# Grice-Lab/HmmUFOtu

Hardware: AMD Instinct MI355X
Metric: reads placed/sec (whole node), gg_97_otus GTR+dGamma 250bp; HBM GB/s %peak (higher is better)
Workload: dtype f64

## Files before the change

hmmufotu_amd/csrc/hu_engine.hip:

```cpp
#include <algorithm>
#include <cmath>
#include <cstdio>
#include <cstring>
#include <limits>
#include <map>
#include <atomic>
#include <thread>
#include <memory>
#include <mutex>
#include <chrono>
#include <fstream>
#include <sstream>
#include <new>
#include <stdexcept>
#include <fcntl.h>
#include <unistd.h>
#include "hu_common.h"
#include "hu_kern_sep.h"
#include "hu_kern_align.h"
#include "hu_kern_tree.h"
#include "hu_kern_blk.h"
#include "hu_kern_refsort.h"
#include "hu_kern_rank.h"
#include "hu_kern_anneal.h"
#include "hu_kern_build.h"
#include "hu_kern_otucs.h"
#include "hu_kern_sum.h"
#include "hu_sum_rule.h"
#include "hu_kern_csfm.h"
#include "hu_kern_sm.h"
#include "hu_kern_sim.h"

#define HIPCHK(call) do { hipError_t e_ = (call); if(e_ != hipSuccess) { \
	hu_set_error("%s failed: %s (%s:%d)", #call, hipGetErrorString(e_), __FILE__, __LINE__); return HU_ERR_DEVICE; } } while(0)

static const double kInf = std::numeric_limits<double>::infinity();

#include <condition_variable>
#include <functional>
struct HuPool {
	std::vector<std::thread> th;
	std::mutex m;
	std::condition_variable cvGo, cvDone;
	std::function<void(size_t)> fn;
	size_t n = 0, chunk = 64;
	std::atomic<size_t> next{0};
	uint64_t gen = 0;
	int active = 0, permit = 0;
	bool quit = false;
	std::exception_ptr err;
	explicit HuPool(unsigned nt) {
		try { th.reserve(nt); } catch(...) { return; }
		for(unsigned t = 0; t < nt; ++t) try { th.emplace_back([this] {
			uint64_t seen = 0;
			for(;;) {
				{
					std::unique_lock<std::mutex> lk(m);
					cvGo.wait(lk, [&] { return quit || gen != seen; });
					if(quit) return;
					seen = gen;
					if(permit > 0) --permit; else { if(--active == 0) cvDone.notify_all(); continue; }
				}
				work();
				std::lock_guard<std::mutex> lk(m);
				if(--active == 0) cvDone.notify_all();
			}
		}); } catch(...) { break; }
	}
	void work() noexcept {
		for(;;) {
			size_t a = next.fetch_add(chunk); if(a >= n) break; size_t e = std::min(n, a + chunk);
			try { for(size_t i = a; i < e; ++i) fn(i); }
			catch(...) { std::lock_guard<std::mutex> lk(m); if(!err) err = std::current_exception(); next = n; }
		}
	}
	template<class F> void run(size_t count, F f) {
		const int got = hu_helpers_acquire((int) th.size());
		{
			std::lock_guard<std::mutex> lk(m);
			fn = f; n = count; next = 0; active = (int) th.size(); permit = got; err = nullptr; ++gen;
		}
		cvGo.notify_all();
		work();
		std::unique_lock<std::mutex> lk(m);
		cvDone.wait(lk, [&] { return active == 0; });
		hu_helpers_release(got);
		if(err) { std::exception_ptr e = err; err = nullptr; lk.unlock(); std::rethrow_exception(e); }
	}
	~HuPool() { { std::lock_guard<std::mutex> lk(m); quit = true; } cvGo.notify_all(); for(auto& t : th) t.join(); }
};
template<class F> static void parallel_for(size_t n, F f) {
	static const unsigned cap = [] { const char* e = getenv("HU_HOST_THREADS"); int v = e ? atoi(e) : 8; return (unsigned)(v < 1 ? 1 : v > 64 ? 64 : v); }();
	unsigned nt = std::thread::hardware_concurrency();
	if(nt > cap) nt = cap;
	if(n < 512 || nt <= 1) { for(size_t i = 0; i < n; ++i) f(i); return; }
	static thread_local std::unique_ptr<HuPool> pool;
	if(!pool) pool.reset(new HuPool(nt - 1));
	pool->run(n, f);
}

template<class T> struct PinnedAlloc {
	typedef T value_type;
	PinnedAlloc() = default;
	template<class U> PinnedAlloc(const PinnedAlloc<U>&) {}
	T* allocate(size_t n) {
		void* p = nullptr;
		if(hipHostMalloc(&p, n * sizeof(T), hipHostMallocDefault) != hipSuccess) { (void) hipGetLastError(); p = malloc(n * sizeof(T)); std::lock_guard<std::mutex> lk(mtx()); pageable().push_back(p); }
		if(!p) throw std::bad_alloc();
		return (T*) p;
	}
	void deallocate(T* p, size_t) {
		{
			std::lock_guard<std::mutex> lk(mtx());
			auto& v = pageable();
			for(size_t i = 0; i < v.size(); ++i) if(v[i] == (void*) p) { v.erase(v.begin() + i); free(p); return; }
		}
		(void) hipHostFree(p);
	}
	static std::vector<void*>& pageable() { static std::vector<void*> v; return v; }
	static std::mutex& mtx() { static std::mutex m; return m; }
	template<class U> bool operator==(const PinnedAlloc<U>&) const { return true; }
	template<class U> bool operator!=(const PinnedAlloc<U>&) const { return false; }
};
template<class T> using PinnedVec = std::vector<T, PinnedAlloc<T>>;

template<class X> struct DBuf {
	X* p = nullptr; size_t cap = 0;
	int ensure(size_t n) {
		if(n <= cap) return HU_OK;
		if(p) (void) hipFree(p);
		p = nullptr; cap = 0;
		size_t want = n + n / 8 + 16;
		hipError_t e = hipMalloc((void**) &p, want * sizeof(X));
		if(e != hipSuccess) { hu_set_error("hipMalloc(%zu bytes) failed: %s", want * sizeof(X), hipGetErrorString(e)); return HU_ERR_NOMEM; }
		cap = want;
		return HU_OK;
	}
	void free_() { if(p) (void) hipFree(p); p = nullptr; cap = 0; }
	DBuf() = default;
	DBuf(const DBuf&) = delete;
	DBuf& operator=(const DBuf&) = delete;
	~DBuf() { free_(); }
};

struct hu_db {
	int device = 0;
	HuDbDev dev;
	double partialFrac = 0;
	HuModelDev mdl;
	hu_model_desc mdesc;
	HuProfileHost prof;
	std::vector<int32_t> parent, annoId;
	std::vector<double> blen, height, annoDist;
	std::vector<int8_t> seq;
	std::vector<std::string> annos, names;
	std::vector<void*> allocs;
	int64_t hbmBytes = 0;
	int32_t* dAnnoId = nullptr;
	double* dLlTab = nullptr;
	bool hasInvalidCode = false;
	std::mutex annealMu;
	bool annealReady = false;
	uint4* dInvPlane = nullptr;
	unsigned long long* dLeafMask = nullptr;
	std::vector<int32_t> colPos;
};

template<class X> static int dev_alloc(hu_db* db, X** p, size_t n) {
	size_t bytes = std::max<size_t>(n, 1) * sizeof(X);
	hipError_t e = hipMalloc((void**) p, bytes);
	if(e != hipSuccess) { hu_set_error("hipMalloc(%zu bytes) failed: %s", bytes, hipGetErrorString(e)); return HU_ERR_NOMEM; }
	db->allocs.push_back(*p);
	db->hbmBytes += (int64_t) bytes;
	return HU_OK;
}
template<class X> static int dev_upload(hu_db* db, X** p, const X* src, size_t n) {
	int rc = dev_alloc(db, p, n);
	if(rc != HU_OK) return rc;
	if(n) HIPCHK(hipMemcpy(*p, src, n * sizeof(X), hipMemcpyHostToDevice));
	return HU_OK;
}

extern "C" int hu_device_count(void) try {
	int n = 0;
	if(hipGetDeviceCount(&n) != hipSuccess) return 0;
	int ok = 0;
	for(int i = 0; i < n; ++i) {
		hipDeviceProp_t p;
		if(hipGetDeviceProperties(&p, i) == hipSuccess && strncmp(p.gcnArchName, "gfx950", 6) == 0) ok++;
	}
	return ok;
} catch(...) { return hu_catch_all("hu_device_count"); }

static int init_sym_map() {
	int8_t m[128];
	for(int i = 0; i < 128; ++i) m[i] = -1;
	m['A'] = 0; m['C'] = 1; m['G'] = 2; m['T'] = 3; m['U'] = 3;
	m['M'] = 0; m['R'] = 0; m['W'] = 0; m['S'] = 1; m['Y'] = 1; m['K'] = 2;
	m['V'] = 0; m['H'] = 0; m['D'] = 0; m['B'] = 1; m['N'] = 0;
	m['-'] = -2; m['.'] = -2; m['_'] = -2;
	HIPCHK(hipMemcpyToSymbol(HIP_SYMBOL(c_sym_map), m, sizeof(m)));
	return HU_OK;
}
static int8_t host_sym(char c) {
	switch(c) {
	case 'A': case 'M': case 'R': case 'W': case 'V': case 'H': case 'D': case 'N': return 0;
	case 'C': case 'S': case 'Y': case 'B': return 1;
	case 'G': case 'K': return 2;
	case 'T': case 'U': return 3;
	case '-': case '.': case '_': return -2;
	default: return -1;
	}
}

static hipError_t hu_wait(hipStream_t st) {
	static const bool spin = [] { const char* e = getenv("HU_SYNC"); return e && !strcmp(e, "spin"); }();
	if(spin) return hipStreamSynchronize(st);
	const auto t0 = std::chrono::steady_clock::now();
	long ns = 20000;
	for(;;) {
		const hipError_t e = hipStreamQuery(st);
		if(e != hipErrorNotReady) return e;
		if(std::chrono::steady_clock::now() - t0 < std::chrono::microseconds(30)) continue;
		timespec ts{0, ns};
		nanosleep(&ts, nullptr);
		if(ns < 100000) ns += 20000;
	}
}

extern "C" int hu_db_create(const hu_profile_desc* prof, const hu_tree_desc* tree, const hu_model_desc* model,
		int device, hu_db** out) try {
	if(!prof || !tree || !model || !out) { hu_set_error("hu_db_create: null argument"); return HU_ERR_ARG; }
	*out = nullptr;
	if(hu_device_count() <= 0) { hu_set_error("no gfx950 device visible: the engine has no CPU path"); return HU_ERR_DEVICE; }
	HIPCHK(hipSetDevice(device));
	hu_db* db = new hu_db;
	bool built = false;
	HuScope guard([&] { if(!built) hu_db_destroy(db); });
	db->device = device;
	int rc = db->prof.init(prof);
	if(rc == HU_OK) rc = hu_model_prepare(model, &db->mdl);
	if(rc != HU_OK) return rc;
	db->mdesc = *model;
	const int n = tree->n_nodes, L = tree->cs_len;
	if(n < 2 || n >= (1 << 24) || L != prof->L) { hu_set_error("tree: n_nodes %d / cs_len %d inconsistent with profile L %d", n, L, prof->L); return HU_ERR_ARG; }
	const int64_t winStart = tree->win_len > 0 ? tree->win_start : 0, winLen = tree->win_len > 0 ? tree->win_len : L;
	if(winStart < 0 || winStart + winLen > L) { hu_set_error("tree: message window out of range"); return HU_ERR_ARG; }
	db->parent.assign(tree->parent, tree->parent + n);
	db->blen.assign(tree->blen, tree->blen + n);
	db->height.assign(tree->height, tree->height + n);
	db->seq.assign(tree->seq, tree->seq + (size_t) n * L);
	if(tree->anno_id) db->annoId.assign(tree->anno_id, tree->anno_id + n);
	else { db->annoId.resize(n); for(int i = 0; i < n; ++i) db->annoId[i] = i; }
	if(tree->anno_dist) db->annoDist.assign(tree->anno_dist, tree->anno_dist + n); else db->annoDist.assign(n, 0.0);
	int root = -1, nroot = 0;
	for(int i = 0; i < n; ++i) {
		if(db->parent[i] < 0) { root = i; nroot++; }
		else if(db->parent[i] >= n) { hu_set_error("tree: parent of node %d out of range", i); return HU_ERR_ARG; }
	}
	if(nroot != 1) { hu_set_error("tree: %d roots", nroot); return HU_ERR_ARG; }
	HuDbDev& d = db->dev;
	memset(&d, 0, sizeof(d));
	d.nNodes = n; d.csLen = L; d.root = root;
	d.nNodesPad = (n + HU_NODE_PAD - 1) / HU_NODE_PAD * HU_NODE_PAD;
	d.W = (L + 31) / 32; d.WQ = (L + 127) / 128;
	d.winStart = winStart; d.winLen = winLen;
	d.K = prof->K; d.L = L;
	auto fail = [&](int code) { return code; };
	std::vector<int32_t> posCol((size_t) d.WQ * 128, -1), colPos(L, -1);
	{
		int p = 0;
		for(int k = 1; k <= prof->K; ++k) { const int c = db->prof.p2cs[k] - 1; colPos[c] = p; posCol[p++] = c; }
		for(int c = 0; c < L; ++c) if(colPos[c] < 0) { colPos[c] = p; posCol[p++] = c; }
		int32_t* dp = nullptr;
		if((rc = dev_upload(db, &dp, posCol.data(), posCol.size())) != HU_OK) return fail(rc);
		d.posCol = dp;
	}
	{
		const size_t np = d.nNodesPad, cnt = (size_t) d.WQ * 3 * np;
		std::vector<uint4> pl(cnt, make_uint4(0, 0, 0, 0));
		for(int i = 0; i < n; ++i) {
			const int8_t* s = &db->seq[(size_t) i * L];
			for(int cc = 0; cc < L; ++cc) {
				const int code = s[cc];
				if(code == -1) db->hasInvalidCode = true;
				if(code < 0) continue;
				const int c = colPos[cc];
				const int q = c >> 7, w = (c >> 5) & 3; const uint32_t bit = 1u << (c & 31);
				uint32_t* p0 = &pl[((size_t) q * 3 + 0) * np + i].x + w;
				uint32_t* p1 = &pl[((size_t) q * 3 + 1) * np + i].x + w;
				uint32_t* pv = &pl[((size_t) q * 3 + 2) * np + i].x + w;
				if(code & 1) *p0 |= bit;
				if(code & 2) *p1 |= bit;
				*pv |= bit;
			}
		}
		uint4* dp = nullptr;
		if((rc = dev_upload(db, &dp, pl.data(), cnt)) != HU_OK) return fail(rc);
		d.planes = dp;
		d.QM = (prof->K + 127) / 128;
		if(d.WQ > d.QM) {
			unsigned long long* cp = nullptr;
			if((rc = dev_alloc(db, &cp, (size_t)(d.WQ - d.QM) * 128 * 3 * (np / 64))) != HU_OK) return fail(rc);
			k_col_planes<<<dim3((unsigned)(np / 64), (unsigned)(d.WQ - d.QM)), 64>>>(d, cp);
			hipError_t e1 = hipGetLastError(), e2 = hipDeviceSynchronize();
			if(e1 != hipSuccess || e2 != hipSuccess) { hu_set_error("transposing the non-profile planes failed: %s", hipGetErrorString(e1 != hipSuccess ? e1 : e2)); return fail(HU_ERR_DEVICE); }
			d.colPlanes = cp;
		}
// ... 1046 lines not shown
	if(n_items > 0) { SCHK(hipMalloc((void**) &dItems, itemBytes)); SCHK(hipMalloc((void**) &dOut, outBytes)); }
	if(stride != cs_len) {
		SCHK(hipMemset(dRows, 0xFE, rowBytes));
		SCHK(hipMemcpy2D(dRows, (size_t) stride, rows, (size_t) cs_len, (size_t) cs_len, (size_t) n_rows, hipMemcpyHostToDevice));
	}
	else SCHK(hipMemcpy(dRows, rows, rowBytes, hipMemcpyHostToDevice));
	if(n_items > 0) SCHK(hipMemcpy(dItems, items, itemBytes, hipMemcpyHostToDevice));
	SCHK(hipDeviceSynchronize());
	g_smTiming[0] = since();
	(void) hipGetLastError();
	k_sm_counts<<<(unsigned)(n_items + n_rows), HU_SM_BLOCK>>>(dRows, n_rows, stride / 16, dItems, n_items, dOut, dBase);
	SCHK(hipGetLastError());
	SCHK(hipDeviceSynchronize());
	g_smTiming[1] = since() - g_smTiming[0];
	SCHK(hipMemcpy(base, dBase, baseBytes, hipMemcpyDeviceToHost));
	if(n_items > 0) {
		std::vector<int32_t> out((size_t) n_items * HU_SM_VALUES);
		SCHK(hipMemcpy(out.data(), dOut, outBytes, hipMemcpyDeviceToHost));
		for(int64_t i = 0; i < n_items; ++i) { memcpy(counts + 16 * i, out.data() + HU_SM_VALUES * i, 64); memcpy(dn + 4 * i, out.data() + HU_SM_VALUES * i + 16, 16); }
	}
	g_smTiming[2] = since() - g_smTiming[0] - g_smTiming[1];
	#undef SCHK
	return HU_OK;
} catch(...) { return hu_catch_all("hu_sm_counts"); }
extern "C" int hu_sm_counts_timing(double* seconds) {
	if(!seconds) return HU_ERR_ARG;
	memcpy(seconds, g_smTiming, sizeof(g_smTiming));
	return HU_OK;
}

static thread_local double g_simTiming[3] = {0, 0, 0};
extern "C" int hu_sim_reads(const hu_db* db, int64_t n, const int32_t* node, const double* rc, const int32_t* start, const int32_t* end,
		const double* gap_frac, uint64_t seed, uint64_t read0, int want_mate, char* aligned, char* seq, char* mate, int32_t* seq_len) try {
	const char* fn = "hu_sim_reads";
	if(!db || n < 0 || n > INT32_MAX || !gap_frac || (n > 0 && (!node || !rc || !start || !end || !aligned || !seq || !seq_len || (want_mate && !mate)))) { hu_set_error("%s: bad argument", fn); return HU_ERR_ARG; }
	const HuDbDev& d = db->dev;
	if(d.winStart != 0 || d.winLen != d.csLen) { hu_set_error("%s: the database holds a column window; the simulation needs the whole database", fn); return HU_ERR_ARG; }
	std::vector<int64_t> off((size_t) n);
	int64_t total = 0;
	for(int64_t r = 0; r < n; ++r) {
		if(node[r] < 0 || node[r] >= d.nNodes || node[r] == d.root) { hu_set_error("%s: read %lld: node %d is %s", fn, (long long) r, node[r], node[r] == d.root ? "the root, which has no branch above it" : "not a node of the database"); return HU_ERR_ARG; }
		if(!(start[r] >= 0 && start[r] <= end[r] && end[r] < d.csLen)) { hu_set_error("%s: read %lld: columns %d .. %d of a database of %d", fn, (long long) r, start[r], end[r], d.csLen); return HU_ERR_ARG; }
		if(!(rc[r] >= 0 && rc[r] <= 1)) { hu_set_error("%s: read %lld: branch point %g outside [0, 1]", fn, (long long) r, rc[r]); return HU_ERR_ARG; }
		off[(size_t) r] = total;
		total += (int64_t) end[r] - start[r] + 1;
	}
	if(n == 0) { g_simTiming[0] = g_simTiming[1] = g_simTiming[2] = 0; return HU_OK; }
	HIPCHK(hipSetDevice(db->device));
	const size_t L = (size_t) d.csLen, R = (size_t) n, T = (size_t) total;
	const size_t planBytes = R * (4 + 8 + 4 + 4 + 8 + 4);
	const int nOut = want_mate ? 3 : 2;
	char* dOut = nullptr; double *dGap = nullptr, *dRc = nullptr; int64_t* dOff = nullptr; int32_t* dI = nullptr;
	HuScope guard([&] { (void) hipFree(dOut); (void) hipFree(dGap); (void) hipFree(dRc); (void) hipFree(dOff); (void) hipFree(dI); });
	#define SCHK(call) do { hipError_t e_ = (call); if(e_ != hipSuccess) { hu_set_error("%s: %s failed: %s", fn, #call, hipGetErrorString(e_)); return HU_ERR_DEVICE; } } while(0)
	{
		size_t freeB = 0, totB = 0;
		SCHK(hipMemGetInfo(&freeB, &totB));
		const size_t need = T * nOut + L * 8 + planBytes + 4096;
		if(need > freeB) { hu_set_error("%s: %lld reads of %lld columns need %.3f GB of device memory, %.3f GB are free", fn, (long long) n, (long long) total, need / 1e9, freeB / 1e9); return HU_ERR_NOMEM; }
	}
	auto t0 = std::chrono::steady_clock::now();
	auto since = [&] { return std::chrono::duration<double>(std::chrono::steady_clock::now() - t0).count(); };
	SCHK(hipMalloc((void**) &dOut, T * nOut)); SCHK(hipMalloc((void**) &dGap, L * 8)); SCHK(hipMalloc((void**) &dRc, R * 8));
	SCHK(hipMalloc((void**) &dOff, R * 8)); SCHK(hipMalloc((void**) &dI, R * 16));
	SCHK(hipMemcpy(dGap, gap_frac, L * 8, hipMemcpyHostToDevice)); SCHK(hipMemcpy(dRc, rc, R * 8, hipMemcpyHostToDevice));
	SCHK(hipMemcpy(dOff, off.data(), R * 8, hipMemcpyHostToDevice));
	SCHK(hipMemcpy(dI, node, R * 4, hipMemcpyHostToDevice)); SCHK(hipMemcpy(dI + R, start, R * 4, hipMemcpyHostToDevice)); SCHK(hipMemcpy(dI + 2 * R, end, R * 4, hipMemcpyHostToDevice));
	SCHK(hipDeviceSynchronize());
	g_simTiming[0] = since();
	HuSimArgs a;
	a.up = d.up; a.down = d.down; a.blen = d.blen; a.csLen = d.csLen; a.gapFrac = dGap;
	a.node = dI; a.start = dI + R; a.end = dI + 2 * R; a.rc = dRc; a.off = dOff;
	a.key0 = (uint32_t)(seed & 0xffffffffu); a.key1 = (uint32_t)(seed >> 32); a.read0 = read0;
	a.aligned = dOut; a.seq = dOut + T; a.mate = want_mate ? dOut + 2 * T : nullptr; a.seqLen = dI + 3 * R;
	(void) hipGetLastError();
	k_sim_reads<<<(unsigned) n, HU_SIM_BLOCK>>>(db->mdl, a);
	SCHK(hipGetLastError());
	SCHK(hipDeviceSynchronize());
	g_simTiming[1] = since() - g_simTiming[0];
	std::vector<char> hOut(T * nOut); std::vector<int32_t> hLen(R);
	SCHK(hipMemcpy(hOut.data(), dOut, T * nOut, hipMemcpyDeviceToHost)); SCHK(hipMemcpy(hLen.data(), dI + 3 * R, R * 4, hipMemcpyDeviceToHost));
	memcpy(aligned, hOut.data(), T); memcpy(seq_len, hLen.data(), R * 4);
	memset(seq, 0, T); if(want_mate) memset(mate, 0, T);
	for(size_t r = 0; r < R; ++r) {
		memcpy(seq + off[r], hOut.data() + T + off[r], (size_t) hLen[r]);
		if(want_mate) memcpy(mate + off[r], hOut.data() + 2 * T + off[r], (size_t) hLen[r]);
	}
	g_simTiming[2] = since() - g_simTiming[0] - g_simTiming[1];
	#undef SCHK
	return HU_OK;
} catch(...) { return hu_catch_all("hu_sim_reads"); }
extern "C" int hu_sim_timing(double* seconds) {
	if(!seconds) return HU_ERR_ARG;
	memcpy(seconds, g_simTiming, sizeof(g_simTiming));
	return HU_OK;
}
extern "C" int hu_sim_gap_frac(const hu_db* db, int64_t n_seq, int64_t msa_len, const char* msa, double* gap_frac) try {
	const char* fn = "hu_sim_gap_frac";
	if(!db || !gap_frac || (msa && (n_seq < 1 || msa_len < 1))) { hu_set_error("%s: bad argument", fn); return HU_ERR_ARG; }
	const int64_t L = db->dev.csLen, n = db->dev.nNodes;
	std::vector<char> own;
	if(!msa) {
		std::vector<int32_t> nb((size_t) n, 0);
		for(int64_t i = 0; i < n; ++i) if(db->parent[i] >= 0) { ++nb[i]; ++nb[db->parent[i]]; }
		n_seq = 0;
		for(int64_t i = 0; i < n; ++i) n_seq += nb[i] == 1;
		if(n_seq < 1) { hu_set_error("%s: the tree has no leaf", fn); return HU_ERR_ARG; }
		own.resize((size_t) n_seq * L);
		size_t k = 0;
		for(int64_t i = 0; i < n; ++i) if(nb[i] == 1) { const int8_t* s = &db->seq[(size_t) i * L]; for(int64_t j = 0; j < L; ++j) { const int8_t b = s[j]; own[k++] = b >= 0 && b < 4 ? "ACGT"[b] : '-'; } }
		msa = own.data(); msa_len = L;
	}
	const size_t M = (size_t) msa_len, N = (size_t) n_seq;
	std::vector<int32_t> res(4 * M), gap(M), st(N), en(N), ln(N);
	std::vector<double> sw(N), wres(4 * M), wgap(M);
	const int rc = hu_msa_stats(db->device, n_seq, msa_len, msa, res.data(), gap.data(), st.data(), en.data(), ln.data(), sw.data(), wres.data(), wgap.data());
	if(rc != HU_OK) return rc;
	const bool prune = own.empty();
	int64_t kept = 0;
	for(size_t j = 0; j < M; ++j) kept += !prune || (res[j] | res[M + j] | res[2 * M + j] | res[3 * M + j]) != 0;
	if(kept != L) { hu_set_error("%s: %lld columns of the alignment hold a residue, the database has %lld columns", fn, (long long) kept, (long long) L); return HU_ERR_ARG; }
	size_t k = 0;
	for(size_t j = 0; j < M; ++j) {
		if(prune && !(res[j] | res[M + j] | res[2 * M + j] | res[3 * M + j])) continue;
		const double numRes = (wres[j] + wres[2 * M + j]) + (wres[M + j] + wres[3 * M + j]);
		gap_frac[k++] = wgap[j] / (numRes + wgap[j]);
	}
	return HU_OK;
} catch(...) { return hu_catch_all("hu_sim_gap_frac"); }

extern "C" int hu_device_mem_info(int device, int64_t* free_bytes, int64_t* total_bytes) try {
	if(hu_device_count() <= 0) { hu_set_error("no gfx950 device visible: the engine has no CPU path"); return HU_ERR_DEVICE; }
	HIPCHK(hipSetDevice(device));
	size_t f = 0, t = 0;
	HIPCHK(hipMemGetInfo(&f, &t));
	if(free_bytes) *free_bytes = (int64_t) f; if(total_bytes) *total_bytes = (int64_t) t;
	return HU_OK;
} catch(...) { return hu_catch_all("hu_device_mem_info"); }
extern "C" int hu_device_malloc(int device, int64_t bytes, void** out) try {
	if(!out || bytes < 1) { hu_set_error("hu_device_malloc: bad argument"); return HU_ERR_ARG; }
	*out = nullptr;
	if(hu_device_count() <= 0) { hu_set_error("no gfx950 device visible: the engine has no CPU path"); return HU_ERR_DEVICE; }
	HIPCHK(hipSetDevice(device));
	const hipError_t e = hipMalloc(out, (size_t) bytes);
	if(e != hipSuccess) { (void) hipGetLastError(); *out = nullptr; hu_set_error("hipMalloc(%lld bytes) failed: %s", (long long) bytes, hipGetErrorString(e)); return HU_ERR_NOMEM; }
	return HU_OK;
} catch(...) { return hu_catch_all("hu_device_malloc"); }
extern "C" void hu_device_free(int device, void* p) try {
	if(!p) return;
	if(hipSetDevice(device) == hipSuccess) (void) hipFree(p);
} catch(...) { (void) hu_catch_all("hu_device_free"); }

namespace {
struct HuSaDev {
	uint8_t* text = nullptr; uint64_t* key[2] = {nullptr, nullptr}; uint32_t* pos[2] = {nullptr, nullptr};
	uint32_t *rank = nullptr, *hist = nullptr, *tileSum = nullptr;
	int cur = 0;
	void dropKeys() { (void) hipFree(key[0]); (void) hipFree(key[1]); key[0] = key[1] = nullptr; }
	~HuSaDev() { dropKeys(); (void) hipFree(text); (void) hipFree(pos[0]); (void) hipFree(pos[1]); (void) hipFree(rank); (void) hipFree(hist); (void) hipFree(tileSum); }
};
inline uint32_t sa_bits(uint64_t v) { uint32_t b = 0; while(v) { ++b; v >>= 1; } return b; }
}
#define SCHK(call) do { hipError_t e_ = (call); if(e_ != hipSuccess) { hu_set_error("%s: %s failed: %s", fn, #call, hipGetErrorString(e_)); return HU_ERR_DEVICE; } } while(0)
static int sa_build(const char* fn, int device, const uint8_t* text, int64_t n64, int64_t extraBytes, HuSaDev& d, int32_t* rounds, double* seconds) {
	if(!text || n64 < 1 || n64 >= (1ll << 31)) { hu_set_error("%s: the text must hold 1 .. 2^31 - 1 symbols, got %lld", fn, (long long) n64); return HU_ERR_ARG; }
	const size_t n = (size_t) n64;
	for(size_t i = 0; i < n; ++i) if(text[i] > 4) { hu_set_error("%s: symbol %d at text position %zu (0 = separator, 1..4 = bases)", fn, (int) text[i], i); return HU_ERR_ARG; }
	if(hu_device_count() <= 0) { hu_set_error("no gfx950 device visible: the engine has no CPU path"); return HU_ERR_DEVICE; }
	SCHK(hipSetDevice(device));
	const uint32_t nTiles = (uint32_t)((n + HU_SA_TILE - 1) / HU_SA_TILE);
	const size_t m = (size_t) nTiles * 256, nScanN = (n + 1023) / 1024, nScanM = (m + 1023) / 1024;
	{
		size_t freeB = 0, totB = 0;
		SCHK(hipMemGetInfo(&freeB, &totB));
		const size_t need = n + 2 * 8 * n + 2 * 4 * n + 4 * n + 4 * m + 4 * (std::max(nScanN, nScanM) + 1) + (size_t) std::max<int64_t>(extraBytes, 0) + 4096;
		if(need > freeB) { hu_set_error("%s: a text of %zu symbols needs %.3f GB of device memory, %.3f GB are free", fn, n, need / 1e9, freeB / 1e9); return HU_ERR_NOMEM; }
	}
	SCHK(hipMalloc((void**) &d.text, n)); SCHK(hipMalloc((void**) &d.key[0], 8 * n)); SCHK(hipMalloc((void**) &d.key[1], 8 * n));
	SCHK(hipMalloc((void**) &d.pos[0], 4 * n)); SCHK(hipMalloc((void**) &d.pos[1], 4 * n)); SCHK(hipMalloc((void**) &d.rank, 4 * n));
	SCHK(hipMalloc((void**) &d.hist, 4 * m)); SCHK(hipMalloc((void**) &d.tileSum, 4 * (std::max(nScanN, nScanM) + 1)));
	SCHK(hipMemcpy(d.text, text, n, hipMemcpyHostToDevice));
	(void) hipGetLastError();
	const auto t0 = std::chrono::steady_clock::now();
	const unsigned gN = (unsigned)((n + 255) / 256), gT = (nTiles + 3) / 4;
	auto pass = [&](int shift) {
		k_sa_hist<<<gT, 256>>>(d.key[d.cur], n, shift, nTiles, d.hist);
		k_sa_scan_sums<<<(unsigned) nScanM, 1024>>>(m, d.hist, d.tileSum);
		k_sa_scan_tiles<<<1, 1024>>>(nScanM, d.tileSum);
		k_sa_scan_apply<<<(unsigned) nScanM, 1024>>>(m, d.hist, d.tileSum);
		k_sa_scatter<<<gT, 256>>>(d.key[d.cur], d.pos[d.cur], n, shift, nTiles, d.hist, d.key[d.cur ^ 1], d.pos[d.cur ^ 1]);
		d.cur ^= 1;
	};
	uint32_t groups = 0;
	auto rank = [&]() -> int {
		k_sa_head_sums<<<(unsigned) nScanN, 1024>>>(d.key[d.cur], n, d.tileSum);
		k_sa_scan_tiles<<<1, 1024>>>(nScanN, d.tileSum);
		k_sa_rank<<<(unsigned) nScanN, 1024>>>(d.key[d.cur], d.pos[d.cur], n, d.tileSum, d.rank);
		SCHK(hipGetLastError());
		SCHK(hipMemcpy(&groups, d.tileSum + nScanN, 4, hipMemcpyDeviceToHost));
		return HU_OK;
	};
	k_sa_key0<<<gN, 256>>>(d.text, n, d.key[d.cur], d.pos[d.cur]);
	for(int shift = 0; shift < 3 * HU_SA_H0; shift += 8) pass(shift);
	int rc = rank();
	if(rc != HU_OK) return rc;
	int32_t r = 0;
	const int32_t maxRounds = (int32_t) sa_bits(n - 1) + 2;
	for(size_t h = HU_SA_H0; groups < n; h *= 2) {
		if(++r > maxRounds || groups == 0) { hu_set_error("%s: internal: %u of %zu suffixes told apart after %d doubling rounds", fn, groups, n, (int) r - 1); return HU_ERR_STATE; }
		k_sa_key<<<gN, 256>>>(d.rank, n, h, d.key[d.cur], d.pos[d.cur]);
		for(int shift = 0; shift < (int) sa_bits(groups); shift += 8) pass(shift);
		for(int shift = 0; shift < (int) sa_bits(groups - 1); shift += 8) pass(32 + shift);
		if((rc = rank()) != HU_OK) return rc;
	}
	SCHK(hipDeviceSynchronize());
	if(rounds) *rounds = r;
	if(seconds) *seconds = std::chrono::duration<double>(std::chrono::steady_clock::now() - t0).count();
	return HU_OK;
}
extern "C" int32_t hu_suffix_array_tile(void) { return HU_SA_TILE; }
extern "C" int hu_suffix_array(int device, const uint8_t* text, int64_t n, int32_t* sa, int32_t* rounds, double* device_seconds) try {
	const char* fn = "hu_suffix_array";
	if(!sa) { hu_set_error("%s: bad argument", fn); return HU_ERR_ARG; }
	HuSaDev d;
	const int rc = sa_build(fn, device, text, n, 0, d, rounds, device_seconds);
	if(rc != HU_OK) return rc;
	SCHK(hipMemcpy(sa, d.pos[d.cur], 4 * (size_t) n, hipMemcpyDeviceToHost));
	return HU_OK;
} catch(...) { return hu_catch_all("hu_suffix_array"); }
int hu_csfm_device_pass(int device, const uint8_t* text, int64_t n64, uint8_t* bwt, uint64_t* marks, uint32_t* sampled, int32_t* rounds, double* sa_seconds) {
	const char* fn = "hu_csfm_write";
	HuSaDev d;
	const int rc = sa_build(fn, device, text, n64, 0, d, rounds, sa_seconds);
	if(rc != HU_OK) return rc;
	const size_t n = (size_t) n64, nScan = (n + 1023) / 1024, nWords = (n + 63) / 64, nSamp = (n + 3) / 4;
	d.dropKeys();
	uint8_t* dBwt = nullptr; unsigned long long* dMarks = nullptr; uint32_t* dSamp = nullptr;
	HuScope guard([&] { (void) hipFree(dBwt); (void) hipFree(dMarks); (void) hipFree(dSamp); });
	SCHK(hipMalloc((void**) &dBwt, n)); SCHK(hipMalloc((void**) &dMarks, 8 * nWords)); SCHK(hipMalloc((void**) &dSamp, 4 * nSamp));
	k_csfm_bwt<<<(unsigned) nScan, 1024>>>(d.text, d.pos[d.cur], n, dBwt, dMarks, d.tileSum);
	k_sa_scan_tiles<<<1, 1024>>>(nScan, d.tileSum);
	k_csfm_samples<<<(unsigned) nScan, 1024>>>(d.pos[d.cur], n, d.tileSum, nSamp, dSamp);
	SCHK(hipGetLastError());
	uint32_t got = 0;
	SCHK(hipMemcpy(&got, d.tileSum + nScan, 4, hipMemcpyDeviceToHost));
	if(got != nSamp) { hu_set_error("%s: internal: %u sampled rows, expected %zu: the sort did not return a permutation", fn, got, nSamp); return HU_ERR_STATE; }
	SCHK(hipMemcpy(bwt, dBwt, n, hipMemcpyDeviceToHost)); SCHK(hipMemcpy(marks, dMarks, 8 * nWords, hipMemcpyDeviceToHost));
	SCHK(hipMemcpy(sampled, dSamp, 4 * nSamp, hipMemcpyDeviceToHost));
	return HU_OK;
}
#undef SCHK

extern "C" int hu_tree_loglik(int device, int32_t n_nodes, int32_t cs_len, int32_t root, const hu_model_desc* model, const double* up_dev,
		double* per_col, double* sum) try {
	if(n_nodes < 1 || cs_len < 1 || root < 0 || root >= n_nodes || !model || !up_dev || !sum) { hu_set_error("hu_tree_loglik: bad argument"); return HU_ERR_ARG; }
	if(((uintptr_t) up_dev) & 15) { hu_set_error("hu_tree_loglik: the message buffer must be 16-byte aligned"); return HU_ERR_ARG; }
	if(hu_device_count() <= 0) { hu_set_error("no gfx950 device visible: the engine has no CPU path"); return HU_ERR_DEVICE; }
	HuModelDev mdl;
	int rc = hu_model_prepare(model, &mdl);
	if(rc != HU_OK) return rc;
	HIPCHK(hipSetDevice(device));
	const int64_t L = cs_len;
	DBuf<double> dOut;
	if((rc = dOut.ensure((size_t) L)) != HU_OK) return rc;
	(void) hipGetLastError();
	k_tree_loglik<<<(unsigned)((L + 255) / 256), 256>>>(up_dev + (size_t) root * L * 4, L, mdl.pi[0], mdl.pi[1], mdl.pi[2], mdl.pi[3], dOut.p);
	HIPCHK(hipGetLastError());
	std::vector<double> own;
	if(!per_col) { own.resize((size_t) L); per_col = own.data(); }
	HIPCHK(hipMemcpy(per_col, dOut.p, (size_t) L * 8, hipMemcpyDeviceToHost));
	double s = 0;
	for(int64_t j = 0; j < L; ++j) s += per_col[j];
	*sum = s;
	return HU_OK;
} catch(...) { return hu_catch_all("hu_tree_loglik"); }


typedef HuPlaceRec HostPlace;

struct HuKnobs {
	int viterbi_hbm = 0;
	int viterbi_values = 0;
	int viterbi_mode = 0;
	int viterbi_dec1 = 0;
	int vw_diag = 0;
	int viterbi_force_redo = 0;
	int tile_unsorted = 0;
	int pairs32 = 0;
	int topk_fast_min = 16384;
	int topk_general = 0;
	int scan_pairs = 0;
	int streaming_sep = 0;
	int est_unsorted = 0, place_unsorted = 0;
	int xcd_map = 1;
	int est_var = 0, place_var = 0;
	int place_nosplit = 0;
	int place_lds_pad = 0;
	int est_lds_pad = 0;
	int vit_lds_pad = 0;
	int scan_lds_pad = 0;
	int trace = 0;
	int width_split = 1;
	int sort_seq = 0;
	int refsort_wgs = HU_RS_WGS_PER_CU * 256;
	int ref_nofuse = 0;
	int refsort_host = 0;
	int inject_fault = 0;
};
struct HuKnobEntry { const char* name; int HuKnobs::* field; };
static const HuKnobEntry kKnobs[] = {
	{"viterbi_hbm", &HuKnobs::viterbi_hbm}, {"viterbi_values", &HuKnobs::viterbi_values}, {"viterbi_mode", &HuKnobs::viterbi_mode},
	{"viterbi_dec1", &HuKnobs::viterbi_dec1}, {"vw_diag", &HuKnobs::vw_diag}, {"viterbi_force_redo", &HuKnobs::viterbi_force_redo},
	{"pairs32", &HuKnobs::pairs32}, {"tile_unsorted", &HuKnobs::tile_unsorted}, {"topk_fast_min", &HuKnobs::topk_fast_min}, {"scan_pairs", &HuKnobs::scan_pairs}, {"topk_general", &HuKnobs::topk_general}, {"streaming_sep", &HuKnobs::streaming_sep},
	{"est_unsorted", &HuKnobs::est_unsorted}, {"place_unsorted", &HuKnobs::place_unsorted}, {"xcd_map", &HuKnobs::xcd_map},
	{"est_var", &HuKnobs::est_var}, {"place_var", &HuKnobs::place_var}, {"place_nosplit", &HuKnobs::place_nosplit}, {"width_split", &HuKnobs::width_split},
	{"place_lds_pad", &HuKnobs::place_lds_pad}, {"est_lds_pad", &HuKnobs::est_lds_pad}, {"vit_lds_pad", &HuKnobs::vit_lds_pad}, {"scan_lds_pad", &HuKnobs::scan_lds_pad}, {"trace", &HuKnobs::trace}, {"inject_fault", &HuKnobs::inject_fault}, {"refsort_host", &HuKnobs::refsort_host}, {"ref_nofuse", &HuKnobs::ref_nofuse}, {"refsort_wgs", &HuKnobs::refsort_wgs}, {"sort_seq", &HuKnobs::sort_seq},
};
static void knobs_from_env(HuKnobs& k) {
	for(const HuKnobEntry& e : kKnobs) {
		std::string env = "HU_";
		for(const char* c = e.name; *c; ++c) env += (char) toupper(*c);
		const char* v = getenv(env.c_str());
		if(!v) continue;
		char* end = nullptr;
		const long x = strtol(v, &end, 10);
		k.*(e.field) = (end == v) ? 1 : (int) x;
	}
}

enum { ST_NONE = 0, ST_READS = 1, ST_ALIGNED = 2, ST_SEEDED = 3, ST_ESTIMATED = 4, ST_FILTERED = 5, ST_PLACED = 6, ST_FINISHED = 7 };

struct hu_batch {
	hu_db* db = nullptr;
	int maxReads = 0, n = 0, nSeq = 0, state = ST_NONE;
	bool paired = false, fromCodes = false, profile = false;
	HuKnobs knob;
	int maxBases = 1 << 30;
	bool fixedRoot = false;
	bool placesGiven = false;
	bool pair16 = false;
	int scanWidth = 0;
	int pairsKind = 0;
	int seedCap = HU_MAX_SEEDS;
	hipStream_t stream = nullptr;
	hipEvent_t ev[2 * HU_T_COUNT];
	bool evSet[HU_T_COUNT] = {false};
	float ms[HU_T_COUNT];
	double wall[4] = {0, 0, 0, 0};
	DBuf<char> dBases, dTraces, dRows;
	DBuf<HuReadDesc> dDescs;
	DBuf<double> dScratch;
	DBuf<uint8_t> dDec;
	DBuf<HuVitOut> dVit;
	DBuf<HuAlnDev> dAlns;
	DBuf<int8_t> dCodes;
	DBuf<int32_t> dStart, dEnd, dSeedCnt, dSeedId, dGiven, dPermCnt;
	DBuf<uint16_t> dPerm;
	DBuf<uint32_t> dRp, dPairs, dSeedDN, dParDN, dBmin, dRSpan, dTileSpan;
	DBuf<int32_t> dTileQ, dSlotRead, dReadSlot;
	DBuf<uint32_t> dRq, dTileW;
	DBuf<unsigned long long> dRefScratch;
	DBuf<int32_t> dHv, dZeroPar; DBuf<unsigned long long> dPairsC; int refHvCount = 0; double refHvHeight = NAN;
	DBuf<int32_t> dBail, dNanCnt, dNanId; DBuf<uint32_t> dNanDN;
	int nRefBail = 0;
	DBuf<uint32_t> dRefPiv; DBuf<unsigned long long> dRefL0; bool refFused = false;
	int refHostAll = 0;
	DBuf<int32_t> dIns, dTileIns, dRetry;
	DBuf<uint32_t> dSortK, dSortV;
	DBuf<uint32_t> dCsCnt;
	DBuf<HuEstOut> dEst;
	DBuf<HuCand> dCands;
	DBuf<HuPlaceOut> dPlaceOut;
	DBuf<int32_t> dCandCnt, dCandOff, dMeta;
	DBuf<uint8_t> dFiltSlot;
	DBuf<HuPlaceRec> dPlaces;
	DBuf<hu_place_rec> dBest;
	size_t nc = 0;
	int maxGapSites = 0, maxBaseSites = 0;
	bool hostCands = false;
	DBuf<double> dRootLL;
	PinnedVec<double> hRootLL;
	std::vector<HuReadDesc> hDescs;
	std::vector<char> hBases;
	PinnedVec<HuVitOut> hVit;
	int64_t cellsTotal = 0, cornerTotal = 0;
	int rMain = 0;
	int maxAll = 1, maxMain = 1;
	std::vector<int32_t> wideReads;
	std::vector<uint32_t> hWideOrd, hWideCand; DBuf<uint32_t> dWideOrd, dWideCand;
	PinnedVec<int32_t> hCandOffAll;
	DBuf<double> dRedoScr; DBuf<HuReadDesc> dRedoDesc; DBuf<HuVitOut> dRedoVit;
	PinnedVec<HuAlnDev> hAlns;
	DBuf<int32_t> dAnRow, dAnThr, dAnTileQ; DBuf<int2> dAnReg; DBuf<uint32_t> dAnMasks; DBuf<unsigned long long> dAnHits;
	PinnedVec<int32_t> hStart, hEnd, hSeedCnt, hSeedId;
	PinnedVec<uint32_t> hSeedDN;
	PinnedVec<HuCand> hCands;
	std::vector<int64_t> candOffs;
	std::vector<HostPlace> places;
	PinnedVec<hu_place_rec> best;
	PinnedVec<int32_t> hMeta, hBail;
	PinnedVec<char> hRows;
	DBuf<uint32_t> dSumBits; DBuf<unsigned char> dSumCls; DBuf<int4> dSumOut; PinnedVec<int4> hSumOut; bool sumReady = false;
	std::vector<char> tsvBuf; std::vector<size_t> tsvOff, tsvLen; size_t tsvSize = 0;
};

struct Timer {
	hu_batch* b; int id;
	Timer(hu_batch* b, int id) : b(b), id(id) { if(b->profile) (void) hipEventRecord(b->ev[2 * id], b->stream); }
	~Timer() { if(b->profile) { (void) hipEventRecord(b->ev[2 * id + 1], b->stream); b->evSet[id] = true; } }
};

extern "C" int hu_batch_create(hu_db* db, int max_reads, hu_batch** out) try {
	if(!db || !out || max_reads < 1) { hu_set_error("hu_batch_create: bad argument"); return HU_ERR_ARG; }
	HIPCHK(hipSetDevice(db->device));
	hu_batch* b = new hu_batch;
	b->db = db; b->maxReads = max_reads;
	knobs_from_env(b->knob);
	for(int i = 0; i < 2 * HU_T_COUNT; ++i) b->ev[i] = nullptr;
	for(int i = 0; i < HU_T_COUNT; ++i) b->ms[i] = 0;
	hipError_t e = hipStreamCreateWithFlags(&b->stream, hipStreamNonBlocking);
	for(int i = 0; i < 2 * HU_T_COUNT && e == hipSuccess; ++i) e = hipEventCreate(&b->ev[i]);
	if(e != hipSuccess) {
		hu_set_error("hu_batch_create: stream / event creation failed: %s", hipGetErrorString(e));
		for(int i = 0; i < 2 * HU_T_COUNT; ++i) if(b->ev[i]) (void) hipEventDestroy(b->ev[i]);
		if(b->stream) (void) hipStreamDestroy(b->stream);
		delete b;
		return HU_ERR_DEVICE;
	}
	*out = b;
	return HU_OK;
} catch(...) { return hu_catch_all("hu_batch_create"); }
extern "C" int hu_batch_set_knob(hu_batch* b, const char* name, int value) try {
	if(!b || !name) return HU_ERR_ARG;
	for(const HuKnobEntry& e : kKnobs) if(strcmp(e.name, name) == 0) { b->knob.*(e.field) = value; return HU_OK; }
	hu_set_error("hu_batch_set_knob: no knob named '%s'", name);
	return HU_ERR_ARG;
} catch(...) { return hu_catch_all("hu_batch_set_knob"); }
extern "C" void hu_batch_destroy(hu_batch* b) try {
	if(!b) return;
	(void) hipSetDevice(b->db->device);
	(void) hu_wait(b->stream);
	for(int i = 0; i < 2 * HU_T_COUNT; ++i) (void) hipEventDestroy(b->ev[i]);
	(void) hipStreamDestroy(b->stream);
	delete b;
} catch(...) { (void) hu_catch_all("hu_batch_destroy"); }
extern "C" int hu_batch_sync(hu_batch* b) try { if(!b) return HU_ERR_ARG; HIPCHK(hu_wait(b->stream)); return HU_OK; } catch(...) { return hu_catch_all("hu_batch_sync"); }
extern "C" int hu_batch_profile(hu_batch* b, int enable) try { if(!b) return HU_ERR_ARG; b->profile = enable != 0; return HU_OK; } catch(...) { return hu_catch_all("hu_batch_profile"); }
extern "C" int hu_batch_timings(hu_batch* b, float* ms) try {
	if(!b || !ms) return HU_ERR_ARG;
	HIPCHK(hu_wait(b->stream));
	for(int i = 0; i < HU_T_COUNT; ++i) {
		float t = 0;
		if(b->profile && b->evSet[i] && hipEventElapsedTime(&t, b->ev[2 * i], b->ev[2 * i + 1]) == hipSuccess) b->ms[i] = t;
		ms[i] = b->ms[i];
	}
	return HU_OK;
} catch(...) { return hu_catch_all("hu_batch_timings"); }

static void build_regions(const hu_db* db, int L, const int32_t* vp , HuReadDesc& rd) {
	const int K = db->dev.K;
	const double kMinGapFrac = 0.2;
	struct VP { int start, end, from, to, nIns, nDel; } v[2];
	int nv = 0;
	for(int p = 0; p < 2 && vp; ++p) {
		VP x{vp[p*6], vp[p*6+1], vp[p*6+2], vp[p*6+3], vp[p*6+4], vp[p*6+5]};
		bool valid = x.start > 0 && x.start <= x.end && x.from > 0 && x.from <= x.to && x.nIns >= 0 && x.nDel >= 0;
		if(valid && x.end <= K && x.to <= L) v[nv++] = x;
	}
	rd.nRegions = 0;
	int64_t off = 0, doff = 0;
	auto add = [&](int j0, int j1, int i0, int i1, int withB, int band, const VP* bp) {
		HuRegion& g = rd.reg[rd.nRegions++];
		g.j0 = j0; g.j1 = j1; g.i0 = i0; g.i1 = i1; g.withB = withB; g.band = band;
		g.from = bp ? bp->from : 0; g.start = bp ? bp->start : 0; g.nIns = bp ? bp->nIns : 0; g.nDel = bp ? bp->nDel : 0;
		g.off = off; g.doff = doff;
		if(j1 >= j0 && i1 >= i0) {
			off += (int64_t)(j1 - j0 + 1) * (i1 - i0 + 1);
			const int64_t ni = i1 - i0 + 1, nj = j1 - j0 + 1;
			int64_t sz = (ni + nj - 1) * ((ni + 15) & ~15);
			sz = std::max(sz, (ni + nj - 1) * 64);
			sz = std::max(sz, (nj + (ni + 3) / 4 - 1) * 256);
			sz = std::max(sz, (nj + (ni + 7) / 8 - 1) * 512);
			doff += (sz + 15) & ~(int64_t) 15;
		}
	};
	if(nv == 0) add(1, K, 1, L, 1, 0, nullptr);
	else {
		for(int p = 0; p < nv; ++p) {
			int upQLen = p == 0 ? v[p].from - 1 : v[p].from - v[p - 1].to;
			if(upQLen < 0) upQLen = 0;
			int up_start = p == 0 ? v[p].start - upQLen * (1 + kMinGapFrac) : v[p - 1].end;
			if(up_start < 1) up_start = 1;
			int up_from = p == 0 ? v[p].from - upQLen * (1 + kMinGapFrac) : v[p - 1].to;
			if(up_from < 1) up_from = 1;
			add(up_start, v[p].start, up_from, v[p].from, 1, 0, nullptr);
			add(v[p].start, v[p].end, v[p].from, v[p].to, 1, 1, &v[p]);
		}
		const VP& last = v[nv - 1];
		int downQLen = L - last.to;
		int down_end = last.end + downQLen * (1 + kMinGapFrac);
		int down_to = last.to + downQLen * (1 + kMinGapFrac);
		if(down_end > K) down_end = K;
		if(down_to > L) down_to = L;
		add(last.end, down_end, last.to, down_to, 0, 0, nullptr);
	}
	int64_t coff = 0;
	for(int r = 0; r < rd.nRegions; ++r) {
		HuRegion& g = rd.reg[r];
		int nearI = INT32_MAX, nearJ = INT32_MAX;
		for(int r2 = r + 1; r2 < rd.nRegions; ++r2) {
			const HuRegion& g2 = rd.reg[r2];
			if(g2.i1 >= g2.i0 && g2.j1 >= g2.j0) { nearI = std::min(nearI, g2.i0 - 1); nearJ = std::min(nearJ, g2.j0 - 1); }
		}
		g.ci0 = std::max(g.i0, nearI); g.cj0 = std::max(g.j0, nearJ); g.coff = coff;
		if(nearI == INT32_MAX || g.ci0 > g.i1 || g.cj0 > g.j1 || g.i1 < g.i0 || g.j1 < g.j0) { g.ci0 = g.i1 + 1; g.cj0 = g.j1 + 1; }
		else coff += (int64_t)(g.i1 - g.ci0 + 1) * (g.j1 - g.cj0 + 1);
	}
	rd.scratchOff = off;
	rd.decOff = doff;
	rd.cornerOff = coff;
}

static int upload_descs(hu_batch* b) {
	int rc;
	if((rc = b->dDescs.ensure(b->hDescs.size())) != HU_OK) return rc;
	HIPCHK(hipMemcpyAsync(b->dDescs.p, b->hDescs.data(), b->hDescs.size() * sizeof(HuReadDesc), hipMemcpyHostToDevice, b->stream));
	return HU_OK;
}

extern "C" int hu_batch_set_reads(hu_batch* b, int n, const char* bases, const int64_t* offs, const int32_t* vpaths,
		const char* mates, const int64_t* moffs, const int32_t* mvpaths) try {
	if(!b || n < 0 || n > b->maxReads || (n > 0 && (!bases || !offs))) { hu_set_error("hu_batch_set_reads: bad argument"); return HU_ERR_ARG; }
	if(mates && !moffs) { hu_set_error("hu_batch_set_reads: mates without offsets"); return HU_ERR_ARG; }
	HIPCHK(hipSetDevice(b->db->device));
	b->n = n; b->paired = mates != nullptr; b->nSeq = b->paired ? 2 * n : n; b->fromCodes = false;
	b->hDescs.assign(b->nSeq, HuReadDesc());
	b->hBases.clear();
	b->maxBases = 0;
	for(int r = 0; r < n; ++r) {
		const int64_t l = (offs[r + 1] - offs[r]) + (mates ? moffs[r + 1] - moffs[r] : 0);
		if(l > b->maxBases) b->maxBases = (int) std::min<int64_t>(l, 1 << 30);
	}
	int64_t cells = 0, tr = 0, decs = 0, corners = 0;
	for(int s = 0; s < b->nSeq; ++s) {
		const bool isMate = s >= n;
		const int r = isMate ? s - n : s;
		const char* src = isMate ? mates + moffs[r] : bases + offs[r];
		const int64_t len64 = isMate ? moffs[r + 1] - moffs[r] : offs[r + 1] - offs[r];
		HuReadDesc& rd = b->hDescs[s];
		memset(&rd, 0, sizeof(rd));
		rd.baseOff = (int64_t) b->hBases.size();
		rd.len = (int32_t) len64;
		bool bad = len64 < 1 || len64 > 65535;
		for(int64_t i = 0; i < len64 && !bad; ++i) if(host_sym(src[i]) < 0) bad = true;
		if(!bad) {
			b->hBases.insert(b->hBases.end(), src, src + len64);
			const int32_t* vp = isMate ? (mvpaths ? mvpaths + (size_t) r * 12 : nullptr) : (vpaths ? vpaths + (size_t) r * 12 : nullptr);
			build_regions(b->db, rd.len, vp, rd);
			const int64_t c = rd.scratchOff, dc = rd.decOff, cc = rd.cornerOff;
			rd.scratchOff = cells; cells += c;
			rd.decOff = decs; decs += dc;
			rd.cornerOff = corners; corners += cc;
		}
		else { rd.len = 0; rd.nRegions = 0; }
		rd.traceOff = tr;
		tr += rd.len + b->db->dev.K + 8;
	}
	int rc;
	if((rc = b->dBases.ensure(b->hBases.size() + 1)) != HU_OK) return rc;
	b->cellsTotal = cells; b->cornerTotal = corners;
	if((rc = b->dDec.ensure((size_t) decs + 1)) != HU_OK) return rc;
	if((rc = b->dTraces.ensure((size_t) tr + 1)) != HU_OK) return rc;
	if((rc = b->dVit.ensure(b->nSeq)) != HU_OK) return rc;
	if(!b->hBases.empty()) HIPCHK(hipMemcpyAsync(b->dBases.p, b->hBases.data(), b->hBases.size(), hipMemcpyHostToDevice, b->stream));
	if((rc = upload_descs(b)) != HU_OK) return rc;
	b->state = ST_READS;
	return HU_OK;
} catch(...) { return hu_catch_all("hu_batch_set_reads"); }

static int ensure_read_buffers(hu_batch* b) {
	const HuDbDev& d = b->db->dev;
	const size_t n = (size_t) b->n;
	const size_t tiles = (n + HU_READ_TILE - 1) / HU_READ_TILE;
	int rc;
	if((rc = b->dCodes.ensure(n * d.csLen)) != HU_OK) return rc;
	if((rc = b->dStart.ensure(n)) != HU_OK) return rc;
	if((rc = b->dEnd.ensure(n)) != HU_OK) return rc;
	if((rc = b->dRp.ensure(tiles * d.WQ * HU_READ_TILE * 16)) != HU_OK) return rc;
	if((rc = b->dTileQ.ensure(tiles * (d.WQ + 1))) != HU_OK) return rc;
	if((rc = b->dTileW.ensure(std::max<size_t>(tiles, 1) * d.WQ * HU_TILEW_QUAD)) != HU_OK) return rc;
	if((rc = b->dSlotRead.ensure(std::max<size_t>(tiles, 1) * HU_READ_TILE)) != HU_OK) return rc;
	if((rc = b->dReadSlot.ensure(std::max<size_t>(n, 1))) != HU_OK) return rc;
	if((rc = b->dRq.ensure(std::max<size_t>(n, 1) * ((d.WQ + 31) / 32))) != HU_OK) return rc;
	if((rc = b->dIns.ensure(std::max<size_t>(n, 1) * (HU_MAX_INS + 1))) != HU_OK) return rc;
	if((rc = b->dTileIns.ensure(std::max<size_t>(tiles, 1) * HU_TILEINS_STRIDE)) != HU_OK) return rc;
	if((rc = b->dRSpan.ensure(std::max<size_t>(n, 1) * 2)) != HU_OK) return rc;
	if((rc = b->dTileSpan.ensure(std::max<size_t>(tiles, 1) * 2)) != HU_OK) return rc;
	return HU_OK;
}

static int order_by_key(hu_batch* b, const uint32_t* key, const uint32_t* val, size_t n, uint32_t bound, uint32_t* out, bool runsInOrder) {
	if(!n) return HU_OK;
	const size_t m = (size_t) bound + 1;
	int rc;
	const size_t nTiles = (m + 1023) / 1024;
	if((rc = b->dCsCnt.ensure(3 * m + nTiles + 8)) != HU_OK) return rc;
	uint32_t* cnt = b->dCsCnt.p; uint32_t* start = cnt + m; uint32_t* cur = start + m + 1; uint32_t* tiles = cur + m;
	HIPCHK(hipMemsetAsync(cnt, 0, m * 4, b->stream));
	k_cs_hist<<<(unsigned)((n + 255) / 256), 256, 0, b->stream>>>((int) n, key, bound, cnt);
	k_cs_tile_sums<<<(unsigned) nTiles, 1024, 0, b->stream>>>((int) m, cnt, tiles);
	k_cs_scan_tiles<<<1, 1024, 0, b->stream>>>((int) nTiles, tiles);
	k_cs_scan<<<(unsigned) nTiles, 1024, 0, b->stream>>>((int) m, cnt, tiles, start, cur);
	k_cs_scatter<<<(unsigned)((n + 255) / 256), 256, 0, b->stream>>>((int) n, key, val, bound, cur, out);
	if(runsInOrder) k_cs_runs<<<(unsigned)((m + 3) / 4), 256, 0, b->stream>>>((int) bound, start, out);
	HIPCHK(hipGetLastError());
	return HU_OK;
}

static int tile_reads(hu_batch* b, const HuAlnDev* alns) {
	const int n = b->n;
	if(!n) return HU_OK;
	const int tiles = (n + HU_READ_TILE - 1) / HU_READ_TILE;
	int rc;
	if((rc = b->dSortK.ensure((size_t) n * 2)) != HU_OK || (rc = b->dSortV.ensure((size_t) n * 2)) != HU_OK) return rc;
	k_tile_keys<<<(n + 255) / 256, 256, 0, b->stream>>>(n, alns, b->dStart.p, b->dEnd.p, b->dSortK.p, b->dSortV.p);
	if(b->knob.tile_unsorted) HIPCHK(hipMemcpyAsync(b->dSortV.p + n, b->dSortV.p, (size_t) n * 4, hipMemcpyDeviceToDevice, b->stream));
	else if((rc = order_by_key(b, b->dSortK.p, b->dSortV.p, (size_t) n, (uint32_t) b->db->dev.csLen + 1u, b->dSortV.p + n, true)) != HU_OK) return rc;
	k_tile_slots<<<(tiles * HU_READ_TILE + 255) / 256, 256, 0, b->stream>>>(n, tiles * HU_READ_TILE, b->dSortV.p + n, b->dSlotRead.p, b->dReadSlot.p);
	HIPCHK(hipGetLastError());
	return HU_OK;
}

static int set_aligned_impl(hu_batch* b, int n, const int8_t* codes, hipMemcpyKind kind, const int32_t* start, const int32_t* end, int maxBases = -1) {
	if(!b || n < 0 || n > b->maxReads || (n > 0 && (!codes || !start || !end))) { hu_set_error("hu_batch_set_aligned: bad argument"); return HU_ERR_ARG; }
	HIPCHK(hipSetDevice(b->db->device));
	const HuDbDev& d = b->db->dev;
	b->n = n; b->nSeq = n; b->paired = false; b->fromCodes = true;
	if(maxBases >= 0) b->maxBases = maxBases;
	else {
		int mb = 0;
		for(int r = 0; r < n; ++r) {
			if(!(start[r] >= 0 && start[r] <= end[r] && end[r] < d.csLen)) continue;
			const int8_t* c = codes + (size_t) r * d.csLen; int k = 0;
			for(int j = start[r]; j <= end[r]; ++j) k += c[j] >= 0;
			mb = std::max(mb, k);
		}
		b->maxBases = mb;
	}
	int rc;
	if((rc = ensure_read_buffers(b)) != HU_OK) return rc;
	b->hAlns.assign(n, HuAlnDev());
	b->hStart.assign(start, start + n); b->hEnd.assign(end, end + n);
	for(int r = 0; r < n; ++r) {
		HuAlnDev& a = b->hAlns[r];
		memset(&a, 0, sizeof(a));
		const bool ok = start[r] >= 0 && start[r] <= end[r] && end[r] < d.csLen && start[r] >= d.winStart && end[r] < d.winStart + d.winLen;
		a.status = ok ? HU_READ_OK : HU_READ_INVALID;
		a.csStart = start[r] + 1; a.csEnd = end[r] + 1;
		if(!ok) { b->hStart[r] = (int32_t) d.winStart; b->hEnd[r] = (int32_t) d.winStart - 1; }
	}
	(void) hipGetLastError();
	if(n) {
		if((const void*) codes != (const void*) b->dCodes.p) HIPCHK(hipMemcpyAsync(b->dCodes.p, codes, (size_t) n * d.csLen, kind, b->stream));
		HIPCHK(hipMemcpyAsync(b->dStart.p, b->hStart.data(), (size_t) n * 4, hipMemcpyHostToDevice, b->stream));
		HIPCHK(hipMemcpyAsync(b->dEnd.p, b->hEnd.data(), (size_t) n * 4, hipMemcpyHostToDevice, b->stream));
		const int tiles = (n + HU_READ_TILE - 1) / HU_READ_TILE;
		HIPCHK(hipMemsetAsync(b->dRp.p, 0, (size_t) tiles * d.WQ * HU_READ_TILE * 16 * 4, b->stream));
		if((rc = tile_reads(b, nullptr)) != HU_OK) return rc;
		k_planes_from_codes<<<n, 64, 0, b->stream>>>(d, b->dCodes.p, b->dStart.p, b->dEnd.p, b->dRp.p, b->dRq.p, b->dIns.p, b->dReadSlot.p, (uint2*) b->dRSpan.p);
		k_tile_lists<<<tiles, 64, 0, b->stream>>>(d, n, b->dRp.p, b->dRq.p, b->dIns.p, b->dTileQ.p, b->dTileW.p, b->dTileIns.p, b->dSlotRead.p, (const uint2*) b->dRSpan.p, (uint2*) b->dTileSpan.p);
		HIPCHK(hipGetLastError());
// ... 399 lines not shown
		for(int i = 0; i < hb[0]; ++i) nNan += (hb[2 + i] >> 26) == 3;
		const bool nanOnDevice = nNan > 16;
		if(nanOnDevice) {
			if((rc = b->dNanCnt.ensure((size_t) n)) != HU_OK || (rc = b->dNanId.ensure((size_t) n * HU_MAX_SEEDS)) != HU_OK || (rc = b->dNanDN.ensure((size_t) n * HU_MAX_SEEDS)) != HU_OK) return rc;
			if(b->pair16) k_seed_topk<uint16_t><<<n, 256, 0, b->stream>>>(d0, (const uint16_t*) b->dPairs.p, o->max_height, o->max_nseed, b->dNanCnt.p, b->dNanId.p, b->dNanDN.p, b->knob.topk_fast_min);
			else k_seed_topk<uint32_t><<<n, 256, 0, b->stream>>>(d0, b->dPairs.p, o->max_height, o->max_nseed, b->dNanCnt.p, b->dNanId.p, b->dNanDN.p, b->knob.topk_fast_min);
			k_take_nan_rows<<<hb[0], 64, 0, b->stream>>>(d0, b->dBail.p, b->dPairs.p, b->pair16 ? 1 : 0, b->dNanCnt.p, b->dNanId.p, b->dNanDN.p, b->dSeedCnt.p, b->dSeedId.p, b->dSeedDN.p, b->dParDN.p);
			HIPCHK(hipGetLastError());
			if(b->knob.trace) fprintf(stderr, "[hu] reference seed order: %d reads with a NaN distance take the (dist, node id) selection on the device\n", nNan);
		}
		for(int i = 0; i < hb[0]; ++i) if(!(nanOnDevice && (hb[2 + i] >> 26) == 3)) only.push_back(hb[2 + i] & 0x3ffffff);
		std::sort(only.begin(), only.end());
		if(!only.empty()) return seed_order_libstdcxx(b, o, &only);
	}
	return HU_OK;
}

static int seed_order_libstdcxx(hu_batch* b, const hu_opts* o, const std::vector<int32_t>* only) {
	const hu_db* db = b->db;
	const HuDbDev& d = db->dev;
	const size_t n = (size_t) b->n, np = (size_t) d.nNodesPad, K = (size_t) o->max_nseed;
	if(only) {
		const size_t rowB = np * (b->pair16 ? 2 : 4);
		std::vector<uint8_t> rowBuf(rowB);
		std::vector<uint64_t> a;
		const bool p16 = b->pair16;
		for(int32_t r : *only) {
			HIPCHK(hipMemcpyAsync(rowBuf.data(), (const uint8_t*) b->dPairs.p + (size_t) r * rowB, rowB, hipMemcpyDeviceToHost, b->stream));
			HIPCHK(hu_wait(b->stream));
			const uint16_t* q16 = (const uint16_t*) rowBuf.data(); const uint32_t* q32 = (const uint32_t*) rowBuf.data();
			auto pairOf = [&](int i) -> uint32_t { return p16 ? (((uint32_t)(q16[i] >> 8) << 16) | (q16[i] & 0xffu)) : q32[i]; };
			a.clear();
			bool nan = false;
			for(int i = 0; i < d.nNodes; ++i) {
				if(i == d.root || !(db->height[i] <= o->max_height)) continue;
				const uint32_t pr = pairOf(i); const uint64_t dd = pr >> 16, N = pr & 0xffffu;
				if(N == 0) { nan = true; a.push_back((((uint64_t) 1 << 39) + 1) << 24 | (uint64_t) i); continue; }
				a.push_back(((dd << 39) / N) << 24 | (uint64_t) i);
			}
			const size_t keep = std::min(K, a.size());
			if(!nan) hu_sort_prefix_packed(a.data(), a.size(), K); else std::partial_sort(a.begin(), a.begin() + keep, a.end());
			int32_t cnt = (b->hAlns[r].status == HU_READ_OK && b->hEnd[r] >= b->hStart[r]) ? (int32_t) keep : 0;
			int32_t ids[HU_MAX_SEEDS]; uint32_t dn[HU_MAX_SEEDS], pn[HU_MAX_SEEDS];
			for(size_t s = 0; s < keep; ++s) { const int id = (int)(a[s] & 0xffffffu); ids[s] = id; dn[s] = pairOf(id); pn[s] = pairOf(db->parent[id]); }
			HIPCHK(hipMemcpyAsync(b->dSeedCnt.p + r, &cnt, 4, hipMemcpyHostToDevice, b->stream));
			HIPCHK(hipMemcpyAsync(b->dSeedId.p + (size_t) r * HU_MAX_SEEDS, ids, keep * 4, hipMemcpyHostToDevice, b->stream));
			HIPCHK(hipMemcpyAsync(b->dSeedDN.p + (size_t) r * HU_MAX_SEEDS, dn, keep * 4, hipMemcpyHostToDevice, b->stream));
			HIPCHK(hipMemcpyAsync(b->dParDN.p + (size_t) r * HU_MAX_SEEDS, pn, keep * 4, hipMemcpyHostToDevice, b->stream));
			HIPCHK(hu_wait(b->stream));
		}
		return HU_OK;
	}
	const size_t rowBytes = np * (b->pair16 ? 2 : 4);
	const size_t CH = std::max<size_t>(1, std::min<size_t>(n, (192u << 20) / rowBytes));
	b->hSeedCnt.assign(n, 0); b->hSeedId.assign(n * HU_MAX_SEEDS, 0); b->hSeedDN.assign(n * HU_MAX_SEEDS, 0);
	PinnedVec<uint32_t> hPar(n * HU_MAX_SEEDS, 0);
	PinnedVec<uint8_t> buf[2];
	buf[0].resize(CH * rowBytes); buf[1].resize(CH * rowBytes);
	hipEvent_t ev[2] = {nullptr, nullptr};
	HuScope guard([&] { for(int i = 0; i < 2; ++i) if(ev[i]) (void) hipEventDestroy(ev[i]); });
	for(int i = 0; i < 2; ++i) HIPCHK(hipEventCreateWithFlags(&ev[i], hipEventDisableTiming));
	auto copy = [&](size_t c) -> int {
		const size_t r0 = c * CH, cnt = std::min(CH, n - r0);
		HIPCHK(hipMemcpyAsync(buf[c & 1].data(), (const uint8_t*) b->dPairs.p + r0 * rowBytes, cnt * rowBytes, hipMemcpyDeviceToHost, b->stream));
		HIPCHK(hipEventRecord(ev[c & 1], b->stream));
		return HU_OK;
	};
	const size_t nChunks = (n + CH - 1) / CH;
	const double maxH = o->max_height;
	const bool p16 = b->pair16;
	const uint64_t nanKey = ((uint64_t) 1 << 39) + 1;
	static const std::vector<uint64_t> key16 = [] {
		std::vector<uint64_t> t(65536);
		for(uint32_t v = 0; v < 65536; ++v) { const uint64_t dd = v >> 8, N = v & 0xffu; t[v] = N ? (dd << 39) / N : ((uint64_t) 1 << 39) + 1; }
		return t;
	}();
	int rc;
	if(nChunks && (rc = copy(0)) != HU_OK) return rc;
	for(size_t c = 0; c < nChunks; ++c) {
		HIPCHK(hipEventSynchronize(ev[c & 1]));
		if(c + 1 < nChunks && (rc = copy(c + 1)) != HU_OK) return rc;
		const size_t r0 = c * CH, cnt = std::min(CH, n - r0);
		const uint8_t* rows = buf[c & 1].data();
		static const unsigned sortThreads = [] { const char* e = getenv("HU_SORT_THREADS"); int v = e ? atoi(e) : 32; unsigned hw = std::thread::hardware_concurrency(); if(hw < 1) hw = 1; return (unsigned) std::min<int>(std::max(v, 1), (int) hw); }();
		std::atomic<size_t> next{0};
		auto oneRead = [&](size_t k) {
			const size_t r = r0 + k;
			if(b->hAlns[r].status != HU_READ_OK || b->hEnd[r] < b->hStart[r]) return;
			static thread_local std::vector<uint64_t> a;
			a.clear();
			const uint16_t* q16 = (const uint16_t*)(rows + k * rowBytes); const uint32_t* q32 = (const uint32_t*)(rows + k * rowBytes);
			auto pairOf = [&](int i) -> uint32_t { return p16 ? (((uint32_t)(q16[i] >> 8) << 16) | (q16[i] & 0xffu)) : q32[i]; };
			bool nan = false;
			for(int i = 0; i < d.nNodes; ++i) {
				if(i == d.root || !(db->height[i] <= maxH)) continue;
				if(p16) {
					const uint64_t kk = key16[q16[i]];
					nan |= kk == nanKey;
					a.push_back(kk << 24 | (uint64_t) i);
					continue;
				}
				const uint32_t pr = q32[i]; const uint64_t dd = pr >> 16, N = pr & 0xffffu;
				if(N == 0) { nan = true; a.push_back(nanKey << 24 | (uint64_t) i); continue; }
				a.push_back(((dd << 39) / N) << 24 | (uint64_t) i);
			}
			const size_t keep = std::min(K, a.size());
			if(!nan) hu_sort_prefix_packed(a.data(), a.size(), K);
			else std::partial_sort(a.begin(), a.begin() + keep, a.end());
			b->hSeedCnt[r] = (int32_t) keep;
			for(size_t s = 0; s < keep; ++s) {
				const int id = (int)(a[s] & 0xffffffu);
				b->hSeedId[r * HU_MAX_SEEDS + s] = id;
				b->hSeedDN[r * HU_MAX_SEEDS + s] = pairOf(id);
				hPar[r * HU_MAX_SEEDS + s] = pairOf(db->parent[id]);
			}
		};
		hu_run_threads(std::min<unsigned>(sortThreads, (unsigned) cnt), [&] { for(;;) { const size_t k = next.fetch_add(4); if(k >= cnt) break; for(size_t q = k; q < std::min(cnt, k + 4); ++q) oneRead(q); } });
	}
	if(n) {
		HIPCHK(hipMemcpyAsync(b->dSeedCnt.p, b->hSeedCnt.data(), n * 4, hipMemcpyHostToDevice, b->stream));
		HIPCHK(hipMemcpyAsync(b->dSeedId.p, b->hSeedId.data(), n * HU_MAX_SEEDS * 4, hipMemcpyHostToDevice, b->stream));
		HIPCHK(hipMemcpyAsync(b->dSeedDN.p, b->hSeedDN.data(), n * HU_MAX_SEEDS * 4, hipMemcpyHostToDevice, b->stream));
		HIPCHK(hipMemcpyAsync(b->dParDN.p, hPar.data(), n * HU_MAX_SEEDS * 4, hipMemcpyHostToDevice, b->stream));
		HIPCHK(hu_wait(b->stream));
	}
	return HU_OK;
}

extern "C" int hu_seed_batch(hu_batch* b, const hu_opts* o) try {
	if(!b || !o) return HU_ERR_ARG;
	if(b->state < ST_ALIGNED) { hu_set_error("hu_seed_batch: reads are not aligned"); return HU_ERR_STATE; }
	if(o->max_nseed < 1 || o->max_nseed > HU_MAX_SEEDS) { hu_set_error("max_nseed must be in 1..%d", HU_MAX_SEEDS); return HU_ERR_ARG; }
	HIPCHK(hipSetDevice(b->db->device));
	const HuDbDev& d = b->db->dev;
	const size_t n = (size_t) b->n;
	int rc;
	const int nBlk = d.nNodesPad / 256;
	const bool manyPartial = b->db->partialFrac > 0.02 && b->knob.scan_pairs != -1;
	if(o->seed_order != HU_SEED_ORDER_STABLE && o->seed_order != HU_SEED_ORDER_LIBSTDCXX) { hu_set_error("seed_order must be HU_SEED_ORDER_STABLE or HU_SEED_ORDER_LIBSTDCXX"); return HU_ERR_ARG; }
	const bool refOrder = o->seed_order == HU_SEED_ORDER_LIBSTDCXX;
	const bool dOnly = !refOrder && b->knob.scan_pairs != 1 && !manyPartial && o->max_height == INFINITY && nBlk >= 2 * o->max_nseed && nBlk <= 2048 && d.nNodes - 1 >= o->max_nseed;
	const bool narrow = !b->knob.pairs32 && b->maxBases <= 255;
	b->pair16 = !dOnly && narrow;
	b->pairsKind = dOnly ? 0 : (b->pair16 ? 16 : 32);
	b->scanWidth = dOnly ? (narrow ? 1 : 2) : 0;
	if((rc = b->dPairs.ensure(std::max<size_t>(n, 1) * d.nNodesPad / (dOnly ? (narrow ? 4 : 2) : (b->pair16 ? 2 : 1)))) != HU_OK) return rc;
	if((rc = b->dSeedCnt.ensure(n)) != HU_OK) return rc;
	if((rc = b->dSeedId.ensure(n * HU_MAX_SEEDS)) != HU_OK) return rc;
	if((rc = b->dSeedDN.ensure(n * HU_MAX_SEEDS)) != HU_OK) return rc;
	if((rc = b->dParDN.ensure(n * HU_MAX_SEEDS)) != HU_OK) return rc;
	uint32_t* bmin = nullptr;
	if(dOnly) {
		if((rc = b->dBmin.ensure(std::max<size_t>(n, 1) * nBlk + 16)) != HU_OK) return rc;
		if((rc = b->dRetry.ensure(n + 1)) != HU_OK) return rc;
		bmin = b->dBmin.p;
	}
	b->refFused = refOrder && n > 0 && ref_fused_l0(b, o, b->pair16);
	if(b->refFused) {
		if((rc = b->dRefPiv.ensure(n * 4)) != HU_OK || (rc = b->dRefL0.ensure(n * (size_t)(d.nNodesPad / 64) * 2)) != HU_OK) return rc;
		k_ref_pivots<<<(unsigned)((n + 63) / 64), 64, 0, b->stream>>>(d, read_planes(b), b->n, b->dRefPiv.p);
		HIPCHK(hipGetLastError());
	}
	uint32_t* stat = bmin && b->knob.trace ? bmin + n * nBlk : nullptr;
	if(stat) HIPCHK(hipMemsetAsync(stat, 0, 64, b->stream));
	(void) hipGetLastError();
	if(n) {
		const int tiles = (b->n + HU_READ_TILE - 1) / HU_READ_TILE;
		const dim3 grid(tiles, d.nNodesPad / 256);
		{
			Timer t(b, HU_T_SEED_PDIST);
			const dim3 grid4(tiles, (d.nNodesPad + 1023) / 1024);
			if(dOnly && narrow) k_seed_dscan4<uint8_t><<<grid4, 256, (size_t)(b->knob.scan_lds_pad > 0 && b->knob.scan_lds_pad <= 44 ? b->knob.scan_lds_pad : 0) * 1024, b->stream>>>(d, b->dRp.p, b->dTileQ.p, (uint8_t*) b->dPairs.p, b->dSlotRead.p, bmin, (const uint2*) b->dTileSpan.p);
			else if(dOnly) k_seed_dscan4<uint16_t><<<grid4, 256, 0, b->stream>>>(d, b->dRp.p, b->dTileQ.p, (uint16_t*) b->dPairs.p, b->dSlotRead.p, bmin, (const uint2*) b->dTileSpan.p);
			else if(b->refFused && b->pair16) k_seed_pdist2<uint16_t, true><<<grid, 256, 0, b->stream>>>(d, b->dTileW.p, b->dTileQ.p, b->dTileIns.p, (uint16_t*) b->dPairs.p, b->dSlotRead.p, b->dRefPiv.p, b->dRefL0.p);
			else if(b->refFused) k_seed_pdist2<uint32_t, true><<<grid, 256, 0, b->stream>>>(d, b->dTileW.p, b->dTileQ.p, b->dTileIns.p, b->dPairs.p, b->dSlotRead.p, b->dRefPiv.p, b->dRefL0.p);
			else if(b->pair16) k_seed_pdist2<uint16_t><<<grid, 256, 0, b->stream>>>(d, b->dTileW.p, b->dTileQ.p, b->dTileIns.p, (uint16_t*) b->dPairs.p, b->dSlotRead.p);
			else k_seed_pdist2<uint32_t><<<grid, 256, 0, b->stream>>>(d, b->dTileW.p, b->dTileQ.p, b->dTileIns.p, b->dPairs.p, b->dSlotRead.p);
		}
		{
			Timer t(b, HU_T_SEED_TOPK);
			if(dOnly) {
				int32_t* retry = b->dRetry.p;
				HIPCHK(hipMemsetAsync(retry, 0, 4, b->stream));
				#define TOPK_ARGS(T) d, (const T*) b->dPairs.p, bmin, read_planes(b), o->max_nseed, b->dSeedCnt.p, b->dSeedId.p, b->dSeedDN.p, b->dParDN.p, stat, retry
				if(narrow) { k_seed_topk_straight<uint8_t><<<b->n, 256, 0, b->stream>>>(TOPK_ARGS(uint8_t), b->knob.topk_general); k_seed_topk_d<uint8_t, true><<<std::min(b->n, 1024), 256, 0, b->stream>>>(TOPK_ARGS(uint8_t)); }
				else { k_seed_topk_straight<uint16_t><<<b->n, 256, 0, b->stream>>>(TOPK_ARGS(uint16_t), b->knob.topk_general); k_seed_topk_d<uint16_t, true><<<std::min(b->n, 1024), 256, 0, b->stream>>>(TOPK_ARGS(uint16_t)); }
				#undef TOPK_ARGS
			}
			else if(refOrder) { if((rc = seed_order_libstdcxx_device(b, o)) != HU_OK) return rc; }
			else {
				if(b->pair16) k_seed_topk<uint16_t><<<b->n, 256, 0, b->stream>>>(d, (const uint16_t*) b->dPairs.p, o->max_height, o->max_nseed, b->dSeedCnt.p, b->dSeedId.p, b->dSeedDN.p, b->knob.topk_fast_min);
				else k_seed_topk<uint32_t><<<b->n, 256, 0, b->stream>>>(d, b->dPairs.p, o->max_height, o->max_nseed, b->dSeedCnt.p, b->dSeedId.p, b->dSeedDN.p, b->knob.topk_fast_min);
				k_parent_pairs<<<((unsigned) n * HU_MAX_SEEDS + 255) / 256, 256, 0, b->stream>>>(d, b->n, b->dPairs.p, b->pair16 ? 1 : 0, b->dSeedCnt.p, b->dSeedId.p, b->dParDN.p);
			}
		}
		k_seed_drop_empty<<<(b->n + 255) / 256, 256, 0, b->stream>>>(b->n, b->dStart.p, b->dEnd.p, b->dSeedCnt.p);
		HIPCHK(hipGetLastError());
		if(stat) {
			uint32_t h[16];
			HIPCHK(hipMemcpyAsync(h, stat, 64, hipMemcpyDeviceToHost, b->stream)); HIPCHK(hu_wait(b->stream));
			fprintf(stderr, "[hu] top-k after the distance-only scan: %u of %zu reads on the block path (%.1f blocks, %.1f candidates per read), %u by the exact recomputation; "
				"%u of them through the general launch\n",
				h[0] + h[8], n, h[0] + h[8] ? (double) h[1] / (h[0] + h[8]) : 0.0, h[0] + h[8] ? (double) h[2] / (h[0] + h[8]) : 0.0, h[3], h[8]);
		}
	}
	b->seedCap = o->max_nseed;
	b->state = ST_SEEDED;
	return HU_OK;
} catch(...) { return hu_catch_all("hu_seed_batch"); }

__global__ void k_seed_drop_empty(int n, const int32_t* __restrict__ rstart, const int32_t* __restrict__ rend, int32_t* __restrict__ seedCnt) {
	const int r = blockIdx.x * 256 + threadIdx.x;
	if(r < n && rend[r] < rstart[r]) seedCnt[r] = 0;
}

__global__ void k_seed_given(HuDbDev db, HuReadPlanes R, int n, const int32_t* __restrict__ cnt, const int32_t* __restrict__ ids,
		const int32_t* __restrict__ distIds, int32_t* __restrict__ seedCnt, int32_t* __restrict__ seedId, uint32_t* __restrict__ seedDN, uint32_t* __restrict__ parDN) {
	const int i = blockIdx.x * 256 + threadIdx.x;
	if(i >= n * HU_MAX_SEEDS) return;
	const int r = i / HU_MAX_SEEDS, sl = i % HU_MAX_SEEDS;
	if(sl == 0) seedCnt[r] = cnt[r];
	if(sl < cnt[r]) {
		seedId[i] = ids[i];
		seedDN[i] = pair_exact(db, R, r, distIds ? distIds[i] : ids[i]);
		parDN[i] = pair_exact(db, R, r, db.parent[ids[i]]);
	}
}

extern "C" int hu_seed_batch_given(hu_batch* b, const int32_t* n_seeds, const int32_t* ids, const int32_t* dist_ids, int stride) try {
	if(!b || (b->n > 0 && (!n_seeds || !ids)) || stride < 1) { hu_set_error("hu_seed_batch_given: bad argument"); return HU_ERR_ARG; }
	if(b->state < ST_ALIGNED) { hu_set_error("hu_seed_batch_given: reads are not aligned"); return HU_ERR_STATE; }
	HIPCHK(hipSetDevice(b->db->device));
	const HuDbDev& d = b->db->dev;
	const size_t n = (size_t) b->n;
	std::vector<int32_t> pk((n * 3) * HU_MAX_SEEDS + n, 0);
	int32_t* pc = pk.data(); int32_t* pi = pc + n; int32_t* pd = pi + n * HU_MAX_SEEDS;
	for(size_t r = 0; r < n; ++r) {
		const int c = n_seeds[r];
		if(c < 0 || c > HU_MAX_SEEDS || c > stride) { hu_set_error("hu_seed_batch_given: read %zu has %d seeds (0..%d)", r, c, std::min(stride, (int) HU_MAX_SEEDS)); return HU_ERR_ARG; }
		pc[r] = c;
		for(int k = 0; k < c; ++k) {
			const int32_t id = ids[r * stride + k], di = dist_ids ? dist_ids[r * stride + k] : id;
			if(id < 0 || id >= d.nNodes || b->db->parent[id] < 0 || di < 0 || di >= d.nNodes) { hu_set_error("hu_seed_batch_given: read %zu seed %d names node %d / %d", r, k, id, di); return HU_ERR_ARG; }
			pi[r * HU_MAX_SEEDS + k] = id; pd[r * HU_MAX_SEEDS + k] = di;
		}
	}
	int rc;
	b->pair16 = false; b->pairsKind = 0; b->scanWidth = 0;
	if((rc = b->dSeedCnt.ensure(n)) != HU_OK) return rc;
	if((rc = b->dSeedId.ensure(n * HU_MAX_SEEDS)) != HU_OK) return rc;
	if((rc = b->dSeedDN.ensure(n * HU_MAX_SEEDS)) != HU_OK) return rc;
	if((rc = b->dParDN.ensure(n * HU_MAX_SEEDS)) != HU_OK) return rc;
	if((rc = b->dGiven.ensure(pk.size())) != HU_OK) return rc;
	(void) hipGetLastError();
	if(n) {
		HIPCHK(hipMemcpyAsync(b->dGiven.p, pk.data(), pk.size() * 4, hipMemcpyHostToDevice, b->stream));
		{
			Timer t(b, HU_T_SEED_PDIST);
			k_seed_given<<<((unsigned) n * HU_MAX_SEEDS + 255) / 256, 256, 0, b->stream>>>(d, read_planes(b), b->n, b->dGiven.p, b->dGiven.p + n,
					dist_ids ? b->dGiven.p + n + n * HU_MAX_SEEDS : nullptr, b->dSeedCnt.p, b->dSeedId.p, b->dSeedDN.p, b->dParDN.p);
			k_seed_drop_empty<<<(b->n + 255) / 256, 256, 0, b->stream>>>(b->n, b->dStart.p, b->dEnd.p, b->dSeedCnt.p);
		}
		HIPCHK(hipGetLastError());
		HIPCHK(hu_wait(b->stream));
	}
	b->seedCap = 1;
	for(size_t r = 0; r < n; ++r) b->seedCap = std::max(b->seedCap, (int) n_seeds[r]);
	b->state = ST_SEEDED;
	return HU_OK;
} catch(...) { return hu_catch_all("hu_seed_batch_given"); }

__global__ void k_seed_sortkeys(int n, const int32_t* __restrict__ seedCnt, const int32_t* __restrict__ seedId, uint32_t* __restrict__ key, uint32_t* __restrict__ val) {
	const int i = blockIdx.x * 256 + threadIdx.x;
	if(i >= n * HU_MAX_SEEDS) return;
	key[i] = (i % HU_MAX_SEEDS) < seedCnt[i / HU_MAX_SEEDS] ? (uint32_t) seedId[i] : 0xffffffffu;
	val[i] = (uint32_t) i;
}

static void plan_width_split(hu_batch* b) {
	b->rMain = 0; b->wideReads.clear(); b->maxAll = b->maxMain = 1;
	if((int) b->hStart.size() < b->n || (int) b->hEnd.size() < b->n) return;
	std::vector<int> R((size_t) b->n);
	for(int r = 0; r < b->n; ++r) { R[r] = std::max(0, b->hEnd[r] - b->hStart[r] + 1); b->maxAll = std::max(b->maxAll, R[r]); }
	b->maxMain = b->maxAll;
	if(!b->knob.width_split || b->n < 256) return;
	const int W = std::min(64, b->n / 128);
	std::vector<int> tmp(R);
	std::nth_element(tmp.begin(), tmp.begin() + W, tmp.end(), std::greater<int>());
	const int kth = tmp[W];
	static const int bounds[] = {512, 768, 1024, 1536, 2048, 3072};
	int bound = 0;
	for(int x : bounds) if(kth <= x) { bound = x; break; }
	if(!bound || bound >= b->maxAll) return;
	b->rMain = bound; b->maxMain = 1;
	for(int r = 0; r < b->n; ++r) { if(R[r] > bound) b->wideReads.push_back(r); else b->maxMain = std::max(b->maxMain, R[r]); }
	if(b->knob.trace) fprintf(stderr, "[hu] width split: %zu of %d reads beyond %d columns (widest %d) take a launch of their own\n", b->wideReads.size(), b->n, bound, b->maxAll);
}
static HuDbDev width_pass_dev(const hu_batch* b, int pass, const uint32_t* wideList) {
	HuDbDev dev = b->db->dev;
	if(b->rMain) { dev.rLo = pass ? b->rMain : -1; dev.rHi = pass ? 0x7fffffff : b->rMain; dev.wideList = pass ? wideList : nullptr; }
	return dev;
}

extern "C" int hu_estimate_batch(hu_batch* b, const hu_opts* o) try {
	if(!b || !o) return HU_ERR_ARG;
	if(b->state < ST_SEEDED) { hu_set_error("hu_estimate_batch: no seeds"); return HU_ERR_STATE; }
	HIPCHK(hipSetDevice(b->db->device));
	const size_t n = (size_t) b->n;
	int rc;
	if((rc = b->dEst.ensure(n * HU_MAX_SEEDS)) != HU_OK) return rc;
	(void) hipGetLastError();
	if(n) {
		Timer t(b, HU_T_ESTIMATE);
		plan_width_split(b);
		const bool stream = b->knob.streaming_sep != 0;
		if(b->rMain) {
			b->hWideOrd.clear();
			for(int r : b->wideReads) for(int sd = 0; sd < HU_MAX_SEEDS; ++sd) b->hWideOrd.push_back((uint32_t) r * HU_MAX_SEEDS + sd);
			if((rc = b->dWideOrd.ensure(b->hWideOrd.size())) != HU_OK) return rc;
			HIPCHK(hipMemcpyAsync(b->dWideOrd.p, b->hWideOrd.data(), b->hWideOrd.size() * 4, hipMemcpyHostToDevice, b->stream));
		}
		for(int pass = 0; pass < (b->rMain ? 2 : 1); ++pass) {
			const int maxR = pass ? b->maxAll : b->maxMain;
			const HuDbDev dev = width_pass_dev(b, pass, b->dWideOrd.p);
			#define EST_ARGS dev, b->db->mdl, b->dCodes.p, b->dStart.p, b->dEnd.p, b->dParDN.p, b->dSeedCnt.p, b->dSeedId.p, b->dSeedDN.p, o->weighted, b->dEst.p
			const unsigned eg = pass ? (unsigned) b->hWideOrd.size() : (unsigned) b->n * HU_MAX_SEEDS;
			const uint32_t* order = nullptr;
			if(pass) order = b->dWideOrd.p;
			else if(!b->knob.est_unsorted) {
				if((rc = b->dSortK.ensure((size_t) eg * 2)) != HU_OK || (rc = b->dSortV.ensure((size_t) eg * 2)) != HU_OK) return rc;
				k_seed_sortkeys<<<(eg + 255) / 256, 256, 0, b->stream>>>(b->n, b->dSeedCnt.p, b->dSeedId.p, b->dSortK.p, b->dSortV.p);
				if((rc = order_by_key(b, b->dSortK.p, b->dSortV.p, (size_t) eg, (uint32_t) b->db->dev.nNodes, b->dSortV.p + eg, false)) != HU_OK) return rc;
				order = b->dSortV.p + eg;
			}
			const int spt = (maxR + 255) / 256;
			const int xm = b->knob.xcd_map;
			const unsigned egl = pass ? eg : order ? std::min<unsigned>(eg, (unsigned) b->n * (unsigned) b->seedCap) : eg;
			const int var = b->knob.est_var;
			auto said = [&](const char* k) { if(b->knob.trace) fprintf(stderr, "[hu] estimate: max region %d, %s\n", maxR, k); };
			if(stream || spt > 12) { said("k_estimate"); k_estimate<<<eg, 64, 0, b->stream>>>(EST_ARGS); }
			else if(var == 2) {
				if(spt <= 2) { said("k_estimate_blk<2,256>"); k_estimate_blk<2, 256><<<eg, 256, 0, b->stream>>>(EST_ARGS); }
				else if(spt <= 4) { said("k_estimate_blk<4,256>"); k_estimate_blk<4, 256><<<eg, 256, 0, b->stream>>>(EST_ARGS); }
				else if(spt <= 6) { said("k_estimate_blk<6,256>"); k_estimate_blk<6, 256><<<eg, 256, 0, b->stream>>>(EST_ARGS); }
				else if(spt <= 8) { said("k_estimate_blk<8,256>"); k_estimate_blk<8, 256><<<eg, 256, 0, b->stream>>>(EST_ARGS); }
				else { said("k_estimate_blk<12,256>"); k_estimate_blk<12, 256><<<eg, 256, 0, b->stream>>>(EST_ARGS); }
			}
			else if(var == 98 && spt > 4 && spt <= 6) {
				said("k_estimate_prod<6,4,4,true>");
				DBuf<long long> ddb;
				if((rc = ddb.ensure((size_t) egl * 4)) != HU_OK) return rc;
				HIPCHK(hipMemsetAsync(ddb.p, 0, (size_t) egl * 4 * sizeof(long long), b->stream));
				k_estimate_prod<6, 4, 4, true><<<egl, 256, 0, b->stream>>>(EST_ARGS, order, xm, ddb.p);
				std::vector<long long> hd((size_t) egl * 4);
				HIPCHK(hipMemcpyAsync(hd.data(), ddb.p, hd.size() * sizeof(long long), hipMemcpyDeviceToHost, b->stream));
				HIPCHK(hu_wait(b->stream));
				double acc[4] = {0}; size_t ran = 0;
				for(size_t c = 0; c < (size_t) egl; ++c) if(hd[c * 4 + 3]) { ++ran; for(int i = 0; i < 4; ++i) acc[i] += (double) hd[c * 4 + i]; }
				if(ran) fprintf(stderr, "[est dbg] per slot (s_memtime ticks, %zu slots): prologue %.0f load %.0f rest %.0f total %.0f\n", ran, acc[0] / ran, acc[1] / ran, acc[2] / ran, acc[3] / ran);
			}
			else if(var == 1 && spt <= 6) { said("k_estimate_prod<12,2>"); k_estimate_prod<12, 2><<<egl, 128, 0, b->stream>>>(EST_ARGS, order, xm); }
			else if(var == 3 && spt <= 6) { said("k_estimate_prod<6,4,1>"); k_estimate_prod<6, 4, 1><<<egl, 256, 0, b->stream>>>(EST_ARGS, order, xm); }
			else if(spt <= 2) { said("k_estimate_prod<2,4>"); k_estimate_prod<2, 4><<<egl, 256, 0, b->stream>>>(EST_ARGS, order, xm); }
			else if(spt <= 4) { said("k_estimate_prod<4,4>"); k_estimate_prod<4, 4><<<egl, 256, 0, b->stream>>>(EST_ARGS, order, xm); }
			else if(spt <= 6) { said("k_estimate_prod<6,4,4>"); k_estimate_prod<6, 4, 4><<<egl, 256, (size_t)(b->knob.est_lds_pad > 0 && b->knob.est_lds_pad <= 60 ? b->knob.est_lds_pad : 0) * 1024, b->stream>>>(EST_ARGS, order, xm); }
			else if(spt <= 8) { said("k_estimate_prod<8,4>"); k_estimate_prod<8, 4><<<egl, 256, 0, b->stream>>>(EST_ARGS, order, xm); }
			else if(var == 4) { said("k_estimate_prod<12,4>"); k_estimate_prod<12, 4><<<egl, 256, 0, b->stream>>>(EST_ARGS, order, xm); }
			else { said("k_estimate_prod<6,8,2>"); k_estimate_prod<6, 8, 2><<<egl, 512, 0, b->stream>>>(EST_ARGS, order, xm); }
			#undef EST_ARGS
		}
	}
	HIPCHK(hipGetLastError());
	if(n) {
		if((rc = b->dPermCnt.ensure(n * 2)) != HU_OK) return rc;
		k_site_count<<<b->n, 64, 0, b->stream>>>(b->db->dev, b->n, b->dCodes.p, b->dStart.p, b->dEnd.p, b->dPermCnt.p);
		HIPCHK(hipGetLastError());
	}
	b->state = ST_ESTIMATED;
	return HU_OK;
} catch(...) { return hu_catch_all("hu_estimate_batch"); }


static int sync_host_cands(hu_batch* b) {
	if(b->hostCands) return HU_OK;
	const size_t n = (size_t) b->n;
	std::vector<int32_t> off(n + 1, 0);
	b->places.resize(b->nc);
	HIPCHK(hipSetDevice(b->db->device));
	if(n) HIPCHK(hipMemcpyAsync(off.data(), b->dCandOff.p, (n + 1) * 4, hipMemcpyDeviceToHost, b->stream));
	if(b->nc) HIPCHK(hipMemcpyAsync(b->places.data(), b->dPlaces.p, b->nc * sizeof(HuPlaceRec), hipMemcpyDeviceToHost, b->stream));
	HIPCHK(hu_wait(b->stream));
	b->candOffs.assign(off.begin(), off.end());
	b->hostCands = true;
	return HU_OK;
}
static int scan_cands(hu_batch* b, bool withPerm) {
	int rc;
	if((rc = b->dCandOff.ensure((size_t) b->n + 1)) != HU_OK || (rc = b->dMeta.ensure(4)) != HU_OK) return rc;
	k_cand_scan<<<1, 1024, 0, b->stream>>>(b->n, b->dCandCnt.p, b->dCandOff.p, withPerm ? b->dPermCnt.p : nullptr, b->dStart.p, b->dEnd.p, b->dMeta.p, b->rMain);
	HIPCHK(hipGetLastError());
	b->hMeta.assign(4, 0);
	int32_t* meta = b->hMeta.data();
	HIPCHK(hipMemcpyAsync(meta, b->dMeta.p, 12, hipMemcpyDeviceToHost, b->stream));
	if(b->rMain) { b->hCandOffAll.resize((size_t) b->n + 1); HIPCHK(hipMemcpyAsync(b->hCandOffAll.data(), b->dCandOff.p, ((size_t) b->n + 1) * 4, hipMemcpyDeviceToHost, b->stream)); }
	HIPCHK(hu_wait(b->stream));
	b->nc = (size_t) meta[0]; b->maxGapSites = meta[1]; b->maxBaseSites = meta[2];
	return HU_OK;
}

extern "C" int hu_filter_batch(hu_batch* b, const hu_opts* o) try {
	if(!b || !o) return HU_ERR_ARG;
	if(b->state < ST_ESTIMATED) { hu_set_error("hu_filter_batch: no estimates"); return HU_ERR_STATE; }
	if(!(o->max_error >= 0)) { hu_set_error("max_error must be >= 0"); return HU_ERR_ARG; }
	HIPCHK(hipSetDevice(b->db->device));
	const size_t n = (size_t) b->n;
	if(b->knob.inject_fault == 1) parallel_for(std::max<size_t>(n, 600), [&](size_t r) { if(r + 1 == std::max<size_t>(n, 600)) throw std::bad_alloc(); });
	int rc;
	if((rc = b->dCandCnt.ensure(std::max<size_t>(n, 1))) != HU_OK || (rc = b->dFiltSlot.ensure(std::max<size_t>(n, 1) * HU_MAX_SEEDS)) != HU_OK) return rc;
	(void) hipGetLastError();
	b->nc = 0; b->maxGapSites = b->maxBaseSites = 0;
	if(n) {
		k_filter<<<(unsigned)((n + 3) / 4), 256, 0, b->stream>>>(b->n, b->dSeedCnt.p, b->dEst.p, o->max_error, b->dCandCnt.p, b->dFiltSlot.p, b->knob.sort_seq);
		HIPCHK(hipGetLastError());
		if((rc = scan_cands(b, true)) != HU_OK) return rc;
		if((rc = b->dCands.ensure(std::max<size_t>(b->nc, 1))) != HU_OK || (rc = b->dPlaces.ensure(std::max<size_t>(b->nc, 1))) != HU_OK) return rc;
		k_build_cands<<<(unsigned)((n * HU_MAX_SEEDS + 255) / 256), 256, 0, b->stream>>>(b->db->dev, b->n, b->dCandCnt.p, b->dCandOff.p, b->dFiltSlot.p, b->dSeedId.p, b->dEst.p, b->dCands.p, b->dPlaces.p);
		HIPCHK(hipGetLastError());
	}
	b->hostCands = false; b->placesGiven = false;
	b->state = ST_FILTERED;
	return HU_OK;
} catch(...) { return hu_catch_all("hu_filter_batch"); }

extern "C" int hu_batch_set_candidates(hu_batch* b, const int64_t* offs, const hu_place_rec* recs, int placed) try {
	if(!b || !offs) { hu_set_error("hu_batch_set_candidates: null argument"); return HU_ERR_ARG; }
	if(b->state < ST_ALIGNED) { hu_set_error("hu_batch_set_candidates: reads are not aligned"); return HU_ERR_STATE; }
	const hu_db* db = b->db;
	const size_t n = (size_t) b->n;
	if(offs[0] != 0) { hu_set_error("hu_batch_set_candidates: offs[0] must be 0"); return HU_ERR_ARG; }
	for(size_t r = 0; r < n; ++r) {
		const int64_t k = offs[r + 1] - offs[r];
		if(k < 0 || k > HU_MAX_SEEDS || (k > 0 && (!recs || b->hAlns[r].status != HU_READ_OK || b->hEnd[r] < b->hStart[r]))) {
			hu_set_error("hu_batch_set_candidates: read %zu: %lld candidates (0..%d, none for a read that is not placed)", r, (long long) k, HU_MAX_SEEDS); return HU_ERR_ARG;
		}
		for(int64_t c = offs[r]; c < offs[r + 1]; ++c) {
			const int32_t u = recs[c].c_node;
			if(u < 0 || u >= db->dev.nNodes || db->parent[u] < 0) { hu_set_error("hu_batch_set_candidates: read %zu names node %d (a branch is named by its child end: a non-root node)", r, u); return HU_ERR_ARG; }
		}
	}
	HIPCHK(hipSetDevice(db->device));
	b->candOffs.assign(offs, offs + n + 1);
	const size_t nc = (size_t) offs[n];
	b->places.resize(nc); b->hCands.resize(nc);
	std::vector<int32_t> hCnt(std::max<size_t>(n, 1), 0);
	for(size_t r = 0; r < n; ++r) hCnt[r] = (int32_t)(offs[r + 1] - offs[r]);
	for(size_t r = 0; r < n; ++r) for(int64_t c = offs[r]; c < offs[r + 1]; ++c) {
		const hu_place_rec& q = recs[c];
		HostPlace p;
		memset(&p, 0, sizeof(p));
		p.seedIdx = (int32_t)(c - offs[r]); p.cNode = q.c_node; p.pNode = db->parent[q.c_node]; p.wuv = db->blen[q.c_node];
		p.ratio = q.ratio; p.wnr = q.wnr; p.estLoglik = q.est_loglik; p.rootLoglik = NAN; p.qPlace = p.qTaxon = NAN;
		if(placed) { p.loglik = q.loglik; p.height = q.height; p.aNode = q.a_node == p.pNode ? p.pNode : p.cNode; p.rootLoglik = q.root_loglik; }
		else { p.loglik = q.est_loglik; p.aNode = p.ratio <= 0.5 ? p.cNode : p.pNode; }
		b->places[c] = p;
		HuCand cd; cd.read = (int32_t) r; cd.node = p.cNode; cd.ratio0 = p.ratio; cd.wnr0 = p.wnr;
		b->hCands[c] = cd;
	}
	{
		int rc;
		if((rc = b->dCandCnt.ensure(std::max<size_t>(n, 1))) != HU_OK || (rc = b->dCands.ensure(std::max<size_t>(nc, 1))) != HU_OK ||
				(rc = b->dPlaces.ensure(std::max<size_t>(nc, 1))) != HU_OK || (rc = b->dPermCnt.ensure(std::max<size_t>(n, 1) * 2)) != HU_OK) return rc;
		(void) hipGetLastError();
		if(n) {
			HIPCHK(hipMemcpyAsync(b->dCandCnt.p, hCnt.data(), n * 4, hipMemcpyHostToDevice, b->stream));
			if(nc) {
				HIPCHK(hipMemcpyAsync(b->dCands.p, b->hCands.data(), nc * sizeof(HuCand), hipMemcpyHostToDevice, b->stream));
				HIPCHK(hipMemcpyAsync(b->dPlaces.p, b->places.data(), nc * sizeof(HuPlaceRec), hipMemcpyHostToDevice, b->stream));
			}
			k_site_count<<<b->n, 64, 0, b->stream>>>(db->dev, b->n, b->dCodes.p, b->dStart.p, b->dEnd.p, b->dPermCnt.p);
			HIPCHK(hipGetLastError());
			plan_width_split(b);
			if((rc = scan_cands(b, true)) != HU_OK) return rc;
		}
		else { b->nc = 0; b->maxGapSites = b->maxBaseSites = 0; }
	}
	b->hostCands = true;
	b->placesGiven = placed != 0;
	b->fixedRoot = false;
	b->state = placed ? ST_PLACED : ST_FILTERED;
	return HU_OK;
} catch(...) { return hu_catch_all("hu_batch_set_candidates"); }

__global__ void k_cand_sortkeys(int nc, const HuCand* __restrict__ cands, uint32_t* __restrict__ key, uint32_t* __restrict__ val) {
	const int i = blockIdx.x * 256 + threadIdx.x;
	if(i >= nc) return;
	key[i] = (uint32_t) cands[i].node; val[i] = (uint32_t) i;
}

extern "C" int hu_place_batch(hu_batch* b, const hu_opts* o) try {
	if(!b || !o) return HU_ERR_ARG;
	if(b->state < ST_FILTERED) { hu_set_error("hu_place_batch: candidates are not filtered"); return HU_ERR_STATE; }
	HIPCHK(hipSetDevice(b->db->device));
	const size_t nc = b->nc;
	int rc;
	if((rc = b->dPlaceOut.ensure(std::max<size_t>(nc, 1))) != HU_OK) return rc;
	(void) hipGetLastError();
	if(nc) {
		Timer t(b, HU_T_PLACE);
		int passes = 1;
		if(b->rMain) {
			b->hWideCand.clear();
			if(b->hCandOffAll.size() < (size_t) b->n + 1) { hu_set_error("hu_place_batch: candidate offsets of the wide reads are missing"); return HU_ERR_STATE; }
			for(int r : b->wideReads) for(int32_t c = b->hCandOffAll[r]; c < b->hCandOffAll[r + 1]; ++c) b->hWideCand.push_back((uint32_t) c);
			if(!b->hWideCand.empty()) {
				if((rc = b->dWideCand.ensure(b->hWideCand.size())) != HU_OK) return rc;
				HIPCHK(hipMemcpyAsync(b->dWideCand.p, b->hWideCand.data(), b->hWideCand.size() * 4, hipMemcpyHostToDevice, b->stream));
				passes = 2;
			}
		}
		for(int pass = 0; pass < passes; ++pass) {
			const int maxR = pass ? b->maxAll : b->maxMain;
			const HuDbDev dev = width_pass_dev(b, pass, b->dWideCand.p);
			const unsigned grid = pass ? (unsigned) b->hWideCand.size() : (unsigned) nc;
			const int spt2 = (maxR + 127) / 128, spt4 = (maxR + 255) / 256;
			const bool stream = b->knob.streaming_sep != 0 || spt4 > 12;
			#define PL_ARGS dev, b->db->mdl, b->dCodes.p, b->dStart.p, b->dEnd.p, b->dCands.p, b->dPlaceOut.p
			auto said = [&](int S, int NW, bool split, const char* text) {
				if(!b->knob.trace) return;
				char k[96]; size_t kn = 0;
				for(const char* c = text; *c && kn + 1 < sizeof(k); ++c) if(*c != ' ') k[kn++] = *c;
				k[kn] = 0;
				if(!S) fprintf(stderr, "[hu] place: %zu candidates, max region %d, sites streamed per sweep, column order, one wave per candidate, %s\n", nc, maxR, k);
				else fprintf(stderr, "[hu] place: %zu candidates, max region %d, %d sites per thread, %s, %s, %s\n", nc, maxR, S, split ? "gap/base split slots" : "column order",
						NW == 2 ? "EM across both waves" : "EM across four waves", k);
			};
			if(stream) {
				const size_t lds = (size_t)(3 * HU_MAX_DGK * 4 + HU_MAX_DGK * 5 * 4 + maxR) * sizeof(double);
				if(lds > 160 * 1024) { hu_set_error("alignment region of %d columns does not fit the placement kernel's LDS", maxR); return HU_ERR_ARG; }
				if(lds > 64 * 1024) HIPCHK(hipFuncSetAttribute((const void*) k_place, hipFuncAttributeMaxDynamicSharedMemorySize, (int) lds));
				said(0, 1, false, "k_place");
				k_place<<<grid, 64, lds, b->stream>>>(PL_ARGS);
			}
			else {
				const int var = b->knob.place_var;
				const int xm = b->knob.xcd_map;
				const uint32_t* order = nullptr;
				if(pass) order = b->dWideCand.p;
				else if(!b->knob.place_unsorted) {
					if((rc = b->dSortK.ensure(nc * 2)) != HU_OK || (rc = b->dSortV.ensure(nc * 2)) != HU_OK) return rc;
					k_cand_sortkeys<<<(unsigned)((nc + 255) / 256), 256, 0, b->stream>>>((int) nc, b->dCands.p, b->dSortK.p, b->dSortV.p);
					if((rc = order_by_key(b, b->dSortK.p, b->dSortV.p, nc, (uint32_t) b->db->dev.nNodes, b->dSortV.p + nc, false)) != HU_OK) return rc;
					order = b->dSortV.p + nc;
				}
				#define PL_RUN(SPLIT, LDS, DD, PERM, PCNT, S, NW, ...) do { said(S, NW, SPLIT, "k_place_blk<" #S "," #NW "," #__VA_ARGS__ ">"); \
					k_place_blk<S, NW, __VA_ARGS__><<<grid, 64 * NW, LDS, b->stream>>>(PL_ARGS, DD, order, PERM, PCNT, xm); } while(0)
				#define PL_GO(S, NW, E, R, O) PL_RUN(false, 0, nullptr, nullptr, nullptr, S, NW, E, R, O)
				const bool split8 = spt2 > 4 && spt2 <= 8 && !pass && !b->knob.place_nosplit && b->maxGapSites <= 6 * 128 && b->maxBaseSites <= 2 * 128;
				if((var == 99 || var == 98) && spt4 <= 6) {
					DBuf<long long> ddb;
					if((rc = ddb.ensure(nc * 12)) != HU_OK) return rc;
					long long* dd = ddb.p;
					HIPCHK(hipMemsetAsync(dd, 0, nc * 12 * sizeof(long long), b->stream));
					const bool split98 = var == 98 && !pass && !b->knob.place_nosplit && spt2 > 8 && b->maxGapSites <= 10 * 128 && b->maxBaseSites <= 2 * 128;
					if(var == 99) { said(6, 4, false, "k_place_blk<6,4,3,0,1,true>"); k_place_blk<6, 4, 3, 0, 1, true><<<grid, 256, 0, b->stream>>>(PL_ARGS, dd); }
					else if(split98) {
						if((rc = b->dPerm.ensure((size_t) b->n * 12 * 128)) != HU_OK) return rc;
						k_site_perm<<<b->n, 64, 0, b->stream>>>(dev, b->n, b->dCodes.p, b->dStart.p, b->dEnd.p, 10 * 128, 2 * 128, b->dPerm.p);
						PL_RUN(true, 0, dd, b->dPerm.p, b->dPermCnt.p, 12, 2, 3, 0, 2, true, 1, 10);
					}
					else PL_RUN(false, 0, dd, nullptr, nullptr, 12, 2, 3, 0, 2, true, 1);
					std::vector<long long> hd(nc * 12);
					HIPCHK(hipMemcpyAsync(hd.data(), dd, nc * 12 * sizeof(long long), hipMemcpyDeviceToHost, b->stream));
					HIPCHK(hu_wait(b->stream));
					double acc[8] = {0}, ae[4] = {0};
					for(size_t c = 0; c < nc; ++c) { for(int i = 0; i < 8; ++i) acc[i] += (double) hd[c * 8 + i]; for(int i = 0; i < 4; ++i) ae[i] += (double) hd[nc * 8 + c * 4 + i]; }
					fprintf(stderr, "[place dbg] %s, per candidate (s_memtime ticks): load %.0f tables %.0f sweeps %.0f em %.0f total %.0f | outer %.2f em steps %.2f\n",
							var == 99 ? "4 waves x 6 sites" : split98 ? "2 waves x 12 sites, gap/base split slots" : "2 waves x 12 sites, column order",
							acc[0] / nc, acc[1] / nc, acc[2] / nc, acc[3] / nc, acc[4] / nc, acc[5] / nc, acc[6] / nc);
					fprintf(stderr, "[place dbg] inside the EM steps, per step: arithmetic %.0f wave reduction %.0f exchange between the waves %.0f tail %.0f\n",
							ae[0] / acc[6], ae[1] / acc[6], ae[2] / acc[6], ae[3] / acc[6]);
				}
				else if(var == 4 && spt4 <= 6) PL_GO(6, 4, 1, 0, 1);
				else if(var == 5 && spt4 <= 6) PL_GO(6, 4, 2, 1, 1);
				else if(var == 6 && spt2 <= 12 && !split8) PL_GO(12, 2, 1, 0, 2);
				else if(spt2 <= 4) PL_GO(4, 2, 3, 0, 2);
				else if(spt2 <= 12 && !(var == 7)) {
					const int S = spt2 <= 8 ? 8 : 12, G = S - 2;
					const bool split = S == 8 ? split8 : !pass && !b->knob.place_nosplit && b->maxGapSites <= G * 128 && b->maxBaseSites <= (S - G) * 128;
					if(split) {
						if((rc = b->dPerm.ensure((size_t) b->n * S * 128)) != HU_OK) return rc;
						k_site_perm<<<b->n, 64, 0, b->stream>>>(dev, b->n, b->dCodes.p, b->dStart.p, b->dEnd.p, G * 128, (S - G) * 128, b->dPerm.p);
						if(S == 8 && var != 6) PL_RUN(true, 3 * 8 * 128 * sizeof(double), nullptr, b->dPerm.p, b->dPermCnt.p, 8, 2, 3, 0, 3, false, 3, 6);
						else if(S == 8) PL_RUN(true, 0, nullptr, b->dPerm.p, b->dPermCnt.p, 8, 2, 3, 0, 2, false, 0, 6);
						else PL_RUN(true, (size_t)(b->knob.place_lds_pad > 0 && b->knob.place_lds_pad <= 44 ? b->knob.place_lds_pad : 0) * 1024, nullptr, b->dPerm.p, b->dPermCnt.p, 12, 2, 3, 0, 2, false, 1, 10);
					}
					else if(S == 8) PL_GO(8, 2, 3, 0, 2);
					else PL_RUN(false, 0, nullptr, nullptr, nullptr, 12, 2, 3, 0, 2, false, 1);
				}
				else if(var == 7 && spt2 <= 12) PL_GO(12, 2, 3, 0, 2);
				else if(spt4 <= 8) PL_GO(8, 4, 3, 0, 1);
				else if(var == 9) PL_GO(12, 4, 3, 0, 1);
				else PL_RUN(false, 0, nullptr, nullptr, nullptr, 12, 4, 3, 0, 2, false, 1);
				#undef PL_GO
				#undef PL_RUN
			}
			#undef PL_ARGS
		}
		HIPCHK(hipGetLastError());
		if(o->fix_root_loglik) {
			if((rc = b->dRootLL.ensure(nc)) != HU_OK) return rc;
			k_root_loglik<<<(unsigned) nc, 64, 0, b->stream>>>(b->db->dev, b->db->mdl, b->dCodes.p, b->dStart.p, b->dEnd.p, b->dCands.p, b->dPlaceOut.p, (int) nc, b->dRootLL.p);
			HIPCHK(hipGetLastError());
		}
	}
	b->fixedRoot = o->fix_root_loglik != 0 && nc > 0;
	b->placesGiven = false;
	b->state = ST_PLACED;
	return HU_OK;
} catch(...) { return hu_catch_all("hu_place_batch"); }


static int hu_alleq_table(int device) {
	static std::mutex mu; static bool done[64] = {false};
	std::lock_guard<std::mutex> lk(mu);
	if(device < 0 || device >= 64) { hu_set_error("device %d out of range", device); return HU_ERR_ARG; }
	if(done[device]) return HU_OK;
	(void) hipGetLastError();
	k_alleq_init<<<1, 128>>>();
	HIPCHK(hipGetLastError());
	HIPCHK(hipDeviceSynchronize());
	done[device] = true;
	return HU_OK;
}

extern "C" int hu_finish_batch(hu_batch* b, const hu_opts* o) try {
	if(!b || !o) return HU_ERR_ARG;
	if(b->state < ST_PLACED) { hu_set_error("hu_finish_batch: candidates are not placed"); return HU_ERR_STATE; }
	const hu_db* db = b->db;
	const size_t n = (size_t) b->n;
	if(b->knob.inject_fault == 2) throw std::length_error("injected");
	HIPCHK(hipSetDevice(db->device));
	b->best.assign(n, hu_place_rec());
	int rc;
	if((rc = b->dBest.ensure(std::max<size_t>(n, 1))) != HU_OK) return rc;
	(void) hipGetLastError();
	if(n) {
		if((rc = hu_alleq_table(db->device)) != HU_OK) return rc;
		k_finish<<<(unsigned)((n + 63) / 64), 64, 0, b->stream>>>(db->dev, b->n, b->dStart.p, b->dEnd.p, b->dCandOff.p, b->dPlaces.p, b->dPlaceOut.p,
				b->fixedRoot ? b->dRootLL.p : nullptr, db->dLlTab, db->dAnnoId, o->max_height, o->only_ml, o->prior, b->placesGiven ? 1 : 0, b->dBest.p, b->knob.sort_seq);
		HIPCHK(hipGetLastError());
		HIPCHK(hipMemcpyAsync(b->best.data(), b->dBest.p, n * sizeof(hu_place_rec), hipMemcpyDeviceToHost, b->stream));
		HIPCHK(hu_wait(b->stream));
	}
	b->hostCands = false;
	b->state = ST_FINISHED;
	return HU_OK;
} catch(...) { return hu_catch_all("hu_finish_batch"); }

extern "C" int hu_assign_batch(hu_batch* b, const hu_opts* o) try {
	int rc;
	if(!b || !o) return HU_ERR_ARG;
	auto now = [] { return std::chrono::steady_clock::now(); };
	auto ms = [](std::chrono::steady_clock::time_point a, std::chrono::steady_clock::time_point c) { return std::chrono::duration<double, std::milli>(c - a).count(); };
	auto t0 = now();
	if(!b->fromCodes && (rc = hu_align_batch(b, o)) != HU_OK) return rc;
	auto t1 = now();
	if((rc = hu_seed_batch(b, o)) != HU_OK) return rc;
	if((rc = hu_estimate_batch(b, o)) != HU_OK) return rc;
	if((rc = hu_filter_batch(b, o)) != HU_OK) return rc;
	auto t2 = now();
	if((rc = hu_place_batch(b, o)) != HU_OK) return rc;
// ... 912 lines not shown
```

hmmufotu_amd/csrc/hu_kern_blk.h:

```cpp
#pragma once
#include "hu_kern_sep.h"

#define HU_BLK_THREADS 256

__device__ inline void lds_wave_sync() { asm volatile("s_waitcnt lgkmcnt(0)" ::: "memory"); }
__device__ inline void lds_barrier() { asm volatile("s_waitcnt lgkmcnt(0)\n\ts_barrier" ::: "memory"); }

template<int NW = 4>
__device__ inline double block_sum(double v, double* red, int& phase) {
	v = wave_sum_uniform(v);
	double* r = red + (phase & 1) * NW;
	if((threadIdx.x & 63) == 0) r[threadIdx.x >> 6] = v;
	lds_barrier();
	double s = r[0];
#pragma unroll
	for(int w = 1; w < NW; ++w) s += r[w];
	phase ^= 1;
	return s;
}
template<int NW = 4>
__device__ inline long long block_sum_ll(long long v, long long* red, int& phase) {
	for(int m = 32; m > 0; m >>= 1) v += __shfl_xor(v, m);
	long long* r = red + (phase & 1) * NW;
	if((threadIdx.x & 63) == 0) r[threadIdx.x >> 6] = v;
	lds_barrier();
	long long s = r[0];
#pragma unroll
	for(int w = 1; w < NW; ++w) s += r[w];
	phase ^= 1;
	return s;
}

template<int SPT, int THREADS>
__global__ __launch_bounds__(THREADS) void k_estimate_blk(HuDbDev db, HuModelDev mdl, const int8_t* __restrict__ codes,
		const int32_t* __restrict__ rstart, const int32_t* __restrict__ rend, const uint32_t* __restrict__ parDN,
		const int32_t* __restrict__ seedCnt, const int32_t* __restrict__ seedId, const uint32_t* __restrict__ seedDN,
		int weighted, HuEstOut* __restrict__ out) {
	__shared__ double red[2 * THREADS / 64];
	__shared__ long long redl[2 * THREADS / 64];
	constexpr int NW = THREADS / 64;
	const uint32_t slot = db.wideList ? db.wideList[blockIdx.x] : blockIdx.x;
	const int read = slot / HU_MAX_SEEDS, s = slot % HU_MAX_SEEDS, tid = threadIdx.x;
	if(s >= seedCnt[read] || hu_skip_width(db, rend[read] - rstart[read] + 1)) return;
	const int u = seedId[(size_t) read * HU_MAX_SEEDS + s];
	const int v = db.parent[u];
	const uint32_t dn = seedDN[(size_t) read * HU_MAX_SEEDS + s];
	const uint32_t pv = parDN[(size_t) read * HU_MAX_SEEDS + s];
	const double cDist = (double)(dn >> 16) / (double)(dn & 0xffffu);
	const double pDist = (double)(pv >> 16) / (double)(pv & 0xffffu);
	double ratio = cDist / (cDist + pDist);
	if(isnan(ratio)) ratio = 0.5;
	const double w0 = db.blen[u];
	const double wur = w0 * ratio, wvr = w0 - wur;
	double Eu[4], Ev[4];
#pragma unroll
	for(int k = 0; k < 4; ++k) { Eu[k] = exp(mdl.lam[k] * wur); Ev[k] = exp(mdl.lam[k] * wvr); }
	const int start = rstart[read], end = rend[read], n = end - start + 1;
	const int8_t* __restrict__ cd = codes + (size_t) read * db.csLen + start;
	const int64_t sOff = (int64_t) u * db.winLen + (start - db.winStart);
	const int piMax = argmax4d(mdl.logpi);
	double piw[4];
	{ double mx = max4d(mdl.logpi), sm; for(int i = 0; i < 4; ++i) piw[i] = exp(mdl.logpi[i] - mx); sm = (piw[0] + piw[2]) + (piw[1] + piw[3]); for(int i = 0; i < 4; ++i) piw[i] /= sm; }
	double z[SPT][4]; int bb[SPT]; long long ksum = 0;
	{
		double eU[SPT][4], eV[SPT][4];
#pragma unroll
		for(int t = 0; t < SPT; ++t) {
			const int j = tid + THREADS * t;
			const int jj = j < n ? j : 0;
			load4(db.up + (sOff + jj) * 4, eU[t]); load4(db.down + (sOff + jj) * 4, eV[t]);
			bb[t] = cd[jj];
			if(j < n) ksum += (long long) db.upK[sOff + jj] + (long long) db.downK[sOff + jj];
		}
#pragma unroll
		for(int t = 0; t < SPT; ++t) {
			double c[4];
			conv_eig(mdl, Eu, eU[t], z[t]);
			conv_eig(mdl, Ev, eV[t], c);
			for(int i = 0; i < 4; ++i) z[t][i] *= c[i];
		}
	}
	int phase = 0;
	double dsum = 0, nsum = 0;
#pragma unroll
	for(int t = 0; t < SPT; ++t) {
		if(tid + THREADS * t >= n) continue;
		const int b = bb[t];
		const int b1 = argmax4_tied_lin(z[t]), b2 = b >= 0 ? b : piMax;
		if(!weighted) { if(b1 != b2) dsum += 1; }
		else {
			const double w1 = sel4(z[t], b1) / ((z[t][0] + z[t][2]) + (z[t][1] + z[t][3]));
			const double w2 = b >= 0 ? 1.0 : piw[b2];
			if(b1 != b2) dsum += w1 * w2;
			nsum += w1 * w2;
		}
	}
	dsum = block_sum<NW>(dsum, red, phase);
	double wnr;
	if(!weighted) wnr = dsum / (double) n;
	else { nsum = block_sum<NW>(nsum, red, phase); wnr = dsum / nsum; }
	double En[4], Ppi[4];
#pragma unroll
	for(int k = 0; k < 4; ++k) En[k] = exp(mdl.lam[k] * wnr);
	{ double a[4]; to_eig(mdl, mdl.pi, a); if(wnr == 0) { for(int i = 0; i < 4; ++i) Ppi[i] = mdl.pi[i]; } else conv_eig(mdl, En, a, Ppi); }
	double ll = 0;
#pragma unroll
	for(int t = 0; t < SPT; ++t) {
		if(tid + THREADS * t >= n) continue;
		const int b = bb[t];
		double c[4];
		if(b >= 0) {
			if(wnr == 0) { for(int i = 0; i < 4; ++i) c[i] = i == b ? 1.0 : 0.0; }
			else { double a[4]; for(int k = 0; k < 4; ++k) a[k] = mdl.U1[k*4+b]; conv_eig(mdl, En, a, c); }
		}
		else for(int i = 0; i < 4; ++i) c[i] = Ppi[i];
		ll += log((mdl.pi[0] * z[t][0] * c[0] + mdl.pi[2] * z[t][2] * c[2]) + (mdl.pi[1] * z[t][1] * c[1] + mdl.pi[3] * z[t][3] * c[3]));
	}
	ll = block_sum<NW>(ll, red, phase);
	int lphase = 0;
	const long long kt = block_sum_ll<NW>(ksum, redl, lphase);
	ll += (double) kt * HU_LN2;
	if(tid == 0) { HuEstOut o; o.ratio = ratio; o.wnr = wnr; o.loglik = ll; out[(size_t) read * HU_MAX_SEEDS + s] = o; }
}

template<int CTRL>
__device__ inline double dpp_mul_full(double v) {
	const int lo = __builtin_amdgcn_mov_dpp(__double2loint(v), CTRL, 0xf, 0xf, true);
	const int hi = __builtin_amdgcn_mov_dpp(__double2hiint(v), CTRL, 0xf, 0xf, true);
	return v * __hiloint2double(hi, lo);
}
__device__ inline double wave_prod(double v) {
	v = dpp_mul_full<0xB1>(v);
	v = dpp_mul_full<0x4E>(v);
	v = dpp_mul_full<0x141>(v);
	v = dpp_mul_full<0x140>(v);
	v *= __shfl_xor(v, 16);
	v *= __shfl_xor(v, 32);
	return v;
}
__device__ inline int wave_sum_i32(int v) {
	for(int m = 32; m > 0; m >>= 1) v += __shfl_xor(v, m);
	return v;
}

__device__ inline uint32_t hu_xcd_pos(uint32_t b, uint32_t nb, int xmap) {
	if(!xmap) return b;
	const uint32_t per = nb >> 3;
	return b < per * 8 ? (b & 7u) * per + (b >> 3) : b;
}

__host__ __device__ constexpr int hu_est_waves(int spt, int occ) {
	const int w = spt <= 2 ? 8 : spt <= 4 ? 5 : spt <= 6 ? 4 : spt <= 8 ? 3 : 2;
	return occ > w ? occ : w;
}
template<int SPT, int NW, int OCC = 1, bool DBG = false>
__global__ __launch_bounds__(64 * NW, hu_est_waves(SPT, OCC)) void k_estimate_prod(HuDbDev db, HuModelDev mdl, const int8_t* __restrict__ codes,
		const int32_t* __restrict__ rstart, const int32_t* __restrict__ rend, const uint32_t* __restrict__ parDN,
		const int32_t* __restrict__ seedCnt, const int32_t* __restrict__ seedId, const uint32_t* __restrict__ seedDN,
		int weighted, HuEstOut* __restrict__ out, const uint32_t* __restrict__ order, int xmap = 0, long long* __restrict__ dbg = nullptr) {
	constexpr int THREADS = 64 * NW;
	long long tk[4] = {0, 0, 0, 0}, t0 = 0, tl = 0;
	auto stamp = [&](int i) { if(DBG) { const long long t = (long long) __builtin_amdgcn_s_memtime(); tk[i] += t - tl; tl = t; } };
	if(DBG) { t0 = tl = (long long) __builtin_amdgcn_s_memtime(); }
	__shared__ double redd[2 * NW];
	__shared__ int redi[2 * NW];
	__shared__ __attribute__((aligned(16))) double Qtab[24];
	__shared__ __attribute__((aligned(16))) double pro[12];
	__shared__ __attribute__((aligned(16))) double mtab[36];
	const uint32_t slot = order ? order[hu_xcd_pos(blockIdx.x, gridDim.x, xmap)] : blockIdx.x;
	const int read = slot / HU_MAX_SEEDS, s = slot % HU_MAX_SEEDS, tid = threadIdx.x, lane = tid & 63;
	const int wave = __builtin_amdgcn_readfirstlane(tid >> 6);
	const bool builder = wave == (int)(blockIdx.x % NW);
	if(s >= seedCnt[read] || hu_skip_width(db, rend[read] - rstart[read] + 1)) return;
	const int un = seedId[(size_t) read * HU_MAX_SEEDS + s];
	double ratio = 0;
	if(builder) {
		static_assert(offsetof(HuModelDev, U) == offsetof(HuModelDev, pi) + 64 && offsetof(HuModelDev, U1) == offsetof(HuModelDev, pi) + 192, "pi, logpi, U, U1 in a row");
		const double* __restrict__ mp = reinterpret_cast<const double*>(reinterpret_cast<const char*>(&mdl) + offsetof(HuModelDev, pi));
		const int l36 = lane < 36 ? lane : 0;
		const double mc = mp[l36 < 4 ? l36 : l36 + 4];
		const uint32_t dn = seedDN[(size_t) read * HU_MAX_SEEDS + s];
		const uint32_t pv = parDN[(size_t) read * HU_MAX_SEEDS + s];
		const double cDist = (double)(dn >> 16) / (double)(dn & 0xffffu);
		const double pDist = (double)(pv >> 16) / (double)(pv & 0xffffu);
		ratio = cDist / (cDist + pDist);
		if(isnan(ratio)) ratio = 0.5;
		ratio = __hiloint2double(__builtin_amdgcn_readfirstlane(__double2hiint(ratio)), __builtin_amdgcn_readfirstlane(__double2loint(ratio)));
		const double w0 = db.blen[un];
		const double wur = w0 * ratio, wvr = w0 - wur;
		const int l6 = lane < 6 ? lane : 0, m3 = l6 % 3;
		const double e = exp((m3 == 0 ? mdl.lam[1] : m3 == 1 ? mdl.lam[2] : mdl.lam[3]) * (l6 < 3 ? wur : wvr));
		if(lane < 6) pro[lane] = e;
		if(weighted) {
			double piw[4];
			{ double mx = max4d(mdl.logpi), sm; for(int i = 0; i < 4; ++i) piw[i] = exp(mdl.logpi[i] - mx); sm = (piw[0] + piw[2]) + (piw[1] + piw[3]); for(int i = 0; i < 4; ++i) piw[i] /= sm; }
			if(lane < 4) pro[8 + lane] = sel4(piw, lane);
		}
		if(lane < 36) mtab[lane] = mc;
	}
	const int start = rstart[read], end = rend[read], n = end - start + 1;
	const int8_t* __restrict__ cd = codes + (size_t) read * db.csLen + start;
	const int64_t sOff = (int64_t) un * db.winLen + (start - db.winStart);
	const int piMax = argmax4d(mdl.logpi);
	double z[SPT][4]; unsigned long long bop = 0; int ksum = 0;
	double Eu[3], Ev[3];
	double aU[SPT][4], aV[SPT][4];
	const double* __restrict__ Ub = db.up + sOff * 4; const double* __restrict__ Vb = db.down + sOff * 4;
	const int32_t* __restrict__ upKb = db.upK + sOff; const int32_t* __restrict__ downKb = db.downK + sOff;
	auto inr = [&](int t) { return tid < n - THREADS * t; };
	stamp(0);
	{
		int kU[SPT], kV[SPT];
#pragma unroll
		for(int t = 0; t < SPT; ++t) {
			const int jj = inr(t) ? tid + THREADS * t : 0;
			kU[t] = upKb[(size_t) jj]; kV[t] = downKb[(size_t) jj];
		}
		__builtin_amdgcn_sched_barrier(0);
#pragma unroll
		for(int t = 0; t < SPT; ++t) {
			const int jj = inr(t) ? tid + THREADS * t : 0;
			load4(Ub + (size_t) jj * 4, aU[t]); load4(Vb + (size_t) jj * 4, aV[t]);
			const int b = cd[jj];
			bop |= (unsigned long long)(b >= 0 ? b : 4) << (3 * t);
		}
		__builtin_amdgcn_sched_barrier(0);
		lds_barrier();
		{
			const double e = pro[lane < 6 ? lane : 0];
			const int lo = __double2loint(e), hi = __double2hiint(e);
#pragma unroll
			for(int k = 0; k < 3; ++k) {
				Eu[k] = __hiloint2double(__builtin_amdgcn_readlane(hi, k), __builtin_amdgcn_readlane(lo, k));
				Ev[k] = __hiloint2double(__builtin_amdgcn_readlane(hi, 3 + k), __builtin_amdgcn_readlane(lo, 3 + k));
			}
		}
#pragma unroll
		for(int t = 0; t < SPT; ++t) {
			asm volatile("" : "+v"(kU[t]), "+v"(kV[t]));
			ksum += inr(t) ? kU[t] + kV[t] : 0;
		}
	}
	if(DBG) { double x = 0; for(int t = 0; t < SPT; ++t) x += aU[t][0] + aV[t][0]; if(x == 1.2345e-300 || bop == ~0ull) tk[2] = 1; }
	stamp(1);
	{
#pragma unroll
		for(int t = 0; t < SPT; ++t) {
			const double su1 = Eu[0] * aU[t][1], su2 = Eu[1] * aU[t][2], su3 = Eu[2] * aU[t][3];
			const double sv1 = Ev[0] * aV[t][1], sv2 = Ev[1] * aV[t][2], sv3 = Ev[2] * aV[t][3];
#pragma unroll
			for(int i = 0; i < 4; ++i) {
				const double cu = fmax(fma(mdl.U[i*4+3], su3, fma(mdl.U[i*4+2], su2, fma(mdl.U[i*4+1], su1, aU[t][0]))), 0.0);
				const double cv = fmax(fma(mdl.U[i*4+3], sv3, fma(mdl.U[i*4+2], sv2, fma(mdl.U[i*4+1], sv1, aV[t][0]))), 0.0);
				z[t][i] = cu * cv;
			}
		}
	}
	double wnr = 0;
	if(!weighted) {
		int nd = 0;
#pragma unroll
		for(int t = 0; t < SPT; ++t) {
			const int bi = (int)((bop >> (3 * t)) & 7u);
			const int b1 = argmax4_tied_lin(z[t]), b2 = bi < 4 ? bi : piMax;
			nd += __popcll(__ballot(inr(t) && b1 != b2));
		}
		if(lane == 0) redi[wave] = nd;
		lds_barrier();
		if(builder) {
			int tot = redi[0];
#pragma unroll
			for(int w = 1; w < NW; ++w) tot += redi[w];
			wnr = (double) tot / (double) n;
		}
	}
	else {
		const double piwGap = pro[8 + piMax];
		double dsum = 0, nsum = 0;
#pragma unroll
		for(int t = 0; t < SPT; ++t) {
			if(!inr(t)) continue;
			const int bi = (int)((bop >> (3 * t)) & 7u);
			const int b1 = argmax4_tied_lin(z[t]), b2 = bi < 4 ? bi : piMax;
			const double w1 = sel4(z[t], b1) / ((z[t][0] + z[t][2]) + (z[t][1] + z[t][3]));
			const double w2 = bi < 4 ? 1.0 : piwGap;
			if(b1 != b2) dsum += w1 * w2;
			nsum += w1 * w2;
		}
		dsum = wave_sum(dsum); nsum = wave_sum(nsum);
		if(lane == 0) { redd[wave] = dsum; redd[NW + wave] = nsum; }
		lds_barrier();
		if(builder) {
			double a = redd[0], c = redd[NW];
#pragma unroll
			for(int w = 1; w < NW; ++w) { a += redd[w]; c += redd[NW + w]; }
			wnr = a / c;
		}
	}
	double* Q = Qtab;
	if(builder) {
		if(lane < 3) Q[1 + lane] = exp((lane == 0 ? mdl.lam[1] : lane == 1 ? mdl.lam[2] : mdl.lam[3]) * wnr);
		lds_wave_sync();
		if(lane < 20) {
			const int b = lane >> 2, i = lane & 3;
			const double* mU = mtab + 4 + i * 4, * mU1 = mtab + 20 + (b & 3);
			const double pii = mtab[i];
			double c;
			if(wnr == 0) c = b < 4 ? (i == b ? 1.0 : 0.0) : pii;
			else {
				double a0, a1, a2, a3;
				if(b < 4) { a0 = mU1[0]; a1 = mU1[4]; a2 = mU1[8]; a3 = mU1[12]; }
				else {
					a0 = (mdl.U1[0] * mdl.pi[0] + mdl.U1[1] * mdl.pi[1]) + (mdl.U1[2] * mdl.pi[2] + mdl.U1[3] * mdl.pi[3]);
					a1 = (mdl.U1[4] * mdl.pi[0] + mdl.U1[5] * mdl.pi[1]) + (mdl.U1[6] * mdl.pi[2] + mdl.U1[7] * mdl.pi[3]);
					a2 = (mdl.U1[8] * mdl.pi[0] + mdl.U1[9] * mdl.pi[1]) + (mdl.U1[10] * mdl.pi[2] + mdl.U1[11] * mdl.pi[3]);
					a3 = (mdl.U1[12] * mdl.pi[0] + mdl.U1[13] * mdl.pi[1]) + (mdl.U1[14] * mdl.pi[2] + mdl.U1[15] * mdl.pi[3]);
				}
				const double Ui1 = mU[1], Ui2 = mU[2], Ui3 = mU[3];
				c = fmax(fma(Ui3, Q[3] * a3, fma(Ui2, Q[2] * a2, fma(Ui1, Q[1] * a1, a0))), 0.0);
			}
			Q[4 + b * 4 + i] = pii * c;
		}
	}
	lds_barrier();
	double mant = 1.0; int esum = ksum;
#pragma unroll
	for(int t = 0; t < SPT; ++t) {
		const double* q = Q + 4 + ((bop >> (3 * t)) & 7u) * 4;
		double x = fmax(fma(q[3], z[t][3], fma(q[2], z[t][2], fma(q[1], z[t][1], q[0] * z[t][0]))), 0.0);
		if(!inr(t)) x = 1.0;
		mant *= __builtin_amdgcn_frexp_mant(x);
		esum += x == 0.0 ? 0 : __builtin_amdgcn_frexp_exp(x);
	}
	esum += __builtin_amdgcn_frexp_exp(mant); mant = __builtin_amdgcn_frexp_mant(mant);
	mant = wave_prod(mant);
	esum = wave_sum_i32(esum);
	if(lane == 0) { redd[wave] = mant; redi[NW + wave] = esum; }
	lds_barrier();
	if(builder && lane == 0) {
		double m = redd[0]; long long e = redi[NW];
#pragma unroll
		for(int w = 1; w < NW; ++w) { m *= redd[w]; e += redi[NW + w]; }
		HuEstOut o; o.ratio = ratio; o.wnr = wnr; o.loglik = log(m) + (double) e * HU_LN2;
		out[(size_t) read * HU_MAX_SEEDS + s] = o;
	}
	if(DBG) {
		stamp(2);
		if(builder && lane == 0) { tk[3] = tl - t0; for(int i = 0; i < 4; ++i) dbg[(size_t) blockIdx.x * 4 + i] = tk[i]; }
	}
}

#define HU_RHO_SKIP 1e60
#define HU_TP 18
#define HU_EXP_MEPS 0.99999000004999983333
#define HU_EXP_PEPS 1.00001000005000016667

__device__ inline double fast_div(double a, double b) {
	double y = __builtin_amdgcn_rcp(b);
	y = fma(fma(-b, y, 1.0), y, y);
	y = fma(fma(-b, y, 1.0), y, y);
	const double q = a * y;
	return fma(fma(-b, q, a), y, q);
}

__device__ __attribute__((noinline)) double hu_exp_call(double x) { return exp(x); }
__device__ __attribute__((noinline)) double hu_log_call(double x) { return log(x); }

template<int SPT, int NW, int EMV, int RED>
__device__ inline double em_branch_blk(const double (&rho)[SPT], int nvalidWave, double q0, double maxL,
		double* red, double* redc, int& phase, int& emIters, long long* st = nullptr) {
	long long tl = st ? (long long) __builtin_amdgcn_s_memtime() : 0;
	auto stamp = [&](int i) { if(st) { const long long t = (long long) __builtin_amdgcn_s_memtime(); st[i] += t - tl; tl = t; } };
	const int lane = threadIdx.x & 63, wave = threadIdx.x >> 6;
	double p0 = 1 - q0, p = p0, q = q0, rc = 0;
	const int em0 = emIters;
	if(lane == 0) redc[(phase & 1) * NW + wave] = (double) nvalidWave;
	for(int it = 0; it < HU_MAX_ITER && p >= 0 && p <= 1; ++it) {
		double s = 0;
		const bool fast = q0 >= 1e-30 && p0 >= 1e-30;
		if(fast) {
			if(EMV == 3 && SPT % 4 == 0) {
				constexpr int G = SPT / 4;
				double x[SPT], ab[G], cd[G], X[G], nm[G], y[G], w[G];
#pragma unroll
				for(int t = 0; t < SPT; ++t) x[t] = fma(rho[t], q0, p0);
				__builtin_amdgcn_sched_barrier(0);
#pragma unroll
				for(int g = 0; g < G; ++g) { ab[g] = x[4 * g] * x[4 * g + 1]; cd[g] = x[4 * g + 2] * x[4 * g + 3]; }
#pragma unroll
				for(int g = 0; g < G; ++g) { X[g] = ab[g] * cd[g]; x[4 * g] += x[4 * g + 1]; x[4 * g + 2] += x[4 * g + 3]; }
				__builtin_amdgcn_sched_barrier(0);
#pragma unroll
				for(int g = 0; g < G; ++g) { y[g] = __builtin_amdgcn_rcp(X[g]); nm[g] = x[4 * g + 2] * ab[g]; }
#pragma unroll
				for(int g = 0; g < G; ++g) nm[g] = fma(x[4 * g], cd[g], nm[g]);
				__builtin_amdgcn_sched_barrier(0);
#pragma unroll
				for(int g = 0; g < G; ++g) { w[g] = fma(-X[g], y[g], 2.0); nm[g] *= y[g]; }
				__builtin_amdgcn_sched_barrier(0);
#pragma unroll
				for(int g = 0; g < G; ++g) s = fma(nm[g], w[g], s);
			}
			else if(EMV == 4 && SPT % 2 == 0) {
#pragma unroll
				for(int t = 0; t < SPT; t += 2) {
					const double a = fma(rho[t], q0, p0), bb = fma(rho[t + 1], q0, p0);
					const double x = a * bb, y = __builtin_amdgcn_rcp(x);
					s = fma((a + bb) * y, fma(-x, y, 2.0), s);
				}
			}
			else {
#pragma unroll
				for(int t = 0; t < SPT; ++t) {
					const double x = fma(rho[t], q0, p0);
					const double y = __builtin_amdgcn_rcp(x);
					if(EMV == 1 || EMV == 3 || EMV == 4) s = fma(y, fma(-x, y, 2.0), s);
					else { const double y1 = fma(fma(-x, y, 1.0), y, y); s = fma(y1, fma(-x, y1, 2.0), s); }
				}
			}
		}
		else {
#pragma unroll
			for(int t = 0; t < SPT; ++t) {
				const double r = rho[t];
				const double tt = p0 / fma(r, q0, p0);
				s += r == HU_RHO_SKIP ? 0.0 : tt;
			}
		}
		if(st) { if(s == 1.2345e-300) st[7] = 1; }
		stamp(0);
		s = wave_sum_uniform(s);
		stamp(1);
		double* r = red + (phase & 1) * NW;
		if(lane == 0) r[wave] = s;
		lds_barrier();
		s = r[0];
#pragma unroll
		for(int w = 1; w < NW; ++w) s += r[w];
		if(it == 0) {
			const double* c = redc + (phase & 1) * NW;
			double cnt = c[0];
#pragma unroll
			for(int w = 1; w < NW; ++w) cnt += c[w];
			rc = 1.0 / cnt;
		}
		phase ^= 1;
		if(st) { if(s == 1.2345e-300) st[7] = 1; }
		stamp(2);
		if(fast) s *= p0;
		p = s * rc; q = 1 - p;
		++emIters;
		if(q0 * HU_EXP_MEPS < q && q < q0 * HU_EXP_PEPS) { stamp(3); break; }
		p0 = p; q0 = q;
		stamp(3);
	}
	double w = -hu_log_call(q);
	if(w > maxL) w = maxL;
	if(q < 0) { w = maxL; emIters = em0 + HU_MAX_ITER; }
	return w;
}

__global__ __launch_bounds__(64) void k_site_count(HuDbDev db, int n, const int8_t* __restrict__ codes, const int32_t* __restrict__ rstart,
		const int32_t* __restrict__ rend, int32_t* __restrict__ cnt) {
	const int read = blockIdx.x, lane = threadIdx.x;
	const int start = rstart[read], len = rend[read] - start + 1;
	int g = 0, bc = 0;
	for(int j0 = 0; j0 < len; j0 += 64) {
		const int j = j0 + lane;
		const bool val = j < len;
		const int b = val ? codes[(size_t) read * db.csLen + start + j] : 0;
		g += __popcll(__ballot(val && b < 0)); bc += __popcll(__ballot(val && b >= 0));
	}
	if(lane == 0) { cnt[2 * read] = g; cnt[2 * read + 1] = bc; }
}
__global__ __launch_bounds__(64) void k_site_perm(HuDbDev db, int n, const int8_t* __restrict__ codes, const int32_t* __restrict__ rstart,
		const int32_t* __restrict__ rend, int gapCap, int baseCap, uint16_t* __restrict__ perm) {
	const int read = blockIdx.x, lane = threadIdx.x;
	const int start = rstart[read], len = rend[read] - start + 1;
	if(hu_skip_width(db, len)) return;
	uint16_t* __restrict__ pr = perm + (size_t) read * (gapCap + baseCap);
	const unsigned long long lt = (1ull << lane) - 1ull;
	int g = 0, bc = 0;
	for(int j0 = 0; j0 < len; j0 += 64) {
		const int j = j0 + lane;
		const bool val = j < len;
		const int b = val ? codes[(size_t) read * db.csLen + start + j] : 0;
		const unsigned long long mg = __ballot(val && b < 0), mb = __ballot(val && b >= 0);
		if(val && b < 0) { const int at = g + __popcll(mg & lt); if(at < gapCap) pr[at] = (uint16_t) j; }
		if(val && b >= 0) { const int at = bc + __popcll(mb & lt); if(at < baseCap) pr[gapCap + at] = (uint16_t) j; }
		g += __popcll(mg); bc += __popcll(mb);
	}
}

__device__ __forceinline__ double hu_gtab_entry(const double* a, const double* b, int Kc) {
	double g = 0;
	if(Kc == 4) {
		const double a0 = a[0], a1 = a[4], a2 = a[8], a3 = a[12], b0 = b[0], b1 = b[4], b2 = b[8], b3 = b[12];
		g += a0 * b0; g += a1 * b1; g += a2 * b2; g += a3 * b3;
	}
	else if(Kc == 1) g += a[0] * b[0];
	else for(int k = 0; k < Kc; ++k) g += a[k * 4] * b[k * 4];
	return g;
}

template<int SPT, int NW, int EMV, int RED, int OCC, bool DBG = false, int VL = 0, int GS = 0>
__global__ __launch_bounds__(64 * NW, OCC) void k_place_blk(HuDbDev db, HuModelDev mdl, const int8_t* __restrict__ codes,
		const int32_t* __restrict__ rstart, const int32_t* __restrict__ rend,
		const HuCand* __restrict__ cands, HuPlaceOut* __restrict__ out, long long* __restrict__ dbg = nullptr, const uint32_t* __restrict__ order = nullptr,
		const uint16_t* __restrict__ perm = nullptr, const int32_t* __restrict__ permCnt = nullptr, int xmap = 0) {
	constexpr int THREADS = 64 * NW;
	long long tk[8] = {0, 0, 0, 0, 0, 0, 0, 0}, t0 = 0, tl = 0;
	long long te[8] = {0, 0, 0, 0, 0, 0, 0, 0};
	auto stamp = [&](int slot) { if(DBG) { const long long t = (long long) __builtin_amdgcn_s_memtime(); tk[slot] += t - tl; tl = t; } };
	if(DBG) { t0 = tl = (long long) __builtin_amdgcn_s_memtime(); }
	__shared__ double red[2 * NW], redc[2 * NW];
	__shared__ double cst[HU_PC_COUNT];
	__shared__ double Etab[3 * HU_MAX_DGK * 4];
	__shared__ double Gtab[16];
	__shared__ __attribute__((aligned(16))) double tabM[5 * HU_TP];
	__shared__ __attribute__((aligned(16))) double tabD[6 * 4];
	__shared__ double q0s[2];
	__shared__ double vl[VL == 1 ? SPT * 64 * NW : 1];
	extern __shared__ double vdyn[];
	const int tid = threadIdx.x;
	const int vt = (tid + 64 * (blockIdx.x % NW)) % THREADS;
	const uint32_t ci = order ? order[hu_xcd_pos(blockIdx.x, gridDim.x, xmap)] : blockIdx.x;
	const HuCand cd = cands[ci];
	const int read = cd.read, un = cd.node;
	const int start = rstart[read], end = rend[read], n = end - start + 1;
	if(hu_skip_width(db, n)) return;
	const int Kc = mdl.dgK > 0 ? mdl.dgK : 1;
	const double rKc = 1.0 / (double) Kc;
	const int8_t* __restrict__ cdr = codes + (size_t) read * db.csLen + start;
	const int64_t mOff = ((int64_t) un * db.winLen + (start - db.winStart)) * 4;
	const double* __restrict__ Ub = db.up + mOff;
	const double* __restrict__ Vb = db.down + mOff;
	const int nGap = GS > 0 ? permCnt[2 * read] : 0, nBase = GS > 0 ? permCnt[2 * read + 1] : 0;
	double u[SPT][3], v[SPT][3]; unsigned long long bop = 0, bop2 = 0;
	{
		double aU[SPT][4], aV[SPT][4];
		int js[SPT];
#pragma unroll
		for(int t = 0; t < SPT; ++t) {
			if(GS > 0) {
				const int i = t < GS ? tid + THREADS * t : tid + THREADS * (t - GS);
				const bool val = i < (t < GS ? nGap : nBase);
				const int e = (int) perm[(size_t) read * (SPT * THREADS) + (t < GS ? 0 : GS * THREADS) + (val ? i : 0)];
				js[t] = val ? e : 0;
			}
			else { const int j = tid + THREADS * t; js[t] = j < n ? j : 0; }
		}
#pragma unroll
		for(int t = 0; t < SPT; ++t) {
			const int jj = js[t];
			load4(Ub + (size_t) jj * 4, aU[t]); load4(Vb + (size_t) jj * 4, aV[t]);
			const int b = cdr[jj];
			if(t < 21) bop |= (unsigned long long)(b >= 0 ? b : 4) << (3 * t);
			else bop2 |= (unsigned long long)(b >= 0 ? b : 4) << (3 * (t - 21));
		}
		__builtin_amdgcn_sched_barrier(0);
#pragma unroll
		for(int t = 0; t < SPT; ++t) {
			const double iu = 1.0 / aU[t][0], iv = 1.0 / aV[t][0];
#pragma unroll
			for(int m = 0; m < 3; ++m) { u[t][m] = aU[t][m + 1] * iu; v[t][m] = aV[t][m + 1] * iv; }
			if(VL == 1) { vl[t * THREADS + tid] = v[t][2]; v[t][2] = 0; }
			if(VL == 3) {
#pragma unroll
				for(int m = 0; m < 3; ++m) { vdyn[(m * SPT + t) * THREADS + tid] = v[t][m]; v[t][m] = 0; }
			}
		}
	}
	for(int i = tid; i < HU_PC_COUNT; i += THREADS) cst[i] = db.placeConst[i];
	lds_barrier();
	const double* clam = cst + HU_PC_LAM; const double* crate = cst + HU_PC_RATE; const double* cW = cst + HU_PC_W;
	const double* cC = cst + HU_PC_C; const double* ccb = cst + HU_PC_CB;
	const double w0 = db.blen[un];
	double lenUR = w0 * cd.ratio0, lenVR = w0 * (1 - cd.ratio0), lenNR = cd.wnr0;
	double wur0 = lenUR, wnr0 = lenNR;
	const double w0j = lenUR + lenVR;
	double wur = wur0, wnr = wnr0;
	int iter = 0, emIters = 0, phase = 0;
	double rho[SPT];
	auto build_exp = [&](int wh0, int nE, double len0, double len1, double w, double* q0p) __attribute__((always_inline)) {
		for(int e = vt; e <= nE; e += THREADS) {
			const bool second = e >= 4 * Kc;
			const int wh = wh0 + (second ? 1 : 0), k = (e >> 2) % Kc, m = e & 3;
			const double len = second ? len1 : len0;
			const double x = hu_exp_call(e == nE ? -w : clam[m] * (len * crate[k]));
			if(e == nE) *q0p = x;
			else Etab[(wh * HU_MAX_DGK + k) * 4 + m] = x;
		}
		lds_barrier();
	};
	if(DBG) { double x = 0; for(int t = 0; t < SPT; ++t) x += u[t][0] + u[t][1]; if(x == 1.2345e-300) tk[7] = 1; }
	stamp(0);
	for(; iter < HU_MAX_ITER && 0 <= wur && wur <= w0j; ++iter) {
		build_exp(0, 8 * Kc, lenUR, lenVR, lenNR, q0s);
		if(vt < 16)
			Gtab[vt] = hu_gtab_entry(Etab + (vt >> 2), Etab + HU_MAX_DGK * 4 + (vt & 3), Kc) * rKc;
		lds_barrier();
		for(int e = vt; e < 84; e += THREADS) {
			if(e < 80) tabM[(e >> 4) * HU_TP + (e & 15)] = cW[e] * Gtab[e & 15];
			else tabD[e - 80] = Gtab[(e - 80) * 5];
		}
		lds_barrier();
		const double q0n = q0s[0];
		stamp(1);
		int nv = 0;
		{
			unsigned long long bq = bop, bq2 = bop2;
			asm volatile("" : "+v"(bq), "+v"(bq2));
			const double g0 = tabD[0], g1 = tabD[1], g2 = tabD[2], g3 = tabD[3];
			double Mg[GS > 0 ? 16 : 1];
			if(GS > 0) {
#pragma unroll
				for(int e = 0; e < 16; ++e) Mg[e] = tabM[4 * HU_TP + e];
			}
#pragma unroll
			for(int t = 0; t < SPT; ++t) {
				const double* M = (GS > 0 && t < GS) ? Mg : tabM + (unsigned)(((t < 21 ? bq >> (3 * t) : bq2 >> (3 * (t - 21)))) & 7u) * HU_TP;
				const double v0 = VL == 3 ? vdyn[(0 * SPT + t) * THREADS + tid] : v[t][0], v1 = VL == 3 ? vdyn[(1 * SPT + t) * THREADS + tid] : v[t][1];
				const double v2 = VL == 3 ? vdyn[(2 * SPT + t) * THREADS + tid] : VL == 1 ? vl[t * THREADS + tid] : v[t][2];
				double num = fma(M[3], v2, fma(M[2], v1, fma(M[1], v0, M[0])));
#pragma unroll
				for(int m = 1; m < 4; ++m) {
					const double tm = fma(M[m * 4 + 3], v2, fma(M[m * 4 + 2], v1, fma(M[m * 4 + 1], v0, M[m * 4 + 0])));
					num = fma(tm, u[t][m - 1], num);
				}
				const double den = fma(g3 * u[t][2], v2, fma(g2 * u[t][1], v1, fma(g1 * u[t][0], v0, g0)));
				const double r = fast_div(num, den);
				const bool inr = GS > 0 ? (t < GS ? tid + THREADS * t < nGap : tid + THREADS * (t - GS) < nBase) : tid + THREADS * t < n;
				const bool ok = inr && fabs(r) < HU_RHO_SKIP;
				rho[t] = ok ? r : HU_RHO_SKIP;
				nv += __popcll(__ballot(ok));
			}
		}
		stamp(2);
		wnr = em_branch_blk<SPT, NW, EMV, RED>(rho, nv, q0n, 1.0, red, redc, phase, emIters, DBG ? te : nullptr);
		lenNR = wnr;
		stamp(3);
		build_exp(2, 4 * Kc, lenNR, lenNR, lenUR, q0s + 1);
		if(vt < 16)
			Gtab[vt] = hu_gtab_entry(Etab + HU_MAX_DGK * 4 + (vt >> 2), Etab + 2 * HU_MAX_DGK * 4 + (vt & 3), Kc) * rKc;
		lds_barrier();
		for(int e = vt; e < 100; e += THREADS) {
			if(e < 80) {
				const int b = e >> 4, m = (e >> 2) & 3, kk = e & 3;
				double z = 0;
#pragma unroll
				for(int nn = 0; nn < 4; ++nn) z = fma(ccb[b * 4 + nn] * Gtab[m * 4 + nn], cC[(m * 4 + nn) * 4 + kk], z);
				tabM[b * HU_TP + m * 4 + kk] = z;
			}
			else { const int b = (e - 80) >> 2, m = (e - 80) & 3; tabD[b * 4 + m] = ccb[b * 4 + m] * Gtab[m * 5]; }
		}
		lds_barrier();
		const double q0u = q0s[1];
		stamp(1);
		nv = 0;
		{
			unsigned long long bq = bop, bq2 = bop2;
			asm volatile("" : "+v"(bq), "+v"(bq2));
			double Mg[GS > 0 ? 16 : 1], Dg[GS > 0 ? 4 : 1];
			if(GS > 0) {
#pragma unroll
				for(int e = 0; e < 16; ++e) Mg[e] = tabM[4 * HU_TP + e];
#pragma unroll
				for(int e = 0; e < 4; ++e) Dg[e] = tabD[4 * 4 + e];
			}
// ... 38 lines not shown
```

profiles/est_isa_count.py:

```python
import argparse
import re
import sys

NAMES = {
    "<2,4>": "ILi2ELi4ELi1ELb0EE", "<4,4>": "ILi4ELi4ELi1ELb0EE", "<6,4,4,false>": "ILi6ELi4ELi4ELb0EE", "<6,4,4,true>": "ILi6ELi4ELi4ELb1EE",
    "<6,4,1>": "ILi6ELi4ELi1ELb0EE", "<8,4>": "ILi8ELi4ELi1ELb0EE", "<12,4>": "ILi12ELi4ELi1ELb0EE", "<12,2>": "ILi12ELi2ELi1ELb0EE",
    "<6,8,2>": "ILi6ELi8ELi2ELb0EE",
}


def kernel_lines(path, inst):
    txt = open(path).read().split("\n")
    pref = "_Z15k_estimate_prod" + NAMES[inst]
    a = next(i for i, l in enumerate(txt) if l.startswith(pref) and l.split(";")[0].rstrip().endswith(":"))
    b = next(i for i in range(a, len(txt)) if txt[i].startswith(".Lfunc_end"))
    out = []
    for i in range(a + 1, b):
        l = txt[i].split(";")[0].strip()
        if l and not l.startswith(".") or re.match(r"\.LBB\d+_\d+:", l):
            out.append((i + 1, l))
    return out


def kind(op):
    if op.startswith("v_"):
        return "valu"
    if op.startswith("ds_"):
        return "lds"
    if op.startswith(("global_", "scratch_", "buffer_", "flat_")):
        return "vmem"
    if op.startswith("s_"):
        return "salu"
    return None


def exec_written(L, i):
    j = i - 1
    while j >= 0 and not L[j][1].endswith(":") and not L[j][1].startswith(("s_cbranch", "s_branch")):
        if re.search(r"saveexec|\bexec\b", L[j][1].split(",")[0]):
            return True
        j -= 1
    return False


def barrier_sets(L):
    lab = {l[:-1]: i for i, (_, l) in enumerate(L) if l.endswith(":")}
    arrive = [set() for _ in L]
    arrive[0].add(0)
    ends = {}
    work = [0]
    while work:
        i = work.pop()
        _, l = L[i]
        op = l.split()[0]
        cnt = {c + (op == "s_barrier") for c in arrive[i]}
        nxt = []
        if op == "s_endpgm":
            continue
        if op == "s_branch":
            nxt = [lab[l.split()[1]]]
        elif op.startswith("s_cbranch_exec") and not exec_written(L, i):
            nxt = [lab[l.split()[1]] if op == "s_cbranch_execnz" else i + 1]
        elif op.startswith("s_cbranch"):
            nxt = [lab[l.split()[1]], i + 1]
        else:
            nxt = [i + 1]
        for j in nxt:
            if L[j][1].split()[0] == "s_endpgm" or (L[j][1].endswith(":") and L[j + 1][1] == "s_endpgm"):
                ends.setdefault(L[i][0], set()).update(cnt)
            if not cnt <= arrive[j]:
                arrive[j] |= cnt
                work.append(j)
    return ends


def walk(L, uniform, idle):
    lab = {l[:-1]: i for i, (_, l) in enumerate(L) if l.endswith(":")}
    seg = dict(valu=0, lds=0, vmem=0, salu=0)
    segs, marks, notes = [], ["entry"], []
    i, nu, ne, seen_load, nbar = 0, 0, 0, False, 0

    def close(mark):
        nonlocal seg
        segs.append(seg)
        marks.append(mark)
        seg = dict(valu=0, lds=0, vmem=0, salu=0)

    while True:
        ln, l = L[i]
        if l.endswith(":"):
            i += 1
            continue
        op = l.split()[0]
        if op == "global_load_dword" and not seen_load:
            seen_load = True
            close("first message load (line %d)" % ln)
        if op.startswith("global_load") and nbar >= 1:
            notes.append("line %d: %s behind barrier %d" % (ln, l, nbar))
        k = kind(op)
        if k:
            seg[k] += 1
        if op == "s_barrier":
            nbar += 1
            close("barrier %d (line %d)" % (nbar, ln))
        if op == "s_endpgm":
            close("s_endpgm (line %d)" % ln)
            return segs, marks, notes, nbar
        if op == "s_branch":
            i = lab[l.split()[1]]
            continue
        if op.startswith("s_cbranch_exec"):
            active = ne not in idle
            taken = (op == "s_cbranch_execnz") == active
            print("  exec branch %2d, line %d: %-34s lanes %s" % (ne, ln, l, "active" if active else "idle"))
            ne += 1
            i = lab[l.split()[1]] if taken else i + 1
            continue
        if op.startswith("s_cbranch"):
            if nu >= len(uniform):
                sys.exit("uniform branch %d at line %d (%s): no letter left in --uniform" % (nu, ln, l))
            taken = uniform[nu] == "T"
            print("  uniform branch %2d, line %d: %-31s %s" % (nu, ln, l, "taken" if taken else "not taken"))
            nu += 1
            i = lab[l.split()[1]] if taken else i + 1
            continue
        i += 1


def main():
    ap = argparse.ArgumentParser()
    ap.add_argument("listing")
    ap.add_argument("--kernel", default="<6,4,4,false>", choices=sorted(NAMES))
    ap.add_argument("--uniform", default="")
    ap.add_argument("--idle", default="")
    a = ap.parse_args()
    L = kernel_lines(a.listing, a.kernel)
    ends = barrier_sets(L)
    allc = set().union(*ends.values())
    print("k_estimate_prod%s: barrier counts at s_endpgm over all paths: %s" % (a.kernel, sorted(allc)))
    for ln, c in sorted(ends.items()):
        print("  edge into s_endpgm from line %d: %s" % (ln, sorted(c)))
    if a.uniform or a.idle:
        idle = {int(x) for x in a.idle.split(",") if x}
        segs, marks, notes, nbar = walk(L, a.uniform, idle)
        tot = dict(valu=0, lds=0, vmem=0, salu=0)
        for s, m0, m1 in zip(segs, marks, marks[1:]):
            print("%-36s -> %-36s VALU %4d  LDS %3d  VMEM %3d  scalar %4d" % (m0, m1, s["valu"], s["lds"], s["vmem"], s["salu"]))
            for k in tot:
                tot[k] += s[k]
        print("path: %d barriers, vector instructions %d (VALU %d, LDS %d, VMEM %d), scalar %d" %
              (nbar, tot["valu"] + tot["lds"] + tot["vmem"], tot["valu"], tot["lds"], tot["vmem"], tot["salu"]))
        for n in notes:
            print("  NOTE", n)


if __name__ == "__main__":
    main()
```

Measured before the change: 430,800.

## Run estimate kernel as persistent workgroups pulling seed slots from atomic tickets

Replaces the one-workgroup-per-seed-slot launch of k_estimate_prod with a grid sized to resident occupancy. Each workgroup loops, drawing slots from per-XCD atomic ticket counters. A scout wave prefetches and decodes the next slot's metadata (read, seed, ratio, branch-length exponentials) into double-buffered LDS while the current slot is being computed. The aim is to cut launch and workgroup-startup overhead and hide prologue load latency. In exchange the kernel carries extra loop-carried state, ticket atomics and barriers, and more register pressure.

```diff
diff --git a/hmmufotu_amd/csrc/hu_engine.hip b/hmmufotu_amd/csrc/hu_engine.hip
--- a/hmmufotu_amd/csrc/hu_engine.hip
+++ b/hmmufotu_amd/csrc/hu_engine.hip
@@ -4,6 +4,7 @@
 #include <cstring>
 #include <limits>
 #include <map>
+#include <tuple>
 #include <atomic>
 #include <thread>
 #include <memory>
@@ -1656,6 +1657,7 @@
 	int trace = 0;
 	int width_split = 1;
 	int sort_seq = 0;
+	int est_wgs = 0;
 	int refsort_wgs = HU_RS_WGS_PER_CU * 256;
 	int ref_nofuse = 0;
 	int refsort_host = 0;
@@ -1668,7 +1670,7 @@
 	{"pairs32", &HuKnobs::pairs32}, {"tile_unsorted", &HuKnobs::tile_unsorted}, {"topk_fast_min", &HuKnobs::topk_fast_min}, {"scan_pairs", &HuKnobs::scan_pairs}, {"topk_general", &HuKnobs::topk_general}, {"streaming_sep", &HuKnobs::streaming_sep},
 	{"est_unsorted", &HuKnobs::est_unsorted}, {"place_unsorted", &HuKnobs::place_unsorted}, {"xcd_map", &HuKnobs::xcd_map},
 	{"est_var", &HuKnobs::est_var}, {"place_var", &HuKnobs::place_var}, {"place_nosplit", &HuKnobs::place_nosplit}, {"width_split", &HuKnobs::width_split},
-	{"place_lds_pad", &HuKnobs::place_lds_pad}, {"est_lds_pad", &HuKnobs::est_lds_pad}, {"vit_lds_pad", &HuKnobs::vit_lds_pad}, {"scan_lds_pad", &HuKnobs::scan_lds_pad}, {"trace", &HuKnobs::trace}, {"inject_fault", &HuKnobs::inject_fault}, {"refsort_host", &HuKnobs::refsort_host}, {"ref_nofuse", &HuKnobs::ref_nofuse}, {"refsort_wgs", &HuKnobs::refsort_wgs}, {"sort_seq", &HuKnobs::sort_seq},
+	{"place_lds_pad", &HuKnobs::place_lds_pad}, {"est_lds_pad", &HuKnobs::est_lds_pad}, {"vit_lds_pad", &HuKnobs::vit_lds_pad}, {"scan_lds_pad", &HuKnobs::scan_lds_pad}, {"trace", &HuKnobs::trace}, {"inject_fault", &HuKnobs::inject_fault}, {"refsort_host", &HuKnobs::refsort_host}, {"ref_nofuse", &HuKnobs::ref_nofuse}, {"refsort_wgs", &HuKnobs::refsort_wgs}, {"est_wgs", &HuKnobs::est_wgs}, {"sort_seq", &HuKnobs::sort_seq},
 };
 static void knobs_from_env(HuKnobs& k) {
 	for(const HuKnobEntry& e : kKnobs) {
@@ -1721,6 +1723,7 @@
 	int refHostAll = 0;
 	DBuf<int32_t> dIns, dTileIns, dRetry;
 	DBuf<uint32_t> dSortK, dSortV;
+	DBuf<uint32_t> dEstTick;
 	DBuf<uint32_t> dCsCnt;
 	DBuf<HuEstOut> dEst;
 	DBuf<HuCand> dCands;
@@ -2726,6 +2729,23 @@
 	return dev;
 }
 
+#define HU_EST_TICKETS 9
+static int resident_workgroups(const void* kern, int threads, size_t lds, int device, int* out) {
+	static std::mutex mu;
+	static std::map<std::tuple<const void*, size_t, int>, int> known;
+	std::lock_guard<std::mutex> g(mu);
+	const auto key = std::make_tuple(kern, lds, device);
+	auto it = known.find(key);
+	if(it == known.end()) {
+		int perCu = 0, cus = 0;
+		HIPCHK(hipOccupancyMaxActiveBlocksPerMultiprocessor(&perCu, kern, threads, lds));
+		HIPCHK(hipDeviceGetAttribute(&cus, hipDeviceAttributeMultiprocessorCount, device));
+		it = known.emplace(key, std::max(1, perCu) * std::max(1, cus)).first;
+	}
+	*out = it->second;
+	return HU_OK;
+}
+
 extern "C" int hu_estimate_batch(hu_batch* b, const hu_opts* o) try {
 	if(!b || !o) return HU_ERR_ARG;
 	if(b->state < ST_SEEDED) { hu_set_error("hu_estimate_batch: no seeds"); return HU_ERR_STATE; }
@@ -2762,6 +2782,23 @@
 			const unsigned egl = pass ? eg : order ? std::min<unsigned>(eg, (unsigned) b->n * (unsigned) b->seedCap) : eg;
 			const int var = b->knob.est_var;
 			auto said = [&](const char* k) { if(b->knob.trace) fprintf(stderr, "[hu] estimate: max region %d, %s\n", maxR, k); };
+			auto walk = [&](auto kern, int threads, size_t lds, long long* dbg) -> int {
+				unsigned G = egl;
+				if(b->knob.est_wgs > 0) G = (unsigned) b->knob.est_wgs;
+				else {
+					int res = 0;
+					const int rcr = resident_workgroups((const void*) kern, threads, lds, b->db->device, &res);
+					if(rcr != HU_OK) return rcr;
+					G = std::min<unsigned>(egl, (unsigned) res);
+				}
+				G = std::max(G, 1u);
+				int rcw;
+				if((rcw = b->dEstTick.ensure(HU_EST_TICKETS)) != HU_OK) return rcw;
+				HIPCHK(hipMemsetAsync(b->dEstTick.p, 0, HU_EST_TICKETS * sizeof(uint32_t), b->stream));
+				if(b->knob.trace) fprintf(stderr, "[hu] estimate walk: %u workgroups take %u slots\n", G, egl);
+				kern<<<G, threads, lds, b->stream>>>(EST_ARGS, order, xm, egl, b->dEstTick.p, dev.blen, dbg);
+				return HU_OK;
+			};
 			if(stream || spt > 12) { said("k_estimate"); k_estimate<<<eg, 64, 0, b->stream>>>(EST_ARGS); }
 			else if(var == 2) {
 				if(spt <= 2) { said("k_estimate_blk<2,256>"); k_estimate_blk<2, 256><<<eg, 256, 0, b->stream>>>(EST_ARGS); }
@@ -2775,7 +2812,7 @@
 				DBuf<long long> ddb;
 				if((rc = ddb.ensure((size_t) egl * 4)) != HU_OK) return rc;
 				HIPCHK(hipMemsetAsync(ddb.p, 0, (size_t) egl * 4 * sizeof(long long), b->stream));
-				k_estimate_prod<6, 4, 4, true><<<egl, 256, 0, b->stream>>>(EST_ARGS, order, xm, ddb.p);
+				if((rc = walk(k_estimate_prod<6, 4, 4, true>, 256, 0, ddb.p)) != HU_OK) return rc;
 				std::vector<long long> hd((size_t) egl * 4);
 				HIPCHK(hipMemcpyAsync(hd.data(), ddb.p, hd.size() * sizeof(long long), hipMemcpyDeviceToHost, b->stream));
 				HIPCHK(hu_wait(b->stream));
@@ -2783,14 +2820,14 @@
 				for(size_t c = 0; c < (size_t) egl; ++c) if(hd[c * 4 + 3]) { ++ran; for(int i = 0; i < 4; ++i) acc[i] += (double) hd[c * 4 + i]; }
 				if(ran) fprintf(stderr, "[est dbg] per slot (s_memtime ticks, %zu slots): prologue %.0f load %.0f rest %.0f total %.0f\n", ran, acc[0] / ran, acc[1] / ran, acc[2] / ran, acc[3] / ran);
 			}
-			else if(var == 1 && spt <= 6) { said("k_estimate_prod<12,2>"); k_estimate_prod<12, 2><<<egl, 128, 0, b->stream>>>(EST_ARGS, order, xm); }
-			else if(var == 3 && spt <= 6) { said("k_estimate_prod<6,4,1>"); k_estimate_prod<6, 4, 1><<<egl, 256, 0, b->stream>>>(EST_ARGS, order, xm); }
-			else if(spt <= 2) { said("k_estimate_prod<2,4>"); k_estimate_prod<2, 4><<<egl, 256, 0, b->stream>>>(EST_ARGS, order, xm); }
-			else if(spt <= 4) { said("k_estimate_prod<4,4>"); k_estimate_prod<4, 4><<<egl, 256, 0, b->stream>>>(EST_ARGS, order, xm); }
-			else if(spt <= 6) { said("k_estimate_prod<6,4,4>"); k_estimate_prod<6, 4, 4><<<egl, 256, (size_t)(b->knob.est_lds_pad > 0 && b->knob.est_lds_pad <= 60 ? b->knob.est_lds_pad : 0) * 1024, b->stream>>>(EST_ARGS, order, xm); }
-			else if(spt <= 8) { said("k_estimate_prod<8,4>"); k_estimate_prod<8, 4><<<egl, 256, 0, b->stream>>>(EST_ARGS, order, xm); }
-			else if(var == 4) { said("k_estimate_prod<12,4>"); k_estimate_prod<12, 4><<<egl, 256, 0, b->stream>>>(EST_ARGS, order, xm); }
-			else { said("k_estimate_prod<6,8,2>"); k_estimate_prod<6, 8, 2><<<egl, 512, 0, b->stream>>>(EST_ARGS, order, xm); }
+			else if(var == 1 && spt <= 6) { said("k_estimate_prod<12,2>"); if((rc = walk(k_estimate_prod<12, 2>, 128, 0, nullptr)) != HU_OK) return rc; }
+			else if(var == 3 && spt <= 6) { said("k_estimate_prod<6,4,1>"); if((rc = walk(k_estimate_prod<6, 4, 1>, 256, 0, nullptr)) != HU_OK) return rc; }
+			else if(spt <= 2) { said("k_estimate_prod<2,4>"); if((rc = walk(k_estimate_prod<2, 4>, 256, 0, nullptr)) != HU_OK) return rc; }
+			else if(spt <= 4) { said("k_estimate_prod<4,4>"); if((rc = walk(k_estimate_prod<4, 4>, 256, 0, nullptr)) != HU_OK) return rc; }
+			else if(spt <= 6) { said("k_estimate_prod<6,4,4>"); if((rc = walk(k_estimate_prod<6, 4, 4>, 256, (size_t)(b->knob.est_lds_pad > 0 && b->knob.est_lds_pad <= 60 ? b->knob.est_lds_pad : 0) * 1024, nullptr)) != HU_OK) return rc; }
+			else if(spt <= 8) { said("k_estimate_prod<8,4>"); if((rc = walk(k_estimate_prod<8, 4>, 256, 0, nullptr)) != HU_OK) return rc; }
+			else if(var == 4) { said("k_estimate_prod<12,4>"); if((rc = walk(k_estimate_prod<12, 4>, 256, 0, nullptr)) != HU_OK) return rc; }
+			else { said("k_estimate_prod<6,8,2>"); if((rc = walk(k_estimate_prod<6, 8, 2>, 512, 0, nullptr)) != HU_OK) return rc; }
 			#undef EST_ARGS
 		}
 	}
diff --git a/hmmufotu_amd/csrc/hu_kern_blk.h b/hmmufotu_amd/csrc/hu_kern_blk.h
--- a/hmmufotu_amd/csrc/hu_kern_blk.h
+++ b/hmmufotu_amd/csrc/hu_kern_blk.h
@@ -143,6 +143,9 @@
 	return v;
 }
 
+__device__ __attribute__((noinline)) double hu_exp_call(double x) { return exp(x); }
+__device__ __attribute__((noinline)) double hu_log_call(double x) { return log(x); }
+
 __device__ inline uint32_t hu_xcd_pos(uint32_t b, uint32_t nb, int xmap) {
 	if(!xmap) return b;
 	const uint32_t per = nb >> 3;
@@ -153,200 +156,271 @@
 	const int w = spt <= 2 ? 8 : spt <= 4 ? 5 : spt <= 6 ? 4 : spt <= 8 ? 3 : 2;
 	return occ > w ? occ : w;
 }
+enum { HU_EST_END = 0, HU_EST_RUN = 1, HU_EST_SKIP = 2 };
 template<int SPT, int NW, int OCC = 1, bool DBG = false>
 __global__ __launch_bounds__(64 * NW, hu_est_waves(SPT, OCC)) void k_estimate_prod(HuDbDev db, HuModelDev mdl, const int8_t* __restrict__ codes,
 		const int32_t* __restrict__ rstart, const int32_t* __restrict__ rend, const uint32_t* __restrict__ parDN,
 		const int32_t* __restrict__ seedCnt, const int32_t* __restrict__ seedId, const uint32_t* __restrict__ seedDN,
-		int weighted, HuEstOut* __restrict__ out, const uint32_t* __restrict__ order, int xmap = 0, long long* __restrict__ dbg = nullptr) {
+		int weighted, HuEstOut* __restrict__ out, const uint32_t* __restrict__ order, int xmap, uint32_t nslots, uint32_t* __restrict__ tick,
+		const double* __restrict__ blen, long long* __restrict__ dbg = nullptr) {
 	constexpr int THREADS = 64 * NW;
 	long long tk[4] = {0, 0, 0, 0}, t0 = 0, tl = 0;
 	auto stamp = [&](int i) { if(DBG) { const long long t = (long long) __builtin_amdgcn_s_memtime(); tk[i] += t - tl; tl = t; } };
 	if(DBG) { t0 = tl = (long long) __builtin_amdgcn_s_memtime(); }
-	__shared__ double redd[2 * NW];
+	__shared__ double redd[NW];
+	__shared__ double redw[2 * NW];
 	__shared__ int redi[2 * NW];
 	__shared__ __attribute__((aligned(16))) double Qtab[24];
-	__shared__ __attribute__((aligned(16))) double pro[12];
+	__shared__ __attribute__((aligned(16))) double pro[2][6];
+	__shared__ __attribute__((aligned(16))) double piw[4];
 	__shared__ __attribute__((aligned(16))) double mtab[36];
-	const uint32_t slot = order ? order[hu_xcd_pos(blockIdx.x, gridDim.x, xmap)] : blockIdx.x;
-	const int read = slot / HU_MAX_SEEDS, s = slot % HU_MAX_SEEDS, tid = threadIdx.x, lane = tid & 63;
+	__shared__ int4 rec[2][3];
+	int tid = threadIdx.x, lane = tid & 63;
 	const int wave = __builtin_amdgcn_readfirstlane(tid >> 6);
-	const bool builder = wave == (int)(blockIdx.x % NW);
-	if(s >= seedCnt[read] || hu_skip_width(db, rend[read] - rstart[read] + 1)) return;
-	const int un = seedId[(size_t) read * HU_MAX_SEEDS + s];
-	double ratio = 0;
+	const bool builder = wave == (int)(blockIdx.x % NW), scout = wave == (int)((blockIdx.x + 1) % NW);
+	int zero = 0;
+	auto M = [&]() __attribute__((always_inline)) -> const HuModelDev& { return *reinterpret_cast<const HuModelDev*>(reinterpret_cast<const char*>(&mdl) + zero); };
+	auto D = [&]() __attribute__((always_inline)) -> const HuDbDev& { return *reinterpret_cast<const HuDbDev*>(reinterpret_cast<const char*>(&db) + zero); };
+	const uint32_t per = xmap ? nslots >> 3 : nslots, nseg = xmap ? 9u : 1u;
+	uint32_t seg = xmap ? blockIdx.x & 7u : 0u, tried = 0;
+	auto draw = [&]() __attribute__((always_inline)) -> uint32_t { uint32_t t = 0; if(lane == 0 && tried < nseg) t = atomicAdd(tick + seg, 1u); return t; };
+	auto settle = [&](uint32_t t) __attribute__((always_inline)) -> uint32_t {
+		for(;;) {
+			t = (uint32_t) __builtin_amdgcn_readfirstlane((int) t);
+			if(tried >= nseg) return ~0u;
+			if(t < (seg < 8u ? per : nslots - 8u * per)) return seg * per + t;
+			if(++tried == nseg) return ~0u;
+			seg = seg + 1u == nseg ? 0u : seg + 1u;
+			t = draw();
+		}
+	};
+	int nState = HU_EST_END, nRead = 0, nS = 0, nUn = 0, nStart = 0, nN = 0;
+	uint32_t nPos = ~0u;
+	auto chain = [&](uint32_t pos) __attribute__((always_inline)) {
+		nPos = pos; nState = HU_EST_END;
+		if(pos != ~0u) {
+			const uint32_t slot = order ? order[pos] : pos;
+			nRead = slot / HU_MAX_SEEDS; nS = slot % HU_MAX_SEEDS;
+			nStart = rstart[nRead]; nN = rend[nRead] - nStart + 1;
+			nState = nS >= seedCnt[nRead] || hu_skip_width(D(), nN) ? HU_EST_SKIP : HU_EST_RUN;
+		}
+		if(nState == HU_EST_RUN) {
+			nUn = seedId[(size_t) nRead * HU_MAX_SEEDS + nS];
+			const uint32_t dn = seedDN[(size_t) nRead * HU_MAX_SEEDS + nS], pv = parDN[(size_t) nRead * HU_MAX_SEEDS + nS];
+			const double w0 = blen[nUn];
+			int touch = (int)(dn ^ pv) ^ __double2loint(w0);
+			asm volatile("" :: "s"(touch));
+		}
+	};
+	auto finish = [&](int p) __attribute__((always_inline)) {
+		double ratio = 0;
+		if(nState == HU_EST_RUN) {
+			int again = 0;
+			asm volatile("" : "+s"(again));
+			const uint32_t dn = seedDN[(size_t) nRead * HU_MAX_SEEDS + nS + again];
+			const uint32_t pv = parDN[(size_t) nRead * HU_MAX_SEEDS + nS + again];
+			const double cDist = (double)(dn >> 16) / (double)(dn & 0xffffu);
+			const double pDist = (double)(pv >> 16) / (double)(pv & 0xffffu);
+			ratio = cDist / (cDist + pDist);
+			if(isnan(ratio)) ratio = 0.5;
+			const double w0 = blen[nUn + again];
+			const double wur = w0 * ratio, wvr = w0 - wur;
+			const int l6 = lane < 6 ? lane : 0, m3 = l6 % 3;
+			const double e = hu_exp_call((m3 == 0 ? M().lam[1] : m3 == 1 ? M().lam[2] : M().lam[3]) * (l6 < 3 ? wur : wvr));
+			if(lane < 6) pro[p][lane] = e;
+		}
+		if(lane == 0) {
+			rec[p][0] = make_int4(nState, nRead, nS, nUn);
+			rec[p][1] = make_int4(nStart, nN, __double2loint(ratio), __double2hiint(ratio));
+			if(DBG) rec[p][2].x = (int) nPos;
+		}
+	};
+	uint32_t tpend = 0;
+	if(scout) { chain(settle(draw())); finish(0); tpend = draw(); }
 	if(builder) {
 		static_assert(offsetof(HuModelDev, U) == offsetof(HuModelDev, pi) + 64 && offsetof(HuModelDev, U1) == offsetof(HuModelDev, pi) + 192, "pi, logpi, U, U1 in a row");
 		const double* __restrict__ mp = reinterpret_cast<const double*>(reinterpret_cast<const char*>(&mdl) + offsetof(HuModelDev, pi));
 		const int l36 = lane < 36 ? lane : 0;
 		const double mc = mp[l36 < 4 ? l36 : l36 + 4];
-		const uint32_t dn = seedDN[(size_t) read * HU_MAX_SEEDS + s];
-		const uint32_t pv = parDN[(size_t) read * HU_MAX_SEEDS + s];
-		const double cDist = (double)(dn >> 16) / (double)(dn & 0xffffu);
-		const double pDist = (double)(pv >> 16) / (double)(pv & 0xffffu);
-		ratio = cDist / (cDist + pDist);
-		if(isnan(ratio)) ratio = 0.5;
-		ratio = __hiloint2double(__builtin_amdgcn_readfirstlane(__double2hiint(ratio)), __builtin_amdgcn_readfirstlane(__double2loint(ratio)));
-		const double w0 = db.blen[un];
-		const double wur = w0 * ratio, wvr = w0 - wur;
-		const int l6 = lane < 6 ? lane : 0, m3 = l6 % 3;
-		const double e = exp((m3 == 0 ? mdl.lam[1] : m3 == 1 ? mdl.lam[2] : mdl.lam[3]) * (l6 < 3 ? wur : wvr));
-		if(lane < 6) pro[lane] = e;
 		if(weighted) {
-			double piw[4];
-			{ double mx = max4d(mdl.logpi), sm; for(int i = 0; i < 4; ++i) piw[i] = exp(mdl.logpi[i] - mx); sm = (piw[0] + piw[2]) + (piw[1] + piw[3]); for(int i = 0; i < 4; ++i) piw[i] /= sm; }
-			if(lane < 4) pro[8 + lane] = sel4(piw, lane);
+			double w[4];
+			{ double mx = max4d(M().logpi), sm; for(int i = 0; i < 4; ++i) w[i] = exp(M().logpi[i] - mx); sm = (w[0] + w[2]) + (w[1] + w[3]); for(int i = 0; i < 4; ++i) w[i] /= sm; }
+			if(lane < 4) piw[lane] = sel4(w, lane);
 		}
 		if(lane < 36) mtab[lane] = mc;
 	}
-	const int start = rstart[read], end = rend[read], n = end - start + 1;
-	const int8_t* __restrict__ cd = codes + (size_t) read * db.csLen + start;
-	const int64_t sOff = (int64_t) un * db.winLen + (start - db.winStart);
-	const int piMax = argmax4d(mdl.logpi);
-	double z[SPT][4]; unsigned long long bop = 0; int ksum = 0;
-	double Eu[3], Ev[3];
-	double aU[SPT][4], aV[SPT][4];
-	const double* __restrict__ Ub = db.up + sOff * 4; const double* __restrict__ Vb = db.down + sOff * 4;
-	const int32_t* __restrict__ upKb = db.upK + sOff; const int32_t* __restrict__ downKb = db.downK + sOff;
-	auto inr = [&](int t) { return tid < n - THREADS * t; };
-	stamp(0);
-	{
-		int kU[SPT], kV[SPT];
+	lds_barrier();
+	for(int par = 0;; par ^= 1) {
+		asm volatile("" : "+s"(zero));
+		asm volatile("" : "+v"(tid));
+		lane = tid & 63;
+		const int4 r0 = rec[par][0], r1 = rec[par][1];
+		const int state = __builtin_amdgcn_readfirstlane(r0.x);
+		if(state == HU_EST_END) break;
+		uint32_t npos = ~0u;
+		if(scout) npos = settle(tpend);
+		if(state == HU_EST_SKIP) {
+			if(scout) { chain(npos); finish(par ^ 1); tpend = draw(); }
+			lds_barrier();
+			continue;
+		}
+		const int read = __builtin_amdgcn_readfirstlane(r0.y), un = __builtin_amdgcn_readfirstlane(r0.w);
+		const int start = __builtin_amdgcn_readfirstlane(r1.x), n = __builtin_amdgcn_readfirstlane(r1.y);
+		const int8_t* __restrict__ cd = codes + (size_t) read * D().csLen + start;
+		const int piMax = argmax4d(M().logpi);
+		const int64_t sOff = (int64_t) un * D().winLen + (start - D().winStart);
+		double z[SPT][4]; unsigned long long bop = 0; int ksum = 0;
+		double Eu[3], Ev[3];
+		double aU[SPT][4], aV[SPT][4];
+		const double* __restrict__ Ub = D().up + sOff * 4; const double* __restrict__ Vb = D().down + sOff * 4;
+		const int32_t* __restrict__ upKb = D().upK + sOff; const int32_t* __restrict__ downKb = D().downK + sOff;
+		auto inr = [&](int t) { return tid < n - THREADS * t; };
+		stamp(0);
+		{
+			int kU[SPT], kV[SPT];
+			__builtin_amdgcn_sched_barrier(0);
+#pragma unroll
+			for(int t = 0; t < SPT; ++t) {
+				const int jj = inr(t) ? tid + THREADS * t : 0;
+				kU[t] = upKb[(size_t) jj]; kV[t] = downKb[(size_t) jj];
+			}
+			__builtin_amdgcn_sched_barrier(0);
+#pragma unroll
+			for(int t = 0; t < SPT; ++t) {
+				const int jj = inr(t) ? tid + THREADS * t : 0;
+				load4(Ub + (size_t) jj * 4, aU[t]); load4(Vb + (size_t) jj * 4, aV[t]);
+				const int b = cd[jj];
+				bop |= (unsigned long long)(b >= 0 ? b : 4) << (3 * t);
+			}
+			__builtin_amdgcn_sched_barrier(0);
+			if(scout) chain(npos);
+			{
+				const double e = pro[par][lane < 6 ? lane : 0];
+				const int lo = __double2loint(e), hi = __double2hiint(e);
+#pragma unroll
+				for(int k = 0; k < 3; ++k) {
+					Eu[k] = __hiloint2double(__builtin_amdgcn_readlane(hi, k), __builtin_amdgcn_readlane(lo, k));
+					Ev[k] = __hiloint2double(__builtin_amdgcn_readlane(hi, 3 + k), __builtin_amdgcn_readlane(lo, 3 + k));
+				}
+			}
+#pragma unroll
+			for(int t = 0; t < SPT; ++t) {
+				asm volatile("" : "+v"(kU[t]), "+v"(kV[t]));
+				ksum += inr(t) ? kU[t] + kV[t] : 0;
+			}
+			asm volatile("" : "+v"(ksum));
+		}
+		if(DBG) { double x = 0; for(int t = 0; t < SPT; ++t) x += aU[t][0] + aV[t][0]; if(x == 1.2345e-300 || bop == ~0ull) tk[2] = 1; }
+		stamp(1);
+		{
+#pragma unroll
+			for(int t = 0; t < SPT; ++t) {
+				const double su1 = Eu[0] * aU[t][1], su2 = Eu[1] * aU[t][2], su3 = Eu[2] * aU[t][3];
+				const double sv1 = Ev[0] * aV[t][1], sv2 = Ev[1] * aV[t][2], sv3 = Ev[2] * aV[t][3];
+#pragma unroll
+				for(int i = 0; i < 4; ++i) {
+					const double cu = fmax(fma(M().U[i*4+3], su3, fma(M().U[i*4+2], su2, fma(M().U[i*4+1], su1, aU[t][0]))), 0.0);
+					const double cv = fmax(fma(M().U[i*4+3], sv3, fma(M().U[i*4+2], sv2, fma(M().U[i*4+1], sv1, aV[t][0]))), 0.0);
+					z[t][i] = cu * cv;
+				}
+			}
+		}
+		double wnr = 0;
+		if(!weighted) {
+			int nd = 0;
+#pragma unroll
+			for(int t = 0; t < SPT; ++t) {
+				const int bi = (int)((bop >> (3 * t)) & 7u);
+				const int b1 = argmax4_tied_lin(z[t]), b2 = bi < 4 ? bi : piMax;
+				nd += __popcll(__ballot(inr(t) && b1 != b2));
+			}
+			if(lane == 0) redi[wave] = nd;
+			lds_barrier();
+			if(builder) {
+				int tot = redi[0];
+#pragma unroll
+				for(int w = 1; w < NW; ++w) tot += redi[w];
+				wnr = (double) tot / (double) n;
+			}
+		}
+		else {
+			const double piwGap = piw[piMax];
+			double dsum = 0, nsum = 0;
+#pragma unroll
+			for(int t = 0; t < SPT; ++t) {
+				if(!inr(t)) continue;
+				const int bi = (int)((bop >> (3 * t)) & 7u);
+				const int b1 = argmax4_tied_lin(z[t]), b2 = bi < 4 ? bi : piMax;
+				const double w1 = sel4(z[t], b1) / ((z[t][0] + z[t][2]) + (z[t][1] + z[t][3]));
+				const double w2 = bi < 4 ? 1.0 : piwGap;
+				if(b1 != b2) dsum += w1 * w2;
+				nsum += w1 * w2;
+			}
+			dsum = wave_sum(dsum); nsum = wave_sum(nsum);
+			if(lane == 0) { redw[wave] = dsum; redw[NW + wave] = nsum; }
+			lds_barrier();
+			if(builder) {
+				double a = redw[0], c = redw[NW];
+#pragma unroll
+				for(int w = 1; w < NW; ++w) { a += redw[w]; c += redw[NW + w]; }
+				wnr = a / c;
+			}
+		}
+		double* Q = Qtab;
+		if(scout) { finish(par ^ 1); tpend = draw(); }
+		if(builder) {
+			if(lane < 3) Q[1 + lane] = hu_exp_call((lane == 0 ? M().lam[1] : lane == 1 ? M().lam[2] : M().lam[3]) * wnr);
+			lds_wave_sync();
+			if(lane < 20) {
+				const int b = lane >> 2, i = lane & 3;
+				const double* mU = mtab + 4 + i * 4, * mU1 = mtab + 20 + (b & 3);
+				const double pii = mtab[i];
+				double c;
+				if(wnr == 0) c = b < 4 ? (i == b ? 1.0 : 0.0) : pii;
+				else {
+					double a0, a1, a2, a3;
+					if(b < 4) { a0 = mU1[0]; a1 = mU1[4]; a2 = mU1[8]; a3 = mU1[12]; }
+					else {
+						a0 = (M().U1[0] * M().pi[0] + M().U1[1] * M().pi[1]) + (M().U1[2] * M().pi[2] + M().U1[3] * M().pi[3]);
+						a1 = (M().U1[4] * M().pi[0] + M().U1[5] * M().pi[1]) + (M().U1[6] * M().pi[2] + M().U1[7] * M().pi[3]);
+						a2 = (M().U1[8] * M().pi[0] + M().U1[9] * M().pi[1]) + (M().U1[10] * M().pi[2] + M().U1[11] * M().pi[3]);
+						a3 = (M().U1[12] * M().pi[0] + M().U1[13] * M().pi[1]) + (M().U1[14] * M().pi[2] + M().U1[15] * M().pi[3]);
+					}
+					const double Ui1 = mU[1], Ui2 = mU[2], Ui3 = mU[3];
+					c = fmax(fma(Ui3, Q[3] * a3, fma(Ui2, Q[2] * a2, fma(Ui1, Q[1] * a1, a0))), 0.0);
+				}
+				Q[4 + b * 4 + i] = pii * c;
+			}
+		}
+		lds_barrier();
+		double mant = 1.0; int esum = ksum;
 #pragma unroll
 		for(int t = 0; t < SPT; ++t) {
-			const int jj = inr(t) ? tid + THREADS * t : 0;
-			kU[t] = upKb[(size_t) jj]; kV[t] = downKb[(size_t) jj];
-		}
-		__builtin_amdgcn_sched_barrier(0);
-#pragma unroll
-		for(int t = 0; t < SPT; ++t) {
-			const int jj = inr(t) ? tid + THREADS * t : 0;
-			load4(Ub + (size_t) jj * 4, aU[t]); load4(Vb + (size_t) jj * 4, aV[t]);
-			const int b = cd[jj];
-			bop |= (unsigned long long)(b >= 0 ? b : 4) << (3 * t);
-		}
-		__builtin_amdgcn_sched_barrier(0);
+			const double* q = Q + 4 + ((bop >> (3 * t)) & 7u) * 4;
+			double x = fmax(fma(q[3], z[t][3], fma(q[2], z[t][2], fma(q[1], z[t][1], q[0] * z[t][0]))), 0.0);
+			if(!inr(t)) x = 1.0;
+			mant *= __builtin_amdgcn_frexp_mant(x);
+			esum += x == 0.0 ? 0 : __builtin_amdgcn_frexp_exp(x);
+		}
+		esum += __builtin_amdgcn_frexp_exp(mant); mant = __builtin_amdgcn_frexp_mant(mant);
+		mant = wave_prod(mant);
+		esum = wave_sum_i32(esum);
+		if(lane == 0) { redd[wave] = mant; redi[NW + wave] = esum; }
+		int4 q0 = make_int4(0, 0, 0, 0), q1 = q0; uint32_t dpos = 0;
+		if(builder) { q0 = rec[par][0]; q1 = rec[par][1]; if(DBG) dpos = (uint32_t) rec[par][2].x; }
 		lds_barrier();
-		{
-			const double e = pro[lane < 6 ? lane : 0];
-			const int lo = __double2loint(e), hi = __double2hiint(e);
-#pragma unroll
-			for(int k = 0; k < 3; ++k) {
-				Eu[k] = __hiloint2double(__builtin_amdgcn_readlane(hi, k), __builtin_amdgcn_readlane(lo, k));
-				Ev[k] = __hiloint2double(__builtin_amdgcn_readlane(hi, 3 + k), __builtin_amdgcn_readlane(lo, 3 + k));
-			}
-		}
-#pragma unroll
-		for(int t = 0; t < SPT; ++t) {
-			asm volatile("" : "+v"(kU[t]), "+v"(kV[t]));
-			ksum += inr(t) ? kU[t] + kV[t] : 0;
-		}
-	}
-	if(DBG) { double x = 0; for(int t = 0; t < SPT; ++t) x += aU[t][0] + aV[t][0]; if(x == 1.2345e-300 || bop == ~0ull) tk[2] = 1; }
-	stamp(1);
-	{
-#pragma unroll
-		for(int t = 0; t < SPT; ++t) {
-			const double su1 = Eu[0] * aU[t][1], su2 = Eu[1] * aU[t][2], su3 = Eu[2] * aU[t][3];
-			const double sv1 = Ev[0] * aV[t][1], sv2 = Ev[1] * aV[t][2], sv3 = Ev[2] * aV[t][3];
-#pragma unroll
-			for(int i = 0; i < 4; ++i) {
-				const double cu = fmax(fma(mdl.U[i*4+3], su3, fma(mdl.U[i*4+2], su2, fma(mdl.U[i*4+1], su1, aU[t][0]))), 0.0);
-				const double cv = fmax(fma(mdl.U[i*4+3], sv3, fma(mdl.U[i*4+2], sv2, fma(mdl.U[i*4+1], sv1, aV[t][0]))), 0.0);
-				z[t][i] = cu * cv;
-			}
-		}
-	}
-	double wnr = 0;
-	if(!weighted) {
-		int nd = 0;
-#pragma unroll
-		for(int t = 0; t < SPT; ++t) {
-			const int bi = (int)((bop >> (3 * t)) & 7u);
-			const int b1 = argmax4_tied_lin(z[t]), b2 = bi < 4 ? bi : piMax;
-			nd += __popcll(__ballot(inr(t) && b1 != b2));
-		}
-		if(lane == 0) redi[wave] = nd;
-		lds_barrier();
-		if(builder) {
-			int tot = redi[0];
-#pragma unroll
-			for(int w = 1; w < NW; ++w) tot += redi[w];
-			wnr = (double) tot / (double) n;
-		}
-	}
-	else {
-		const double piwGap = pro[8 + piMax];
-		double dsum = 0, nsum = 0;
-#pragma unroll
-		for(int t = 0; t < SPT; ++t) {
-			if(!inr(t)) continue;
-			const int bi = (int)((bop >> (3 * t)) & 7u);
-			const int b1 = argmax4_tied_lin(z[t]), b2 = bi < 4 ? bi : piMax;
-			const double w1 = sel4(z[t], b1) / ((z[t][0] + z[t][2]) + (z[t][1] + z[t][3]));
-			const double w2 = bi < 4 ? 1.0 : piwGap;
-			if(b1 != b2) dsum += w1 * w2;
-			nsum += w1 * w2;
-		}
-		dsum = wave_sum(dsum); nsum = wave_sum(nsum);
-		if(lane == 0) { redd[wave] = dsum; redd[NW + wave] = nsum; }
-		lds_barrier();
-		if(builder) {
-			double a = redd[0], c = redd[NW];
-#pragma unroll
-			for(int w = 1; w < NW; ++w) { a += redd[w]; c += redd[NW + w]; }
-			wnr = a / c;
-		}
-	}
-	double* Q = Qtab;
-	if(builder) {
-		if(lane < 3) Q[1 + lane] = exp((lane == 0 ? mdl.lam[1] : lane == 1 ? mdl.lam[2] : mdl.lam[3]) * wnr);
-		lds_wave_sync();
-		if(lane < 20) {
-			const int b = lane >> 2, i = lane & 3;
-			const double* mU = mtab + 4 + i * 4, * mU1 = mtab + 20 + (b & 3);
-			const double pii = mtab[i];
-			double c;
-			if(wnr == 0) c = b < 4 ? (i == b ? 1.0 : 0.0) : pii;
-			else {
-				double a0, a1, a2, a3;
-				if(b < 4) { a0 = mU1[0]; a1 = mU1[4]; a2 = mU1[8]; a3 = mU1[12]; }
-				else {
-					a0 = (mdl.U1[0] * mdl.pi[0] + mdl.U1[1] * mdl.pi[1]) + (mdl.U1[2] * mdl.pi[2] + mdl.U1[3] * mdl.pi[3]);
-					a1 = (mdl.U1[4] * mdl.pi[0] + mdl.U1[5] * mdl.pi[1]) + (mdl.U1[6] * mdl.pi[2] + mdl.U1[7] * mdl.pi[3]);
-					a2 = (mdl.U1[8] * mdl.pi[0] + mdl.U1[9] * mdl.pi[1]) + (mdl.U1[10] * mdl.pi[2] + mdl.U1[11] * mdl.pi[3]);
-					a3 = (mdl.U1[12] * mdl.pi[0] + mdl.U1[13] * mdl.pi[1]) + (mdl.U1[14] * mdl.pi[2] + mdl.U1[15] * mdl.pi[3]);
-				}
-				const double Ui1 = mU[1], Ui2 = mU[2], Ui3 = mU[3];
-				c = fmax(fma(Ui3, Q[3] * a3, fma(Ui2, Q[2] * a2, fma(Ui1, Q[1] * a1, a0))), 0.0);
-			}
-			Q[4 + b * 4 + i] = pii * c;
-		}
-	}
-	lds_barrier();
-	double mant = 1.0; int esum = ksum;
-#pragma unroll
-	for(int t = 0; t < SPT; ++t) {
-		const double* q = Q + 4 + ((bop >> (3 * t)) & 7u) * 4;
-		double x = fmax(fma(q[3], z[t][3], fma(q[2], z[t][2], fma(q[1], z[t][1], q[0] * z[t][0]))), 0.0);
-		if(!inr(t)) x = 1.0;
-		mant *= __builtin_amdgcn_frexp_mant(x);
-		esum += x == 0.0 ? 0 : __builtin_amdgcn_frexp_exp(x);
-	}
-	esum += __builtin_amdgcn_frexp_exp(mant); mant = __builtin_amdgcn_frexp_mant(mant);
-	mant = wave_prod(mant);
-	esum = wave_sum_i32(esum);
-	if(lane == 0) { redd[wave] = mant; redi[NW + wave] = esum; }
-	lds_barrier();
-	if(builder && lane == 0) {
-		double m = redd[0]; long long e = redi[NW];
-#pragma unroll
-		for(int w = 1; w < NW; ++w) { m *= redd[w]; e += redi[NW + w]; }
-		HuEstOut o; o.ratio = ratio; o.wnr = wnr; o.loglik = log(m) + (double) e * HU_LN2;
-		out[(size_t) read * HU_MAX_SEEDS + s] = o;
-	}
-	if(DBG) {
-		stamp(2);
-		if(builder && lane == 0) { tk[3] = tl - t0; for(int i = 0; i < 4; ++i) dbg[(size_t) blockIdx.x * 4 + i] = tk[i]; }
+		if(builder && lane == 0) {
+			double m = redd[0]; long long e = redi[NW];
+#pragma unroll
+			for(int w = 1; w < NW; ++w) { m *= redd[w]; e += redi[NW + w]; }
+			HuEstOut o; o.ratio = __hiloint2double(q1.w, q1.z); o.wnr = wnr; o.loglik = hu_log_call(m) + (double) e * HU_LN2;
+			out[(size_t) q0.y * HU_MAX_SEEDS + q0.z] = o;
+		}
+		if(DBG) {
+			stamp(2);
+			if(builder && lane == 0) { tk[3] = tl - t0; for(int i = 0; i < 4; ++i) dbg[(size_t) dpos * 4 + i] = tk[i]; }
+			t0 = tl; for(int i = 0; i < 4; ++i) tk[i] = 0;
+		}
 	}
 }
 
@@ -363,8 +437,6 @@
 	return fma(fma(-b, q, a), y, q);
 }
 
-__device__ __attribute__((noinline)) double hu_exp_call(double x) { return exp(x); }
-__device__ __attribute__((noinline)) double hu_log_call(double x) { return log(x); }
 
 template<int SPT, int NW, int EMV, int RED>
 __device__ inline double em_branch_blk(const double (&rho)[SPT], int nvalidWave, double q0, double maxL,
diff --git a/profiles/est_isa_count.py b/profiles/est_isa_count.py
--- a/profiles/est_isa_count.py
+++ b/profiles/est_isa_count.py
@@ -43,12 +43,24 @@
     return False
 
 
-def barrier_sets(L):
+def walk_header(L):
+    lab = {l[:-1]: i for i, (_, l) in enumerate(L) if l.endswith(":")}
+    bars = [i for i, (_, l) in enumerate(L) if l.split()[0] == "s_barrier"]
+    heads = []
+    for i, (_, l) in enumerate(L):
+        if l.startswith(("s_cbranch", "s_branch")):
+            t = lab[l.split()[1]]
+            if t <= i and any(t <= b <= i for b in bars):
+                heads.append(t)
+    return min(heads) if heads else None
+
+
+def barrier_sets(L, start=0, cut=None, back=None):
     lab = {l[:-1]: i for i, (_, l) in enumerate(L) if l.endswith(":")}
     arrive = [set() for _ in L]
-    arrive[0].add(0)
+    arrive[start].add(0)
     ends = {}
-    work = [0]
+    work = [start]
     while work:
         i = work.pop()
         _, l = L[i]
@@ -66,6 +78,9 @@
         else:
             nxt = [i + 1]
         for j in nxt:
+            if cut is not None and j == cut:
+                back.update(cnt)
+                continue
             if L[j][1].split()[0] == "s_endpgm" or (L[j][1].endswith(":") and L[j + 1][1] == "s_endpgm"):
                 ends.setdefault(L[i][0], set()).update(cnt)
             if not cnt <= arrive[j]:
@@ -135,6 +150,18 @@
     ap.add_argument("--idle", default="")
     a = ap.parse_args()
     L = kernel_lines(a.listing, a.kernel)
+    head = walk_header(L)
+    if head is not None:
+        to_head, again = set(), set()
+        e0 = barrier_sets(L, 0, head, to_head)
+        e1 = barrier_sets(L, head, head, again)
+        print("k_estimate_prod%s: slot walk with its header at line %d" % (a.kernel, L[head][0]))
+        print("  barriers from the entry to the header: %s; to s_endpgm without entering the loop: %s" % (sorted(to_head), sorted(set().union(*e0.values())) if e0 else []))
+        print("  barriers of one iteration (header to header), all branches both ways: %s" % sorted(again))
+        print("  barriers from the header to s_endpgm: %s" % (sorted(set().union(*e1.values())) if e1 else []))
+        for ln, c in sorted(e1.items()):
+            print("    edge into s_endpgm from line %d: %s" % (ln, sorted(c)))
+        return
     ends = barrier_sets(L)
     allc = set().union(*ends.values())
     print("k_estimate_prod%s: barrier counts at s_endpgm over all paths: %s" % (a.kernel, sorted(allc)))
```

Result: slower. 405,000 (-6.0%).
